# gnlpfjh/Scalable-E3-GNN

Hardware: AMD Instinct MI355X
Metric: particles/sec (octree build + SEGNN fwd), 1M pts l_max=2, 1/2/4/8 MI355X (higher is better)
Workload: dtype f32; 1 GPU; 1000000 particles/GPU uniform in unit box, radius graph k~24 (E=23519616), SEGNN l_max=2 4 layers H=32 f32 storage; particles_per_gpu=1000000, edges_per_gpu=23519616, hidden=32, layers=4, lmax=2, parallelism=single GPU

## Files before the change

include/e3gnn.h:

```cpp
#ifndef E3GNN_H
#define E3GNN_H

#include <stdint.h>

#ifdef __cplusplus
extern "C" {
#endif

#define E3GNN_ABI_VERSION 3

enum {
  E3_OK = 0,
  E3_ERR_INVALID_ARG = 1,
  E3_ERR_BAD_IRREPS = 2,
  E3_ERR_MISSING_WEIGHT = 3,
  E3_ERR_UNSUPPORTED = 4,
  E3_ERR_HIP = 5,
  E3_ERR_NO_DEVICE = 6
};

enum { E3_F32 = 0, E3_F64 = 1, E3_BF16 = 2 };

enum { E3_CLS_0E = 0, E3_CLS_0O = 1, E3_CLS_1E = 2, E3_CLS_1O = 3 };

typedef struct e3_l1tp_plan e3_l1tp_plan;

int         e3_abi_version(void);
const char* e3_status_string(int status);
const char* e3_last_hip_error(void);

int e3_l1tp_plan_create(const int32_t* in1_blocks, int n_in1,
                        const int32_t* out_blocks, int n_out,
                        e3_l1tp_plan** plan);
int e3_l1tp_plan_destroy(e3_l1tp_plan* plan);

int e3_l1tp_in1_dim(const e3_l1tp_plan* plan);
int e3_l1tp_out_dim(const e3_l1tp_plan* plan);
int e3_l1tp_weight_shape(const e3_l1tp_plan* plan, int cls, int* rows, int* cols);
int e3_l1tp_norm_len(const e3_l1tp_plan* plan, int cls);

int64_t e3_l1tp_packed_bytes(const e3_l1tp_plan* plan, int dtype);
int e3_l1tp_pack_weights(const e3_l1tp_plan* plan,
                         const void* const weights[4], const void* const norms[4],
                         int dtype, void* packed, void* stream);

int e3_l1tp_forward(const e3_l1tp_plan* plan,
                    const void* in1, int64_t ld_in1,
                    const void* in2, int64_t ld_in2,
                    const void* packed,
                    void* out, int64_t ld_out,
                    int64_t B, int dtype, int kernel, void* stream);

int64_t e3_l1tp_backward_workspace_bytes(const e3_l1tp_plan* plan, int64_t B, int dtype);
int e3_l1tp_backward(const e3_l1tp_plan* plan,
                     const void* in1, int64_t ld_in1,
                     const void* in2, int64_t ld_in2,
                     const void* const weights[4], const void* const norms[4],
                     const void* grad_out, int64_t ld_gout,
                     void* grad_in1, int64_t ld_gin1,
                     void* grad_in2,
                     void* const grad_weights[4],
                     void* workspace,
                     int64_t B, int dtype, void* stream);

typedef struct e3_rg_params {
  float lo[3], hi[3];
  float r;
  int32_t n[3];
  float inv[3];
  int32_t bits;
} e3_rg_params;

int     e3_rg_grid(e3_rg_params* prm);
int64_t e3_rg_workspace_bytes(int64_t N, const e3_rg_params* prm);
int e3_rg_sort_count(const float* pos, int64_t N, const e3_rg_params* prm,
                     int32_t* perm, float* sorted_pos4, int32_t* rowptr,
                     void* workspace, int64_t workspace_bytes, void* stream);
int e3_rg_fill(int64_t N, const e3_rg_params* prm, const float* sorted_pos4, const int32_t* rowptr,
               int32_t* src, void* workspace, int64_t workspace_bytes, void* stream);

int e3_rg_sort_count_pbc(const float* pos, int64_t N, const e3_rg_params* prm, int32_t periodic,
                         int32_t* perm, float* sorted_pos4, int32_t* rowptr,
                         void* workspace, int64_t workspace_bytes, void* stream);
int e3_rg_fill_pbc(int64_t N, const e3_rg_params* prm, int32_t periodic, const float* sorted_pos4,
                   const int32_t* rowptr, int32_t* src, void* workspace, int64_t workspace_bytes, void* stream);

int e3_cell_derive(const float cell[9], float ginv[9], float heights[3], float* volume);
int e3_rg_sort_count_cell(const float* pos, int64_t N, const e3_rg_params* prm, const float cell[9], const float origin[3],
                          int32_t* perm, float* sorted_pos4, int32_t* rowptr,
                          void* workspace, int64_t workspace_bytes, void* stream);
int e3_rg_fill_cell(int64_t N, const e3_rg_params* prm, const float cell[9], const float origin[3],
                    const float* sorted_pos4, const int32_t* rowptr, int32_t* src,
                    void* workspace, int64_t workspace_bytes, void* stream);

int e3_edge_geometry(const float* pos4, const int32_t* rowptr, const int32_t* src, int64_t N,
                     float* edge_y, float* edge_d, float* node_a, void* stream);
int e3_edge_geometry_pbc(const float* pos4, const int32_t* rowptr, const int32_t* src, int64_t N, const float box[3],
                         float* edge_y, float* edge_d, float* node_a, void* stream);
int e3_edge_geometry_cell(const float* pos4, const int32_t* rowptr, const int32_t* src, int64_t N, const float cell[9],
                          float* edge_y, float* edge_d, float* node_a, void* stream);
int e3_gather_concat(const float* h, int64_t ld_h, int D, const int32_t* rowptr, const int32_t* src, int64_t N,
                     const float* extra, int n_extra, float* out, int64_t ld_out, void* stream);
int e3_gate(const float* in, int64_t ld_in, float* out, int64_t ld_out, int64_t B, int ns, int nv, void* stream);
int e3_segment_sum(const float* msg, int64_t ld_msg, const int32_t* rowptr, int64_t N, int D,
                   float* agg, int64_t ld_agg, void* stream);

int64_t e3_split_edges_workspace_bytes(int64_t N);
int e3_split_edges(const int32_t* rowptr, const int32_t* src, const uint8_t* is_ghost, int64_t N, int64_t E,
                   int32_t* rowptr_kept, int32_t* src_kept, int32_t* dst_kept, int32_t* src_interior, int32_t* dst_interior,
                   int32_t* src_boundary, int32_t* dst_boundary, int32_t* counts, void* workspace, void* stream);

#define E3_HALO_MAX_ENTRIES 26
typedef struct e3_halo_entry {
  float lo[3], hi[3], shift[3];
} e3_halo_entry;
int64_t e3_halo_select_workspace_bytes(int64_t n, int n_entries);
int e3_halo_select_count(const float* pos, int64_t n, const float lo[3], const float hi[3], int32_t periodic, float r,
                         const e3_halo_entry* entries, int n_entries, float* pos_wrapped, int32_t* counts, void* workspace,
                         int64_t workspace_bytes, void* stream);
int e3_halo_select_fill(const float* pos_wrapped, int64_t n, const float lo[3], const float hi[3], int32_t periodic, float r,
                        const e3_halo_entry* entries, int n_entries, int64_t total, int32_t* idx, float* ghost_pos,
                        void* workspace, int64_t workspace_bytes, void* stream);

#define E3_MORTON_MAX_RANKS 64
int e3_morton_keys(const float* pos, int64_t n, const float lo[3], const float hi[3], const int32_t n_cells[3], int32_t* keys,
                   void* stream);
int64_t e3_morton_select_workspace_bytes(int64_t n, int n_ranks);
int e3_morton_select_count(const float* pos, int64_t n, const float lo[3], const float hi[3], const int32_t n_cells[3], float r,
                           const int32_t* splitters, int n_ranks, int self_rank, int32_t* counts, void* workspace,
                           int64_t workspace_bytes, void* stream);
int e3_morton_select_fill(const float* pos, int64_t n, const float lo[3], const float hi[3], const int32_t n_cells[3], float r,
                          const int32_t* splitters, int n_ranks, int self_rank, int64_t total, int32_t* idx, void* workspace,
                          int64_t workspace_bytes, void* stream);

typedef struct e3_tp_plan e3_tp_plan;
typedef struct e3_tp_segment {
  const void* base;
  int64_t ld;
  const int32_t* row_index;
  int32_t ncols;
  int32_t reserved;
} e3_tp_segment;
int e3_tp_plan_create(const int32_t* in1_blocks, int n_in1, int lmax_sh,
                      const int32_t* out_blocks, int n_out, e3_tp_plan** plan);
int e3_tp_plan_destroy(e3_tp_plan* plan);
int e3_tp_in1_dim(const e3_tp_plan* plan);
int e3_tp_in2_dim(const e3_tp_plan* plan);
int e3_tp_out_dim(const e3_tp_plan* plan);
int e3_tp_weight_shape(const e3_tp_plan* plan, int cls, int* rows, int* cols);
int e3_tp_norm_len(const e3_tp_plan* plan, int cls);
int64_t e3_tp_packed_bytes(const e3_tp_plan* plan, int dtype);
int e3_tp_pack_weights(const e3_tp_plan* plan, const void* const weights[6], const void* const norms[6],
                       int dtype, void* packed, void* stream);
int e3_tp_forward(const e3_tp_plan* plan, const void* in1, int64_t ld_in1, const void* in2, int64_t ld_in2,
                  const void* packed, void* out, int64_t ld_out, int64_t B, int dtype, const float* in_scale,
                  int exact, void* stream);
int e3_pow2_scale(const e3_tp_segment* segs, const int64_t* nrows, int nseg, int target_log2, float* out4,
                  void* stream);
int e3_add_pow2_scale(const float* h, const float* u, float* out, int64_t n, int target_log2, float* out4,
                      void* stream);
int e3_tp_forward_fused(const e3_tp_plan* plan, const e3_tp_segment* segs, int nseg,
                        const void* in2, int64_t ld_in2, const void* packed, void* out, int64_t ld_out,
                        int64_t B, int dtype, int gate, const float* in_scale, void* stream);
int e3_tp_forward_fused_epilogue(const e3_tp_plan* plan, const e3_tp_segment* segs, int nseg, const void* in2,
                                 int64_t ld_in2, const void* packed, void* out, int64_t ld_out, int64_t B, int dtype,
                                 int gate, const float* in_scale, const void* residual, int64_t ld_residual,
                                 float* out_scale4, int target_log2, void* stream);
int e3_tp_forward_update_pair(const e3_tp_plan* plan1, const e3_tp_plan* plan2, const e3_tp_segment* segs, int nseg,
                              const void* in2, int64_t ld_in2, const void* packed1, const void* packed2,
                              const float* in_scale, const void* residual, int64_t ld_residual, void* out,
                              int64_t ld_out, int64_t B, int dtype, float* out_scale4, int target_log2, void* stream);
int e3_tp_backward(const e3_tp_plan* plan, const void* in1, int64_t ld_in1, const void* in2, int64_t ld_in2,
                   const void* packed, const void* grad_out, int64_t ld_gout, void* grad_in1, int64_t ld_gin1,
                   void* grad_in2, int64_t ld_gin2, void* const grad_weights[6], int64_t B, int dtype, void* stream);
int e3_tp_backward_weights(const e3_tp_plan* plan, const void* in1, int64_t ld_in1, const void* in2, int64_t ld_in2,
                           const void* packed, const void* grad_out, int64_t ld_gout, void* const grad_weights[6],
                           int64_t B, int dtype, void* stream);
int e3_tp_backward_operands(const e3_tp_plan* plan, const void* in1, int64_t ld_in1, const void* in2, int64_t ld_in2,
                            const void* packed, const void* grad_out, int64_t ld_gout, void* const features[6],
                            void* const gout[6], int64_t B, int dtype, void* stream);
int e3_tp_backward_contract(const e3_tp_plan* plan, const void* in1, int64_t ld_in1, const void* in2, int64_t ld_in2,
                            void* const t[6], void* grad_in1, int64_t ld_gin1, void* grad_in2, int64_t ld_gin2,
                            int64_t B, int dtype, void* stream);
int e3_tp_fused_supported(const e3_tp_plan* plan, int gate);
const char* e3_tp_last_fused_kernel(void);
int e3_tp_forward_fused_scatter(const e3_tp_plan* plan, const e3_tp_segment* segs, int nseg,
                                const void* in2, int64_t ld_in2, const void* packed, const int32_t* row_node,
                                void* out_nodes, int64_t ld_out, int64_t B, int dtype, int gate,
                                const float* in_scale, void* stream);
typedef struct e3_msg_plan e3_msg_plan;
int e3_msg_plan_create(int lmax, int hidden, e3_msg_plan** plan);
int e3_msg_plan_destroy(e3_msg_plan* plan);
int64_t e3_msg_packed_bytes(const e3_msg_plan* plan);
int64_t e3_msg_premix_floats_per_node(const e3_msg_plan* plan);
int e3_msg_weight_shape(const e3_msg_plan* plan, int tp , int l3, int* rows, int* cols);
int e3_msg_supports(const e3_msg_plan* plan, int dtype);
int e3_msg_pack_weights(e3_msg_plan* plan, const void* const w1[3], const void* const n1[3],
                        const void* const w2[3], const void* const n2[3], int dtype, void* packed, void* stream);
int e3_msg_premix(e3_msg_plan* plan, const void* h, int64_t ld_h, int64_t N, const void* packed,
                  const float* in_scale, float* premix, int dtype, void* stream);
int e3_msg_forward(e3_msg_plan* plan, const void* h, int64_t ld_h, int64_t N, const float* pos4,
                   const int32_t* src, const int32_t* dst, int64_t E, const void* packed, const float* in_scale,
                   const float* premix, float* out, int64_t ld_out, int dtype, int accumulate, int tiles_per_block,
                   void* stream);
int e3_msg_forward_pbc(e3_msg_plan* plan, const void* h, int64_t ld_h, int64_t N, const float* pos4,
                       const int32_t* src, const int32_t* dst, int64_t E, const void* packed, const float* in_scale,
                       const float* premix, float* out, int64_t ld_out, int dtype, int accumulate, int tiles_per_block,
                       const float box[3], void* stream);
int e3_msg_forward_cell(e3_msg_plan* plan, const void* h, int64_t ld_h, int64_t N, const float* pos4,
                        const int32_t* src, const int32_t* dst, int64_t E, const void* packed, const float* in_scale,
                        const float* premix, float* out, int64_t ld_out, int dtype, int accumulate, int tiles_per_block,
                        const float cell[9], void* stream);
int e3_segment_sum_bf16(const void* msg, int64_t ld_msg, const int32_t* rowptr, int64_t N, int D,
                        void* agg, int64_t ld_agg, void* stream);
int e3_edge_geometry_l2(const float* pos4, const int32_t* rowptr, const int32_t* src, int64_t N,
                        float* edge_y, float* edge_d, float* node_a, void* stream);
int e3_edge_geometry_l2_pbc(const float* pos4, const int32_t* rowptr, const int32_t* src, int64_t N, const float box[3],
                            float* edge_y, float* edge_d, float* node_a, void* stream);
int e3_edge_geometry_l2_cell(const float* pos4, const int32_t* rowptr, const int32_t* src, int64_t N, const float cell[9],
                             float* edge_y, float* edge_d, float* node_a, void* stream);
int e3_gate_blocks(const float* in, int64_t ld_in, float* out, int64_t ld_out, int64_t B, int ns,
                   int nblocks, const int32_t* ls, const int32_t* muls, void* stream);

int e3_edge_geometry_backward(const float* pos4, const int32_t* rowptr, const int32_t* src, int64_t N, int lmax,
                              const float* g_edge_y, const float* g_edge_d, const float* g_node_a, float* g_pos,
                              void* stream);
int e3_edge_geometry_backward_pbc(const float* pos4, const int32_t* rowptr, const int32_t* src, int64_t N, int lmax,
                                  const float box[3], const float* g_edge_y, const float* g_edge_d,
                                  const float* g_node_a, float* g_pos, void* stream);
int e3_edge_geometry_backward_cell(const float* pos4, const int32_t* rowptr, const int32_t* src, int64_t N, int lmax,
                                   const float cell[9], const float* g_edge_y, const float* g_edge_d,
                                   const float* g_node_a, float* g_pos, void* stream);
int e3_gather_concat_backward(const float* g_out, int64_t ld_gout, int D, const int32_t* rowptr, const int32_t* src,
                              int64_t N, int n_extra, float* g_h, int64_t ld_gh, float* g_extra, void* stream);

int e3_edge_geometry_strained(const float* pos4, const int32_t* rowptr, const int32_t* src, int64_t N, int lmax,
                              const float* box, const float* strain, const int32_t* structure, int S, float* edge_y,
                              float* edge_d, float* node_a, void* stream);
int64_t e3_edge_geometry_backward_strained_workspace_bytes(int64_t N);
int e3_edge_geometry_backward_strained(const float* pos4, const int32_t* rowptr, const int32_t* src, int64_t N, int lmax,
                                       const float* box, const float* strain, const int32_t* structure, int S,
                                       const float* g_edge_y, const float* g_edge_d, const float* g_node_a, float* g_pos,
                                       float* g_strain, void* workspace, int64_t workspace_bytes, void* stream);
int e3_edge_geometry_strained_cell(const float* pos4, const int32_t* rowptr, const int32_t* src, int64_t N, int lmax,
                                   const float cell[9], const float* strain, const int32_t* structure, int S,
                                   float* edge_y, float* edge_d, float* node_a, void* stream);
int e3_edge_geometry_backward_strained_cell(const float* pos4, const int32_t* rowptr, const int32_t* src, int64_t N,
                                            int lmax, const float cell[9], const float* strain, const int32_t* structure,
                                            int S, const float* g_edge_y, const float* g_edge_d, const float* g_node_a,
                                            float* g_pos, float* g_strain, void* workspace, int64_t workspace_bytes,
                                            void* stream);
int e3_gate_blocks_backward(const float* in, int64_t ld_in, const float* g_out, int64_t ld_gout, float* g_in,
                            int64_t ld_gin, int64_t B, int ns, int nblocks, const int32_t* ls, const int32_t* muls,
                            void* stream);
int e3_segment_sum_backward(const float* g_agg, int64_t ld_gagg, const int32_t* rowptr, int64_t N, int D, float* g_msg,
                            int64_t ld_gmsg, void* stream);

#ifdef __cplusplus
}
#endif
#endif
```

scalable-e3-gnn_amd/_lib.py:

```python
from __future__ import annotations

import ctypes
import os
from ctypes import POINTER, c_char_p, c_int, c_int32, c_int64, c_void_p

_HERE = os.path.dirname(os.path.abspath(__file__))
LIB_PATH = os.path.join(_HERE, "lib", "libe3gnn_hip.so")

E3_OK = 0
E3_F32, E3_F64, E3_BF16 = 0, 1, 2
CLS_NAMES = ("l0e", "l0o", "l1e", "l1o")

_lib = None

VoidP4 = c_void_p * 4
Float3 = ctypes.c_float * 3
Float9 = ctypes.c_float * 9
Int3 = c_int32 * 3


class HaloEntry(ctypes.Structure):
    _fields_ = [("lo", ctypes.c_float * 3), ("hi", ctypes.c_float * 3), ("shift", ctypes.c_float * 3)]


SIGNATURES = {
    "e3_abi_version": (c_int, []),
    "e3_status_string": (c_char_p, [c_int]),
    "e3_last_hip_error": (c_char_p, []),
    "e3_l1tp_plan_create": (c_int, [POINTER(c_int32), c_int, POINTER(c_int32), c_int, POINTER(c_void_p)]),
    "e3_l1tp_plan_destroy": (c_int, [c_void_p]),
    "e3_l1tp_in1_dim": (c_int, [c_void_p]),
    "e3_l1tp_out_dim": (c_int, [c_void_p]),
    "e3_l1tp_weight_shape": (c_int, [c_void_p, c_int, POINTER(c_int), POINTER(c_int)]),
    "e3_l1tp_norm_len": (c_int, [c_void_p, c_int]),
    "e3_l1tp_packed_bytes": (c_int64, [c_void_p, c_int]),
    "e3_l1tp_pack_weights": (c_int, [c_void_p, VoidP4, VoidP4, c_int, c_void_p, c_void_p]),
    "e3_l1tp_forward": (c_int, [c_void_p, c_void_p, c_int64, c_void_p, c_int64, c_void_p, c_void_p, c_int64,
                                c_int64, c_int, c_int, c_void_p]),
    "e3_l1tp_backward_workspace_bytes": (c_int64, [c_void_p, c_int64, c_int]),
    "e3_rg_grid": (c_int, [c_void_p]),
    "e3_rg_workspace_bytes": (c_int64, [c_int64, c_void_p]),
    "e3_rg_sort_count": (c_int, [c_void_p, c_int64, c_void_p, c_void_p, c_void_p, c_void_p, c_void_p, c_int64,
                                 c_void_p]),
    "e3_rg_fill": (c_int, [c_int64, c_void_p, c_void_p, c_void_p, c_void_p, c_void_p, c_int64, c_void_p]),
    "e3_edge_geometry": (c_int, [c_void_p, c_void_p, c_void_p, c_int64, c_void_p, c_void_p, c_void_p, c_void_p]),
    "e3_gather_concat": (c_int, [c_void_p, c_int64, c_int, c_void_p, c_void_p, c_int64, c_void_p, c_int, c_void_p,
                                 c_int64, c_void_p]),
    "e3_gate": (c_int, [c_void_p, c_int64, c_void_p, c_int64, c_int64, c_int, c_int, c_void_p]),
    "e3_segment_sum": (c_int, [c_void_p, c_int64, c_void_p, c_int64, c_int, c_void_p, c_int64, c_void_p]),
    "e3_split_edges_workspace_bytes": (c_int64, [c_int64]),
    "e3_split_edges": (c_int, [c_void_p, c_void_p, c_void_p, c_int64, c_int64, c_void_p, c_void_p, c_void_p, c_void_p,
                               c_void_p, c_void_p, c_void_p, c_void_p, c_void_p, c_void_p]),
    "e3_halo_select_workspace_bytes": (c_int64, [c_int64, c_int]),
    "e3_halo_select_count": (c_int, [c_void_p, c_int64, Float3, Float3, c_int32, ctypes.c_float, c_void_p, c_int, c_void_p,
                                     c_void_p, c_void_p, c_int64, c_void_p]),
    "e3_halo_select_fill": (c_int, [c_void_p, c_int64, Float3, Float3, c_int32, ctypes.c_float, c_void_p, c_int, c_int64,
                                    c_void_p, c_void_p, c_void_p, c_int64, c_void_p]),
    "e3_morton_keys": (c_int, [c_void_p, c_int64, Float3, Float3, Int3, c_void_p, c_void_p]),
    "e3_morton_select_workspace_bytes": (c_int64, [c_int64, c_int]),
    "e3_morton_select_count": (c_int, [c_void_p, c_int64, Float3, Float3, Int3, ctypes.c_float, POINTER(c_int32), c_int,
                                       c_int, c_void_p, c_void_p, c_int64, c_void_p]),
    "e3_morton_select_fill": (c_int, [c_void_p, c_int64, Float3, Float3, Int3, ctypes.c_float, POINTER(c_int32), c_int,
                                      c_int, c_int64, c_void_p, c_void_p, c_int64, c_void_p]),
    "e3_tp_plan_create": (c_int, [POINTER(c_int32), c_int, c_int, POINTER(c_int32), c_int, POINTER(c_void_p)]),
    "e3_tp_plan_destroy": (c_int, [c_void_p]),
    "e3_tp_in1_dim": (c_int, [c_void_p]),
    "e3_tp_in2_dim": (c_int, [c_void_p]),
    "e3_tp_out_dim": (c_int, [c_void_p]),
    "e3_tp_weight_shape": (c_int, [c_void_p, c_int, POINTER(c_int), POINTER(c_int)]),
    "e3_tp_norm_len": (c_int, [c_void_p, c_int]),
    "e3_tp_packed_bytes": (c_int64, [c_void_p, c_int]),
    "e3_tp_pack_weights": (c_int, [c_void_p, c_void_p * 6, c_void_p * 6, c_int, c_void_p, c_void_p]),
    "e3_tp_forward": (c_int, [c_void_p, c_void_p, c_int64, c_void_p, c_int64, c_void_p, c_void_p, c_int64, c_int64,
                              c_int, c_void_p, c_int, c_void_p]),
    "e3_tp_forward_fused": (c_int, [c_void_p, c_void_p, c_int, c_void_p, c_int64, c_void_p, c_void_p, c_int64, c_int64,
                                    c_int, c_int, c_void_p, c_void_p]),
    "e3_msg_plan_create": (c_int, [c_int, c_int, POINTER(c_void_p)]),
    "e3_msg_plan_destroy": (c_int, [c_void_p]),
    "e3_msg_packed_bytes": (c_int64, [c_void_p]),
    "e3_msg_premix_floats_per_node": (c_int64, [c_void_p]),
    "e3_msg_weight_shape": (c_int, [c_void_p, c_int, c_int, POINTER(c_int), POINTER(c_int)]),
    "e3_msg_supports": (c_int, [c_void_p, c_int]),
    "e3_msg_pack_weights": (c_int, [c_void_p, c_void_p * 3, c_void_p * 3, c_void_p * 3, c_void_p * 3, c_int, c_void_p,
                                    c_void_p]),
    "e3_msg_premix": (c_int, [c_void_p, c_void_p, c_int64, c_int64, c_void_p, c_void_p, c_void_p, c_int, c_void_p]),
    "e3_msg_forward": (c_int, [c_void_p, c_void_p, c_int64, c_int64, c_void_p, c_void_p, c_void_p, c_int64, c_void_p,
                               c_void_p, c_void_p, c_void_p, c_int64, c_int, c_int, c_int, c_void_p]),
    "e3_edge_geometry_backward": (c_int, [c_void_p, c_void_p, c_void_p, c_int64, c_int, c_void_p, c_void_p, c_void_p,
                                          c_void_p, c_void_p]),
    "e3_rg_sort_count_pbc": (c_int, [c_void_p, c_int64, c_void_p, c_int32, c_void_p, c_void_p, c_void_p, c_void_p,
                                     c_int64, c_void_p]),
    "e3_rg_fill_pbc": (c_int, [c_int64, c_void_p, c_int32, c_void_p, c_void_p, c_void_p, c_void_p, c_int64, c_void_p]),
    "e3_edge_geometry_pbc": (c_int, [c_void_p, c_void_p, c_void_p, c_int64, Float3, c_void_p, c_void_p, c_void_p,
                                     c_void_p]),
    "e3_edge_geometry_l2_pbc": (c_int, [c_void_p, c_void_p, c_void_p, c_int64, Float3, c_void_p, c_void_p, c_void_p,
                                        c_void_p]),
    "e3_edge_geometry_backward_pbc": (c_int, [c_void_p, c_void_p, c_void_p, c_int64, c_int, Float3, c_void_p, c_void_p,
                                              c_void_p, c_void_p, c_void_p]),
    "e3_msg_forward_pbc": (c_int, [c_void_p, c_void_p, c_int64, c_int64, c_void_p, c_void_p, c_void_p, c_int64,
                                   c_void_p, c_void_p, c_void_p, c_void_p, c_int64, c_int, c_int, c_int, Float3,
                                   c_void_p]),
    "e3_cell_derive": (c_int, [Float9, Float9, Float3, POINTER(ctypes.c_float)]),
    "e3_rg_sort_count_cell": (c_int, [c_void_p, c_int64, c_void_p, Float9, Float3, c_void_p, c_void_p, c_void_p, c_void_p,
                                      c_int64, c_void_p]),
    "e3_rg_fill_cell": (c_int, [c_int64, c_void_p, Float9, Float3, c_void_p, c_void_p, c_void_p, c_void_p, c_int64,
                                c_void_p]),
    "e3_edge_geometry_cell": (c_int, [c_void_p, c_void_p, c_void_p, c_int64, Float9, c_void_p, c_void_p, c_void_p,
                                      c_void_p]),
    "e3_edge_geometry_l2_cell": (c_int, [c_void_p, c_void_p, c_void_p, c_int64, Float9, c_void_p, c_void_p, c_void_p,
                                         c_void_p]),
    "e3_edge_geometry_backward_cell": (c_int, [c_void_p, c_void_p, c_void_p, c_int64, c_int, Float9, c_void_p, c_void_p,
                                               c_void_p, c_void_p, c_void_p]),
    "e3_msg_forward_cell": (c_int, [c_void_p, c_void_p, c_int64, c_int64, c_void_p, c_void_p, c_void_p, c_int64,
                                    c_void_p, c_void_p, c_void_p, c_void_p, c_int64, c_int, c_int, c_int, Float9,
                                    c_void_p]),
    "e3_edge_geometry_strained_cell": (c_int, [c_void_p, c_void_p, c_void_p, c_int64, c_int, Float9, c_void_p, c_void_p,
                                               c_int, c_void_p, c_void_p, c_void_p, c_void_p]),
    "e3_edge_geometry_backward_strained_cell": (c_int, [c_void_p, c_void_p, c_void_p, c_int64, c_int, Float9, c_void_p,
                                                        c_void_p, c_int, c_void_p, c_void_p, c_void_p, c_void_p, c_void_p,
                                                        c_void_p, c_int64, c_void_p]),
    "e3_gather_concat_backward": (c_int, [c_void_p, c_int64, c_int, c_void_p, c_void_p, c_int64, c_int, c_void_p, c_int64,
                                          c_void_p, c_void_p]),
    "e3_gate_blocks_backward": (c_int, [c_void_p, c_int64, c_void_p, c_int64, c_void_p, c_int64, c_int64, c_int, c_int,
                                        POINTER(c_int32), POINTER(c_int32), c_void_p]),
    "e3_segment_sum_backward": (c_int, [c_void_p, c_int64, c_void_p, c_int64, c_int, c_void_p, c_int64, c_void_p]),
    "e3_pow2_scale": (c_int, [c_void_p, POINTER(c_int64), c_int, c_int, c_void_p, c_void_p]),
    "e3_add_pow2_scale": (c_int, [c_void_p, c_void_p, c_void_p, c_int64, c_int, c_void_p, c_void_p]),
    "e3_tp_backward": (c_int, [c_void_p, c_void_p, c_int64, c_void_p, c_int64, c_void_p, c_void_p, c_int64, c_void_p,
                               c_int64, c_void_p, c_int64, c_void_p * 6, c_int64, c_int, c_void_p]),
    "e3_tp_backward_weights": (c_int, [c_void_p, c_void_p, c_int64, c_void_p, c_int64, c_void_p, c_void_p, c_int64, c_void_p,
                                       c_int64, c_int, c_void_p]),
    "e3_tp_backward_operands": (c_int, [c_void_p, c_void_p, c_int64, c_void_p, c_int64, c_void_p, c_void_p, c_int64, c_void_p,
                                        c_void_p, c_int64, c_int, c_void_p]),
    "e3_tp_backward_contract": (c_int, [c_void_p, c_void_p, c_int64, c_void_p, c_int64, c_void_p, c_void_p, c_int64, c_void_p,
                                        c_int64, c_int64, c_int, c_void_p]),
    "e3_tp_forward_fused_epilogue": (c_int, [c_void_p, c_void_p, c_int, c_void_p, c_int64, c_void_p, c_void_p, c_int64,
                                             c_int64, c_int, c_int, c_void_p, c_void_p, c_int64, c_void_p, c_int, c_void_p]),
    "e3_tp_forward_update_pair": (c_int, [c_void_p, c_void_p, c_void_p, c_int, c_void_p, c_int64, c_void_p, c_void_p,
                                          c_void_p, c_void_p, c_int64, c_void_p, c_int64, c_int64, c_int, c_void_p, c_int,
                                          c_void_p]),
    "e3_tp_fused_supported": (c_int, [c_void_p, c_int]),
    "e3_tp_last_fused_kernel": (ctypes.c_char_p, []),
    "e3_tp_forward_fused_scatter": (c_int, [c_void_p, c_void_p, c_int, c_void_p, c_int64, c_void_p, c_void_p, c_void_p,
                                            c_int64, c_int64, c_int, c_int, c_void_p, c_void_p]),
    "e3_segment_sum_bf16": (c_int, [c_void_p, c_int64, c_void_p, c_int64, c_int, c_void_p, c_int64, c_void_p]),
    "e3_edge_geometry_l2": (c_int, [c_void_p, c_void_p, c_void_p, c_int64, c_void_p, c_void_p, c_void_p, c_void_p]),
    "e3_gate_blocks": (c_int, [c_void_p, c_int64, c_void_p, c_int64, c_int64, c_int, c_int, POINTER(c_int32),
                               POINTER(c_int32), c_void_p]),
    "e3_l1tp_backward": (c_int, [c_void_p, c_void_p, c_int64, c_void_p, c_int64, VoidP4, VoidP4, c_void_p, c_int64,
                                 c_void_p, c_int64, c_void_p, VoidP4, c_void_p, c_int64, c_int, c_void_p]),
    "e3_edge_geometry_strained": (c_int, [c_void_p, c_void_p, c_void_p, c_int64, c_int, POINTER(ctypes.c_float), c_void_p,
                                          c_void_p, c_int, c_void_p, c_void_p, c_void_p, c_void_p]),
    "e3_edge_geometry_backward_strained_workspace_bytes": (c_int64, [c_int64]),
    "e3_edge_geometry_backward_strained": (c_int, [c_void_p, c_void_p, c_void_p, c_int64, c_int, POINTER(ctypes.c_float),
                                                   c_void_p, c_void_p, c_int, c_void_p, c_void_p, c_void_p, c_void_p,
                                                   c_void_p, c_void_p, c_int64, c_void_p]),
}


def load():
    global _lib
    if _lib is not None:
        return _lib
    if not os.path.exists(LIB_PATH):
        raise RuntimeError(
            f"{LIB_PATH} is missing: the HIP library has not been built. Run "
            "`python -c 'import __graft_entry__ as g; g.build()'` (or `make -C scalable-e3-gnn_amd/csrc`). "
            "There is no CPU fallback.")
    import torch

    lib = ctypes.CDLL(LIB_PATH)
    for name, (res, args) in SIGNATURES.items():
        fn = getattr(lib, name, None)
        if fn is None:
            continue
        fn.restype = res
        fn.argtypes = args
    _lib = lib
    return lib


def check(status: int, what: str = ""):
    if status != E3_OK:
        lib = load()
        msg = lib.e3_status_string(status).decode()
        if status == 5:
            msg += " — " + lib.e3_last_hip_error().decode()
        raise RuntimeError(f"libe3gnn_hip: {what}: {msg} (status {status})")


def blocks_array(blocks):
    flat = [int(v) for b in blocks for v in b]
    return (c_int32 * len(flat))(*flat), len(blocks)


def ptr4(tensors):
    return VoidP4(*[(t.data_ptr() if (t is not None and t.numel() > 0) else None) for t in tensors])


def dtype_code(dtype) -> int:
    import torch

    try:
        return {torch.float32: E3_F32, torch.float64: E3_F64, torch.bfloat16: E3_BF16}[dtype]
    except KeyError:
        raise RuntimeError(f"libe3gnn_hip supports float32 / float64 / bfloat16, got {dtype}") from None


class DevicePlans:

    def __init__(self, create_name: str, destroy_name: str, *args):
        self._create, self._destroy_name, self._args = create_name, destroy_name, args
        self._handles = {}

    def _make(self):
        lib = load()
        cargs = []
        for a in self._args:
            if isinstance(a, (list, tuple)):
                arr, n = blocks_array(a)
                cargs += [arr, n]
            else:
                cargs.append(int(a))
        h = c_void_p()
        check(getattr(lib, self._create)(*cargs, ctypes.byref(h)), self._create)
        return h

    def handle(self, device=None) -> c_void_p:
        key = -1
        if device is not None:
            import torch
            key = torch.device(device).index
            if key is None:
                key = torch.cuda.current_device()
        h = self._handles.get(key)
        if h is None:
            h = self._handles[key] = self._make()
        return h

    def __deepcopy__(self, memo):
        return DevicePlans(self._create, self._destroy_name, *self._args)

    def __reduce__(self):
        return (DevicePlans, (self._create, self._destroy_name) + tuple(self._args))

    def __del__(self):
        try:
            lib = load()
            for h in self._handles.values():
                if h:
                    getattr(lib, self._destroy_name)(h)
            self._handles = {}
        except Exception:
            pass
```

scalable-e3-gnn_amd/csrc/e3_edge_ops.hip:

```cpp
#include "e3_common.h"

#include <algorithm>
#include <cmath>

namespace e3 {

constexpr float kSqrt3 = 1.7320508075688772f;

template <int PBC, bool STRAIN>
__global__ __launch_bounds__(256) void edge_geometry_kernel(const float4* __restrict__ pos4,
                                                            const int32_t* __restrict__ rowptr,
                                                            const int32_t* __restrict__ src, int64_t N,
                                                            float4* __restrict__ edge_y, float* __restrict__ edge_d,
                                                            float4* __restrict__ node_a,
                                                            const typename PbcArg<PBC>::type box, const StrainArg st) {
  const int lane = threadIdx.x & 63;
  const int64_t wave0 = (blockIdx.x * (int64_t)blockDim.x + threadIdx.x) >> 6;
  const int64_t nw = ((int64_t)gridDim.x * blockDim.x) >> 6;
  for (int64_t i = wave0; i < N; i += nw) {
    const int b = rowptr[i], e = rowptr[i + 1];
    const float4 pi = pos4[i];
    float eps[9];
    if constexpr (STRAIN) load_strain(st, row_structure(st, i), eps);
    float sx = 0.f, sy = 0.f, sz = 0.f;
    for (int q = b + lane; q < e; q += 64) {
      const float4 pj = pos4[src[q]];
      float rx, ry, rz;
      edge_rel<PBC>(pj, pi, box, rx, ry, rz);
      if constexpr (STRAIN) apply_strain(eps, rx, ry, rz);
      const float d = sqrtf(rx * rx + ry * ry + rz * rz);
      const float s = d > 0.f ? kSqrt3 / d : 0.f;
      const float4 y = make_float4(1.0f, s * rx, s * ry, s * rz);
      if (edge_y) edge_y[q] = y;
      if (edge_d) edge_d[q] = d;
      sx += y.y; sy += y.z; sz += y.w;
    }
    if (node_a) {
      for (int o = 32; o > 0; o >>= 1) {
        sx += __shfl_xor(sx, o);
        sy += __shfl_xor(sy, o);
        sz += __shfl_xor(sz, o);
      }
      if (lane == 0) {
        const float inv = e > b ? 1.0f / (float)(e - b) : 0.f;
        node_a[i] = make_float4(1.0f, sx * inv, sy * inv, sz * inv);
      }
    }
  }
}

__global__ __launch_bounds__(256) void gather_concat_kernel(const float* __restrict__ h, int64_t ld_h, int D,
                                                            const int32_t* __restrict__ rowptr,
                                                            const int32_t* __restrict__ src, int64_t N,
                                                            const float* __restrict__ extra, int n_extra,
                                                            float* __restrict__ out, int64_t ld_out) {
  const int lane = threadIdx.x & 63;
  const int64_t wave0 = (blockIdx.x * (int64_t)blockDim.x + threadIdx.x) >> 6;
  const int64_t nw = ((int64_t)gridDim.x * blockDim.x) >> 6;
  for (int64_t i = wave0; i < N; i += nw) {
    const int b = rowptr[i], e = rowptr[i + 1];
    if (b == e) continue;
    const float* hi = h + i * ld_h;
    for (int c0 = 0; c0 < D; c0 += 64) {
      const int c = c0 + lane;
      const float vi = c < D ? hi[c] : 0.f;
      for (int q = b; q < e; ++q) {
        if (c < D) {
          float* o = out + (int64_t)q * ld_out;
          o[c] = vi;
          o[D + c] = h[(int64_t)src[q] * ld_h + c];
        }
      }
    }
    for (int q = b; q < e; ++q)
      if (lane < n_extra) out[(int64_t)q * ld_out + 2 * D + lane] = extra[(int64_t)q * n_extra + lane];
  }
}

__device__ __forceinline__ float sigmoidf_(float x) { return 1.0f / (1.0f + __expf(-x)); }

__global__ __launch_bounds__(256) void gate_kernel(const float* __restrict__ in, int64_t ld_in, float* __restrict__ out,
                                                   int64_t ld_out, int64_t B, int ns, int nv) {
  const int W = ns + 3 * nv;
  const int64_t total = B * (int64_t)W;
  for (int64_t t = blockIdx.x * (int64_t)blockDim.x + threadIdx.x; t < total; t += (int64_t)gridDim.x * blockDim.x) {
    const int64_t row = t / W;
    const int c = (int)(t - row * W);
    const float* x = in + row * ld_in;
    float v;
    if (c < ns) {
      const float s = x[c];
      v = s * sigmoidf_(s);
    } else {
      const int k = (c - ns) / 3;
      v = sigmoidf_(x[ns + k]) * x[ns + nv + (c - ns)];
    }
    out[row * ld_out + c] = v;
  }
}

__global__ __launch_bounds__(256) void segment_sum_kernel(const float* __restrict__ msg, int64_t ld_msg,
                                                          const int32_t* __restrict__ rowptr, int64_t N, int D,
                                                          float* __restrict__ agg, int64_t ld_agg) {
  const int lane = threadIdx.x & 63;
  const int64_t wave0 = (blockIdx.x * (int64_t)blockDim.x + threadIdx.x) >> 6;
  const int64_t nw = ((int64_t)gridDim.x * blockDim.x) >> 6;
  for (int64_t i = wave0; i < N; i += nw) {
    const int b = rowptr[i], e = rowptr[i + 1];
    for (int c = lane; c < D; c += 64) {
      float acc = 0.f;
      const float* m = msg + (int64_t)b * ld_msg + c;
#pragma unroll 4
      for (int q = b; q < e; ++q) {
        acc += *m;
        m += ld_msg;
      }
      agg[i * ld_agg + c] = acc;
    }
  }
}


template <int PBC, bool STRAIN>
__global__ __launch_bounds__(256) void edge_geometry_l2_kernel(const float4* __restrict__ pos4,
                                                               const int32_t* __restrict__ rowptr,
                                                               const int32_t* __restrict__ src, int64_t N,
                                                               float* __restrict__ edge_y, float* __restrict__ edge_d,
                                                               float* __restrict__ node_a,
                                                               const typename PbcArg<PBC>::type box, const StrainArg st) {
  const int lane = threadIdx.x & 63;
  const int64_t wave0 = (blockIdx.x * (int64_t)blockDim.x + threadIdx.x) >> 6;
  const int64_t nw = ((int64_t)gridDim.x * blockDim.x) >> 6;
  const float s5 = 2.2360679774997896f;
  for (int64_t i = wave0; i < N; i += nw) {
    const int b = rowptr[i], e = rowptr[i + 1];
    const float4 pi = pos4[i];
    float eps[9];
    if constexpr (STRAIN) load_strain(st, row_structure(st, i), eps);
    float acc[8] = {0, 0, 0, 0, 0, 0, 0, 0};
    for (int q = b + lane; q < e; q += 64) {
      const float4 pj = pos4[src[q]];
      float rx, ry, rz;
      edge_rel<PBC>(pj, pi, box, rx, ry, rz);
      if constexpr (STRAIN) apply_strain(eps, rx, ry, rz);
      const float d = sqrtf(rx * rx + ry * ry + rz * rz);
      const float inv = d > 0.f ? 1.0f / d : 0.f;
      const float x = rx * inv, y = ry * inv, z = rz * inv;
      float Y[9];
      Y[0] = 1.0f;
      Y[1] = kSqrt3 * x; Y[2] = kSqrt3 * y; Y[3] = kSqrt3 * z;
      Y[4] = s5 * kSqrt3 * x * y;
      Y[5] = s5 * kSqrt3 * y * z;
      Y[6] = s5 * 0.5f * (2.f * z * z - x * x - y * y);
      Y[7] = s5 * kSqrt3 * z * x;
      Y[8] = s5 * 0.5f * kSqrt3 * (x * x - y * y);
      if (edge_y) {
        float* o = edge_y + (int64_t)q * 9;
#pragma unroll
        for (int k = 0; k < 9; ++k) o[k] = Y[k];
      }
      if (edge_d) edge_d[q] = d;
#pragma unroll
      for (int k = 0; k < 8; ++k) acc[k] += Y[k + 1];
    }
    if (node_a) {
#pragma unroll
      for (int k = 0; k < 8; ++k)
        for (int o = 32; o > 0; o >>= 1) acc[k] += __shfl_xor(acc[k], o);
      if (lane == 0) {
        const float inv = e > b ? 1.0f / (float)(e - b) : 0.f;
        float* a = node_a + i * 9;
        a[0] = 1.0f;
#pragma unroll
        for (int k = 0; k < 8; ++k) a[k + 1] = acc[k] * inv;
      }
    }
  }
}

struct GateBlocks {
  int nblocks;
  int l[8], mul[8];
};

__global__ __launch_bounds__(256) void gate_blocks_kernel(const float* __restrict__ in, int64_t ld_in,
                                                          float* __restrict__ out, int64_t ld_out, int64_t B, int ns,
                                                          int ngates, int W, GateBlocks gb) {
  const int64_t total = B * (int64_t)W;
  for (int64_t t = blockIdx.x * (int64_t)blockDim.x + threadIdx.x; t < total; t += (int64_t)gridDim.x * blockDim.x) {
    const int64_t row = t / W;
    int c = (int)(t - row * W);
    const float* x = in + row * ld_in;
    float v;
    if (c < ns) {
      const float s = x[c];
      v = s * sigmoidf_(s);
    } else {
      int rem = c - ns, g0 = 0, bi = 0;
      while (rem >= gb.mul[bi] * (2 * gb.l[bi] + 1)) { rem -= gb.mul[bi] * (2 * gb.l[bi] + 1); g0 += gb.mul[bi]; ++bi; }
      const int k = rem / (2 * gb.l[bi] + 1);
      v = sigmoidf_(x[ns + g0 + k]) * x[ngates + c];
    }
    out[row * ld_out + c] = v;
  }
}

__global__ __launch_bounds__(256) void segment_sum_bf16_kernel(const bf16* __restrict__ msg, int64_t ld_msg,
                                                               const int32_t* __restrict__ rowptr, int64_t N, int D,
                                                               bf16* __restrict__ agg, int64_t ld_agg) {
  const int lane = threadIdx.x & 63;
  const int64_t wave0 = (blockIdx.x * (int64_t)blockDim.x + threadIdx.x) >> 6;
  const int64_t nw = ((int64_t)gridDim.x * blockDim.x) >> 6;
  for (int64_t i = wave0; i < N; i += nw) {
    const int b = rowptr[i], e = rowptr[i + 1];
    for (int c = lane; c < D; c += 64) {
      float acc = 0.f;
      const bf16* m = msg + (int64_t)b * ld_msg + c;
#pragma unroll 4
      for (int q = b; q < e; ++q) {
        acc += __bfloat162float(*m);
        m += ld_msg;
      }
      agg[i * ld_agg + c] = __float2bfloat16(acc);
    }
  }
}

static inline int wave_grid(int64_t N) { return (int)std::max<int64_t>(1, std::min<int64_t>((N + 3) / 4, 256 * 16)); }

}

using namespace e3;

template <int PBC>
static int edge_geometry(int lmax, const float* pos4, const int32_t* rowptr, const int32_t* src, int64_t N, float* edge_y,
                         float* edge_d, float* node_a, const typename PbcArg<PBC>::type& b, const StrainArg* st,
                         void* stream) {
  if (N < 0) return E3_ERR_INVALID_ARG;
  if (N == 0) return E3_OK;
  if (!pos4 || !rowptr || !src || (!edge_y && !node_a)) return E3_ERR_INVALID_ARG;
  const StrainArg sa = st ? *st : StrainArg{nullptr, nullptr, 0};
  const hipStream_t s = (hipStream_t)stream;
  if (lmax == 1) {
    auto kern = st ? edge_geometry_kernel<PBC, true> : edge_geometry_kernel<PBC, false>;
    hipLaunchKernelGGL(kern, dim3(wave_grid(N)), dim3(256), 0, s, (const float4*)pos4, rowptr, src, N, (float4*)edge_y,
                       edge_d, (float4*)node_a, b, sa);
  } else {
    auto kern = st ? edge_geometry_l2_kernel<PBC, true> : edge_geometry_l2_kernel<PBC, false>;
    hipLaunchKernelGGL(kern, dim3(wave_grid(N)), dim3(256), 0, s, (const float4*)pos4, rowptr, src, N, edge_y, edge_d,
                       node_a, b, sa);
  }
  E3_HIP_CHECK(hipGetLastError());
  return E3_OK;
}
static int edge_geometry(int lmax, const float* pos4, const int32_t* rowptr, const int32_t* src, int64_t N, float* edge_y,
                         float* edge_d, float* node_a, const float* box, const StrainArg* st, void* stream) {
  const PbcBox b = make_box(box);
  return box ? edge_geometry<kBox>(lmax, pos4, rowptr, src, N, edge_y, edge_d, node_a, b, st, stream)
             : edge_geometry<kOpen>(lmax, pos4, rowptr, src, N, edge_y, edge_d, node_a, b, st, stream);
}

bool e3::cell_derive(const float* cell, float ginv[9], float heights[3], float* volume) {
#pragma clang fp contract(off)
  if (!cell) return false;
  double a[9];
  for (int k = 0; k < 9; ++k) {
    if (!(fabs((double)cell[k]) < 3.0e38)) return false;
    a[k] = (double)cell[k];
  }
  const double c00 = a[4] * a[8] - a[5] * a[7], c01 = a[5] * a[6] - a[3] * a[8], c02 = a[3] * a[7] - a[4] * a[6];
  const double c10 = a[2] * a[7] - a[1] * a[8], c11 = a[0] * a[8] - a[2] * a[6], c12 = a[1] * a[6] - a[0] * a[7];
  const double c20 = a[1] * a[5] - a[2] * a[4], c21 = a[2] * a[3] - a[0] * a[5], c22 = a[0] * a[4] - a[1] * a[3];
  const double det = (a[0] * c00 + a[1] * c01) + a[2] * c02;
  if (!(fabs(det) > 0.0)) return false;
  const double g[9] = {c00 / det, c10 / det, c20 / det, c01 / det, c11 / det, c21 / det, c02 / det, c12 / det, c22 / det};
  for (int k = 0; k < 9; ++k) {
    ginv[k] = (float)g[k];
    if (!(fabsf(ginv[k]) < 3.0e38f)) return false;
  }
  for (int c = 0; c < 3; ++c) {
    heights[c] = (float)(1.0 / sqrt((g[c] * g[c] + g[3 + c] * g[3 + c]) + g[6 + c] * g[6 + c]));
    if (!(heights[c] > 0.0f && heights[c] < 3.0e38f)) return false;
  }
  *volume = (float)fabs(det);
  return *volume > 0.0f && *volume < 3.0e38f;
}

extern "C" {

int e3_edge_geometry(const float* pos4, const int32_t* rowptr, const int32_t* src, int64_t N, float* edge_y,
                     float* edge_d, float* node_a, void* stream) {
  return edge_geometry(1, pos4, rowptr, src, N, edge_y, edge_d, node_a, nullptr, nullptr, stream);
}

int e3_edge_geometry_pbc(const float* pos4, const int32_t* rowptr, const int32_t* src, int64_t N, const float box[3],
                         float* edge_y, float* edge_d, float* node_a, void* stream) {
  if (!box_valid(box, 0.0f)) return E3_ERR_INVALID_ARG;
  return edge_geometry(1, pos4, rowptr, src, N, edge_y, edge_d, node_a, box, nullptr, stream);
}

int e3_cell_derive(const float cell[9], float ginv[9], float heights[3], float* volume) {
  if (!ginv || !heights || !volume) return E3_ERR_INVALID_ARG;
  return cell_derive(cell, ginv, heights, volume) ? E3_OK : E3_ERR_INVALID_ARG;
}

int e3_edge_geometry_cell(const float* pos4, const int32_t* rowptr, const int32_t* src, int64_t N, const float cell[9],
                          float* edge_y, float* edge_d, float* node_a, void* stream) {
  PbcCell c;
  if (!make_cell(cell, 0.0f, &c)) return E3_ERR_INVALID_ARG;
  return edge_geometry<kCell>(1, pos4, rowptr, src, N, edge_y, edge_d, node_a, c, nullptr, stream);
}

int e3_edge_geometry_l2_cell(const float* pos4, const int32_t* rowptr, const int32_t* src, int64_t N, const float cell[9],
                             float* edge_y, float* edge_d, float* node_a, void* stream) {
  PbcCell c;
  if (!make_cell(cell, 0.0f, &c)) return E3_ERR_INVALID_ARG;
  return edge_geometry<kCell>(2, pos4, rowptr, src, N, edge_y, edge_d, node_a, c, nullptr, stream);
}

int e3_edge_geometry_strained_cell(const float* pos4, const int32_t* rowptr, const int32_t* src, int64_t N, int lmax,
                                   const float cell[9], const float* strain, const int32_t* structure, int S,
                                   float* edge_y, float* edge_d, float* node_a, void* stream) {
  PbcCell c;
  if ((lmax != 1 && lmax != 2) || !strain || S < 1 || !make_cell(cell, 0.0f, &c)) return E3_ERR_INVALID_ARG;
  const StrainArg st = {strain, structure, S};
  return edge_geometry<kCell>(lmax, pos4, rowptr, src, N, edge_y, edge_d, node_a, c, &st, stream);
}

int e3_gather_concat(const float* h, int64_t ld_h, int D, const int32_t* rowptr, const int32_t* src, int64_t N,
                     const float* extra, int n_extra, float* out, int64_t ld_out, void* stream) {
  if (N < 0 || D <= 0 || n_extra < 0 || n_extra > 64 || ld_out < 2 * D + n_extra) return E3_ERR_INVALID_ARG;
  if (N == 0) return E3_OK;
  if (!h || !rowptr || !src || !out || (n_extra > 0 && !extra)) return E3_ERR_INVALID_ARG;
  hipLaunchKernelGGL(gather_concat_kernel, dim3(wave_grid(N)), dim3(256), 0, (hipStream_t)stream, h, ld_h, D, rowptr,
                     src, N, extra, n_extra, out, ld_out);
  E3_HIP_CHECK(hipGetLastError());
  return E3_OK;
}

int e3_gate(const float* in, int64_t ld_in, float* out, int64_t ld_out, int64_t B, int ns, int nv, void* stream) {
  if (B < 0 || ns < 0 || nv < 0 || ld_in < ns + 4 * nv || ld_out < ns + 3 * nv) return E3_ERR_INVALID_ARG;
  if (B == 0 || ns + nv == 0) return E3_OK;
  if (!in || !out) return E3_ERR_INVALID_ARG;
  int64_t total = B * (int64_t)(ns + 3 * nv);
  int grid = (int)std::min<int64_t>((total + 255) / 256, 256 * 16);
  hipLaunchKernelGGL(gate_kernel, dim3(grid), dim3(256), 0, (hipStream_t)stream, in, ld_in, out, ld_out, B, ns, nv);
  E3_HIP_CHECK(hipGetLastError());
  return E3_OK;
}

int e3_segment_sum(const float* msg, int64_t ld_msg, const int32_t* rowptr, int64_t N, int D, float* agg,
                   int64_t ld_agg, void* stream) {
  if (N < 0 || D <= 0 || ld_msg < D || ld_agg < D) return E3_ERR_INVALID_ARG;
  if (N == 0) return E3_OK;
  if (!msg || !rowptr || !agg) return E3_ERR_INVALID_ARG;
  hipLaunchKernelGGL(segment_sum_kernel, dim3(wave_grid(N)), dim3(256), 0, (hipStream_t)stream, msg, ld_msg, rowptr, N,
                     D, agg, ld_agg);
  E3_HIP_CHECK(hipGetLastError());
  return E3_OK;
}

int e3_segment_sum_bf16(const void* msg, int64_t ld_msg, const int32_t* rowptr, int64_t N, int D, void* agg,
                        int64_t ld_agg, void* stream) {
  if (N < 0 || D <= 0 || ld_msg < D || ld_agg < D) return E3_ERR_INVALID_ARG;
  if (N == 0) return E3_OK;
  if (!msg || !rowptr || !agg) return E3_ERR_INVALID_ARG;
  hipLaunchKernelGGL(segment_sum_bf16_kernel, dim3(wave_grid(N)), dim3(256), 0, (hipStream_t)stream, (const bf16*)msg,
                     ld_msg, rowptr, N, D, (bf16*)agg, ld_agg);
  E3_HIP_CHECK(hipGetLastError());
  return E3_OK;
}

int e3_edge_geometry_l2(const float* pos4, const int32_t* rowptr, const int32_t* src, int64_t N, float* edge_y,
                        float* edge_d, float* node_a, void* stream) {
  return edge_geometry(2, pos4, rowptr, src, N, edge_y, edge_d, node_a, nullptr, nullptr, stream);
}

int e3_edge_geometry_l2_pbc(const float* pos4, const int32_t* rowptr, const int32_t* src, int64_t N, const float box[3],
                            float* edge_y, float* edge_d, float* node_a, void* stream) {
  if (!box_valid(box, 0.0f)) return E3_ERR_INVALID_ARG;
  return edge_geometry(2, pos4, rowptr, src, N, edge_y, edge_d, node_a, box, nullptr, stream);
}

int e3_edge_geometry_strained(const float* pos4, const int32_t* rowptr, const int32_t* src, int64_t N, int lmax,
                              const float* box, const float* strain, const int32_t* structure, int S, float* edge_y,
                              float* edge_d, float* node_a, void* stream) {
  if ((lmax != 1 && lmax != 2) || !strain || S < 1 || (box && !box_valid(box, 0.0f))) return E3_ERR_INVALID_ARG;
  const StrainArg st = {strain, structure, S};
  return edge_geometry(lmax, pos4, rowptr, src, N, edge_y, edge_d, node_a, box, &st, stream);
}

int e3_gate_blocks(const float* in, int64_t ld_in, float* out, int64_t ld_out, int64_t B, int ns, int nblocks,
                   const int32_t* ls, const int32_t* muls, void* stream) {
  if (B < 0 || ns < 0 || nblocks < 0 || nblocks > 8 || (nblocks > 0 && (!ls || !muls))) return E3_ERR_INVALID_ARG;
  GateBlocks gb;
  gb.nblocks = nblocks;
  int ngates = 0, wide = 0;
  for (int i = 0; i < 8; ++i) { gb.l[i] = 0; gb.mul[i] = 1 << 30; }
  for (int i = 0; i < nblocks; ++i) {
    if (ls[i] < 0 || ls[i] > 2 || muls[i] < 0) return E3_ERR_INVALID_ARG;
    gb.l[i] = ls[i]; gb.mul[i] = muls[i];
    ngates += muls[i];
    wide += muls[i] * (2 * ls[i] + 1);
  }
  const int W = ns + wide;
  if (ld_in < W + ngates || ld_out < W) return E3_ERR_INVALID_ARG;
  if (B == 0 || W == 0) return E3_OK;
  if (!in || !out) return E3_ERR_INVALID_ARG;
  int64_t total = B * (int64_t)W;
  int grid = (int)std::min<int64_t>((total + 255) / 256, 256 * 16);
  hipLaunchKernelGGL(gate_blocks_kernel, dim3(grid), dim3(256), 0, (hipStream_t)stream, in, ld_in, out, ld_out, B, ns,
                     ngates, W, gb);
  E3_HIP_CHECK(hipGetLastError());
  return E3_OK;
}

}
```

scalable-e3-gnn_amd/csrc/e3_msg_fused.hip:

```cpp
#include "e3_common.h"
#include "cg_tables.h"
#include "e3_msg_ws.h"

#include <algorithm>
#include <cstddef>
#include <mutex>
#include <type_traits>
#include <utility>
#include <vector>

#ifndef E3_MSG_WD
#define E3_MSG_WD 1
#endif
#ifndef E3_MSG_UDP
#define E3_MSG_UDP 1
#endif
#ifndef E3_MSG_WPS
#define E3_MSG_WPS 2
#endif

#ifndef E3_MSG_STAMP
#define E3_MSG_STAMP 0
#endif

// ... 774 lines not shown
          f32x4 o;
#pragma unroll
          for (int r = 0; r < 4; ++r) {
            const float sv = a0[t][r] * nv[r] * isrow;
            o[r] = sv * sigmoid_(sv);
          }
          *reinterpret_cast<f32x4*>(wp + 16 * t) = o;
        }
        auto put_block = [&](auto dtag, auto& acc, const int slot, const int gslot, float* wq) {
          constexpr int Dc = decltype(dtag)::value;
#pragma unroll
          for (int t = 0; t < TT; ++t) {
            const f32x4 gn = nt2[4 * (gslot + t)];
            float gt[4];
#pragma unroll
            for (int r = 0; r < 4; ++r) gt[r] = sigmoid_(a0[gslot + t][r] * gn[r] * isrow) * isrow;
            float o[4 * Dc];
#pragma unroll
            for (int c = 0; c < Dc; ++c) {
              const f32x4 nv = nt2[4 * (slot + Dc * t + c)];
#pragma unroll
              for (int r = 0; r < 4; ++r) o[r * Dc + c] = acc[t][c][r] * nv[r] * gt[r];
            }
            f32x4* dq = reinterpret_cast<f32x4*>(wq + 16 * t * Dc);
#pragma unroll
            for (int k = 0; k < Dc; ++k) dq[k] = f32x4{o[4 * k], o[4 * k + 1], o[4 * k + 2], o[4 * k + 3]};
          }
        };
        put_block(std::integral_constant<int, 3>{}, a1, G::slot0(1), TT, wbuf + j * RS + H + 12 * g);
        if constexpr (LMAX == 2) put_block(std::integral_constant<int, 5>{}, a2, G::slot0(2), 2 * TT, wbuf + j * RS + 4 * H + 20 * g);
        wave_sync_lds();
        E3_STAMP(6)
        int ln;
        asm volatile("v_mbcnt_lo_u32_b32 %0, -1, 0\n\tv_mbcnt_hi_u32_b32 %0, -1, %0" : "=v"(ln));
        const float* sp = wbuf + ln;
#pragma unroll
        for (int rb = 0; rb < 16; rb += 4) {
          float v[4][NQ];
#pragma unroll
          for (int rr = 0; rr < 4; ++rr)
#pragma unroll
            for (int q = 0; q < NQ; ++q) v[rr][q] = (64 * q + ln < D) ? sp[(rb + rr) * RS + 64 * q] : 0.f;
#pragma unroll
          for (int rr = 0; rr < 4; ++rr) {
            const int dn = __builtin_amdgcn_readlane(sd, rb + rr);
            if (dn >= 0) {
              if (dn != cur) {
                flush();
                cur = dn;
              }
#pragma unroll
              for (int q = 0; q < NQ; ++q) carry[q] += v[rr][q];
            }
          }
        }
      }
      E3_STAMP(7)
    }
    flush();
    cur = -1;
  }
#if E3_MSG_STAMP
  if (lane == 0)
    for (int i = 0; i < 8; ++i) atomicAdd(&g_msg_stamps[i], (unsigned long long)st_acc[i]);
#endif
#undef E3_STAMP
}

static_assert(std::is_same_v<decltype(&msg_fused_kernel<1, 1, false, kCell>),
                             void (*)(decltype(MsgFusedKernarg::hv), decltype(MsgFusedKernarg::ldh), decltype(MsgFusedKernarg::pos4),
                                      decltype(MsgFusedKernarg::src), decltype(MsgFusedKernarg::dst), decltype(MsgFusedKernarg::E),
                                      decltype(MsgFusedKernarg::packed), decltype(MsgFusedKernarg::U),
                                      decltype(MsgFusedKernarg::in_scale), decltype(MsgFusedKernarg::out),
                                      decltype(MsgFusedKernarg::ldo), decltype(MsgFusedKernarg::blk),
                                      decltype(MsgFusedKernarg::cell))>,
              "MsgFusedKernarg must list the parameters of msg_fused_kernel in order");
static_assert(offsetof(MsgFusedKernarg, cell) == 92 && sizeof(PbcCell) == 72, "the cell follows `int blk` at byte 92");

struct MsgKernels {
  int lmax, tt;
  const void* fused[2];
  const void* fused_pbc[2];
  const void* fused_cell[2];
  const void* premix[2];
  int64_t total_floats;
  int UD, D, lds_tab, lds_wave, nblk, NS, WD, o_norm1, o_norm2, o_wd, o_w, waves_per_simd;
};
template <int LMAX, int TT>
static MsgKernels make_entry() {
  using G = MsgGeom<LMAX, TT>;
  MsgKernels k = {LMAX, TT, {(const void*)msg_fused_kernel<LMAX, TT, false, kOpen>, nullptr},
                  {(const void*)msg_fused_kernel<LMAX, TT, false, kBox>, nullptr},
                  {(const void*)msg_fused_kernel<LMAX, TT, false, kCell>, nullptr},
                  {(const void*)msg_premix_kernel<LMAX, TT, false>, nullptr}, G::total_floats,
                  G::UD, G::D, G::lds_tab, G::lds_wave, G::nblk(), G::NS, G::WD, G::o_norm1, G::o_norm2, G::o_wd, G::o_w,
                  msg_waves_per_simd(LMAX, TT)};
  if constexpr (TT >= 2) {
    k.fused[1] = (const void*)msg_fused_kernel<LMAX, TT, true, kOpen>;
    k.fused_pbc[1] = (const void*)msg_fused_kernel<LMAX, TT, true, kBox>;
    k.fused_cell[1] = (const void*)msg_fused_kernel<LMAX, TT, true, kCell>;
    k.premix[1] = (const void*)msg_premix_kernel<LMAX, TT, true>;
  }
  return k;
}
static const std::vector<MsgKernels>& msg_kernels() {
  static const std::vector<MsgKernels> k = {make_entry<2, 2>(), make_entry<1, 2>(), make_entry<2, 1>(), make_entry<1, 1>(),
                                            make_entry<2, 4>(), make_entry<1, 4>()};
  return k;
}

}

using namespace e3;

struct e3_msg_plan {
  int lmax, H;
  const MsgKernels* k;
  std::vector<MsgPackDesc> desc;
  int rowd[3];
  int K1[3], K2[3], M[3];
  MsgPackDesc* d_desc = nullptr;
  int device = -1;
  int grid[2] = {0, 0};
  int grid_pbc[2] = {0, 0};
  int grid_cell[2] = {0, 0};
  std::mutex mu;
};

static int msg_ensure_device(e3_msg_plan* P) {
  std::lock_guard<std::mutex> lock(P->mu);
  int cur = -1;
  if (hipGetDevice(&cur) != hipSuccess) return E3_ERR_NO_DEVICE;
  if (P->d_desc) return cur == P->device ? E3_OK : E3_ERR_INVALID_ARG;
  MsgPackDesc* d = nullptr;
  E3_HIP_CHECK(hipMalloc((void**)&d, P->desc.size() * sizeof(MsgPackDesc)));
  if (hipMemcpy(d, P->desc.data(), P->desc.size() * sizeof(MsgPackDesc), hipMemcpyHostToDevice) != hipSuccess) {
    (void)hipFree(d);
    return E3_ERR_HIP;
  }
  const size_t lds = (size_t)(P->k->lds_tab + 4 * P->k->lds_wave) * 4 + 4 * 256;
  int cus = 0;
  if (hipDeviceGetAttribute(&cus, hipDeviceAttributeMultiprocessorCount, cur) != hipSuccess || cus <= 0) cus = 256;
  for (int io = 0; io < 2; ++io) {
    if (!P->k->fused[io]) continue;
    for (int pb = 0; pb < 2; ++pb) {
      const void* kern = pb ? P->k->fused_pbc[io] : P->k->fused[io];
      int per_cu = 0;
      if (hipFuncSetAttribute(kern, hipFuncAttributeMaxDynamicSharedMemorySize, (int)lds) != hipSuccess ||
          hipOccupancyMaxActiveBlocksPerMultiprocessor(&per_cu, kern, 256, lds) != hipSuccess || per_cu < 1) {
        (void)hipFree(d);
        return E3_ERR_HIP;
      }
      (pb ? P->grid_pbc : P->grid)[io] = cus * (per_cu < 4 ? per_cu : 4);
    }
  }
  P->device = cur;
  P->d_desc = d;
  return E3_OK;
}

static int msg_ensure_cell(e3_msg_plan* P, int io) {
  std::lock_guard<std::mutex> lock(P->mu);
  if (P->grid_cell[io]) return E3_OK;
  const size_t lds = (size_t)(P->k->lds_tab + 4 * P->k->lds_wave) * 4 + 4 * 256;
  int cus = 0, per_cu = 0;
  if (hipDeviceGetAttribute(&cus, hipDeviceAttributeMultiprocessorCount, P->device) != hipSuccess || cus <= 0) cus = 256;
  const void* kern = P->k->fused_cell[io];
  if (!kern || hipFuncSetAttribute(kern, hipFuncAttributeMaxDynamicSharedMemorySize, (int)lds) != hipSuccess ||
      hipOccupancyMaxActiveBlocksPerMultiprocessor(&per_cu, kern, 256, lds) != hipSuccess || per_cu < 1)
    return E3_ERR_HIP;
  P->grid_cell[io] = cus * (per_cu < 4 ? per_cu : 4);
  return E3_OK;
}

extern "C" {

int e3_msg_plan_create(int lmax, int hidden, e3_msg_plan** plan_out) {
  if (!plan_out || lmax < 1 || lmax > 2) return E3_ERR_INVALID_ARG;
  const MsgKernels* k = nullptr;
  for (auto& e : msg_kernels())
    if (e.lmax == lmax && 16 * e.tt == hidden) k = &e;
  if (!k) return E3_ERR_UNSUPPORTED;
  auto* P = new e3_msg_plan();
  P->lmax = lmax; P->H = hidden; P->k = k;
  const int H = hidden, TT = k->tt, KS = (H + 31) / 32;
  auto ok = [&](int l1, int l2, int l3) {
    return l1 <= lmax && l2 <= lmax && l3 <= lmax && ((l1 + l2 + l3) % 2 == 0) && l3 >= std::abs(l1 - l2) && l3 <= l1 + l2;
  };
  auto T = [&](int l3) { return l3 == 0 ? TT * (1 + lmax) : TT; };
  const int n1[3] = {2 * H + 1, 2 * H, 2 * H}, n2[3] = {H, H, H};
  int wrow1[3][3][3], wrow2[3][3][3];
  for (int l3 = 0; l3 <= 2; ++l3) {
    int r1 = 0, r2 = 0;
    for (int l1 = 0; l1 <= 2; ++l1)
      for (int l2 = 0; l2 <= 2; ++l2) {
        wrow1[l1][l2][l3] = wrow2[l1][l2][l3] = -1;
        if (l3 > lmax || !ok(l1, l2, l3)) continue;
        wrow1[l1][l2][l3] = r1; r1 += n1[l1];
        wrow2[l1][l2][l3] = r2; r2 += n2[l1];
      }
    P->K1[l3] = l3 <= lmax ? r1 : 0;
    P->K2[l3] = l3 <= lmax ? r2 : 0;
    P->M[l3] = l3 <= lmax ? 16 * T(l3) : 0;
    P->rowd[l3] = (l3 <= lmax) ? wrow1[0][l3][l3] + 2 * H : 0;
  }
  int b = 0;
  for (int l1 = 0; l1 <= lmax; ++l1)
    for (int l3 = 0; l3 <= lmax; ++l3)
      for (int l2 = 0; l2 <= lmax; ++l2) {
        if (!ok(l1, l2, l3)) continue;
        for (int ks = 0; ks < KS; ++ks)
          for (int t = 0; t < T(l3); ++t) {
            const int nvalid = std::min(32, H - 32 * ks);
            const int M = 16 * T(l3);
            P->desc.push_back({0, l3, wrow1[l1][l2][l3] + H + 32 * ks, nvalid, M, 16 * t, b + ks * T(l3) + t});
            P->desc.push_back({2, l3, wrow1[l1][l2][l3] + 32 * ks, nvalid, M, 16 * t, b + ks * T(l3) + t});
            P->desc.push_back({1, l3, wrow2[l1][l2][l3] + 32 * ks, nvalid, M, 16 * t, b + ks * T(l3) + t});
          }
        b += KS * T(l3);
      }
  if (b != k->nblk) { delete P; return E3_ERR_INVALID_ARG; }
  *plan_out = P;
  return E3_OK;
}

int e3_msg_plan_destroy(e3_msg_plan* P) {
  if (!P) return E3_OK;
  if (P->d_desc) (void)hipFree(P->d_desc);
  delete P;
  return E3_OK;
}

int64_t e3_msg_packed_bytes(const e3_msg_plan* P) { return P ? (P->k->total_floats * 4 + 255) / 256 * 256 : -1; }
int64_t e3_msg_premix_floats_per_node(const e3_msg_plan* P) { return P ? P->k->UD + 1 : -1; }
int e3_msg_weight_shape(const e3_msg_plan* P, int tp, int l3, int* rows, int* cols) {
  if (!P || !rows || !cols || l3 < 0 || l3 > 2 || (tp != 1 && tp != 2)) return E3_ERR_INVALID_ARG;
  *rows = tp == 1 ? P->K1[l3] : P->K2[l3];
  *cols = P->M[l3];
  return E3_OK;
}

int e3_msg_supports(const e3_msg_plan* P, int dtype) {
  if (!P) return 0;
  return dtype == E3_F32 ? 1 : (dtype == E3_BF16 && P->k->fused[1] != nullptr) ? 1 : 0;
}

int e3_msg_pack_weights(e3_msg_plan* P, const void* const w1[3], const void* const n1[3], const void* const w2[3],
                        const void* const n2[3], int dtype, void* packed, void* stream) {
  if (!P || !w1 || !w2 || !packed) return E3_ERR_INVALID_ARG;
  if (!e3_msg_supports(P, dtype)) return E3_ERR_UNSUPPORTED;
  for (int l = 0; l <= P->lmax; ++l)
    if (!w1[l] || !w2[l]) return E3_ERR_MISSING_WEIGHT;
  int st = msg_ensure_device(P);
  if (st != E3_OK) return st;
  const MsgKernels& k = *P->k;
  MsgPackArgs a;
  for (int l = 0; l < 3; ++l) {
    const bool on = l <= P->lmax;
    a.w1[l] = on ? w1[l] : nullptr; a.w2[l] = on ? w2[l] : nullptr;
    a.n1[l] = (on && n1) ? n1[l] : nullptr; a.n2[l] = (on && n2) ? n2[l] : nullptr;
    a.nw1[l] = on ? (int64_t)P->K1[l] * P->M[l] : 0;
    a.nw2[l] = on ? (int64_t)P->K2[l] * P->M[l] : 0;
    a.rowd[l] = P->rowd[l];
  }
  a.M0 = P->M[0]; a.H = P->H; a.LMAX = P->lmax; a.TT = k.tt; a.NS = k.NS; a.WD = k.WD;
  a.o_norm1 = k.o_norm1; a.o_norm2 = k.o_norm2; a.o_wd = k.o_wd; a.o_w = k.o_w; a.nblk = k.nblk;
  hipStream_t s = (hipStream_t)stream;
  E3_HIP_CHECK(hipMemsetAsync(packed, 0, 256, s));
  const dim3 grid(std::min<int>((int)P->desc.size(), 512));
  if (dtype == E3_F32) {
    hipLaunchKernelGGL(msg_absmax_kernel, dim3(64), dim3(256), 0, s, a, (uint32_t*)packed);
    hipLaunchKernelGGL(msg_pack_kernel<float>, grid, dim3(256), 0, s, a, P->d_desc, (int)P->desc.size(), (float*)packed);
  } else {
    hipLaunchKernelGGL(msg_pack_kernel<bf16>, grid, dim3(256), 0, s, a, P->d_desc, (int)P->desc.size(), (float*)packed);
  }
  E3_HIP_CHECK(hipGetLastError());
  return E3_OK;
}

int e3_msg_premix(e3_msg_plan* P, const void* h, int64_t ld_h, int64_t N, const void* packed, const float* in_scale,
                  float* premix, int dtype, void* stream) {
  if (!P || N < 0) return E3_ERR_INVALID_ARG;
  if (!e3_msg_supports(P, dtype)) return E3_ERR_UNSUPPORTED;
  const MsgKernels& k = *P->k;
  const int io = dtype == E3_BF16 ? 1 : 0, es = io ? 2 : 4;
  if (N == 0) return E3_OK;
  if (!h || !packed || !premix || ld_h < k.D) return E3_ERR_INVALID_ARG;
  if ((ld_h * es & 15) || ((uintptr_t)h & 15) || ((uintptr_t)premix & 15)) return E3_ERR_INVALID_ARG;
  int st = msg_ensure_device(P);
  if (st != E3_OK) return st;
  const int64_t ntiles = (N + 15) / 16;
  const int grid = (int)std::min<int64_t>((ntiles + 3) / 4, 2048);
  float* hmax = premix + (size_t)N * k.UD;
  void* args[] = {&h, &ld_h, &N, &packed, &in_scale, &premix, &hmax};
  if (hipLaunchKernel(k.premix[io], dim3(grid), dim3(256), args, 0, (hipStream_t)stream) != hipSuccess) return E3_ERR_HIP;
  return E3_OK;
}

}

static int msg_forward(e3_msg_plan* P, const void* h, int64_t ld_h, int64_t N, const float* pos4, const int32_t* src,
                       const int32_t* dst, int64_t E, const void* packed, const float* in_scale, const float* premix,
                       float* out, int64_t ld_out, int dtype, int accumulate, int tiles_per_block, void* stream,
                       const float* box, const PbcCell* cell = nullptr) {
  if (!P || N < 0 || E < 0 || E > 0x7fffffffLL - 16) return E3_ERR_INVALID_ARG;
  if (!e3_msg_supports(P, dtype)) return E3_ERR_UNSUPPORTED;
  const MsgKernels& k = *P->k;
  const int io = dtype == E3_BF16 ? 1 : 0, es = io ? 2 : 4;
  if (N == 0) return E3_OK;
  if (!h || !pos4 || !packed || !premix || !out || ld_h < k.D || ld_out < k.D || (E > 0 && (!src || !dst)))
    return E3_ERR_INVALID_ARG;
  if ((ld_h * es & 15) || ((uintptr_t)h & 15) || ((uintptr_t)premix & 15)) return E3_ERR_INVALID_ARG;
  int st = msg_ensure_device(P);
  if (st != E3_OK) return st;
  hipStream_t s = (hipStream_t)stream;
  if (!accumulate) E3_HIP_CHECK(hipMemset2DAsync(out, (size_t)ld_out * 4, 0, (size_t)k.D * 4, (size_t)N, s));
  if (E == 0) return E3_OK;
  if (tiles_per_block >= 0 && msg_ws_supported(P->lmax, P->H, dtype)) {
    st = msg_ws_launch(P->lmax, P->H, dtype, h, ld_h, N, pos4, src, dst, E, packed, in_scale, premix, out, ld_out,
                       tiles_per_block > (1 << 20) ? (1 << 24) : tiles_per_block * 16, s, box, cell);
    if (st != E3_ERR_UNSUPPORTED) return st;
  }
  if (tiles_per_block < 0) tiles_per_block = -tiles_per_block;
  if (cell && (st = msg_ensure_cell(P, io)) != E3_OK) return st;
  const int64_t ntiles = (E + 15) / 16;
  int nwg = (cell ? P->grid_cell : (box ? P->grid_pbc : P->grid))[io];
  nwg = (int)std::min<int64_t>(nwg, (ntiles + 3) / 4);
  nwg = std::max(8, (nwg + 7) / 8 * 8);
  int blk = tiles_per_block > 0 ? tiles_per_block : 4;
  if (blk > (1 << 16)) blk = 1 << 16;
  const size_t lds = (size_t)(k.lds_tab + 4 * k.lds_wave) * 4 + 4 * 256;
  PbcBox pbox;
  if (!cell) pbox = make_box(box);
  void* args[] = {&h, &ld_h, &pos4, &src, &dst, &E, &packed, &premix, &in_scale, &out, &ld_out, &blk,
                  cell ? (void*)cell : (void*)&pbox};
  if (hipLaunchKernel(cell ? k.fused_cell[io] : (box ? k.fused_pbc[io] : k.fused[io]), dim3(nwg), dim3(256), args, lds,
                      s) != hipSuccess)
    return E3_ERR_HIP;
  return E3_OK;
}

extern "C" {

int e3_msg_forward(e3_msg_plan* P, const void* h, int64_t ld_h, int64_t N, const float* pos4, const int32_t* src,
                   const int32_t* dst, int64_t E, const void* packed, const float* in_scale, const float* premix,
                   float* out, int64_t ld_out, int dtype, int accumulate, int tiles_per_block, void* stream) {
  return msg_forward(P, h, ld_h, N, pos4, src, dst, E, packed, in_scale, premix, out, ld_out, dtype, accumulate,
                     tiles_per_block, stream, nullptr);
}

int e3_msg_forward_pbc(e3_msg_plan* P, const void* h, int64_t ld_h, int64_t N, const float* pos4, const int32_t* src,
                       const int32_t* dst, int64_t E, const void* packed, const float* in_scale, const float* premix,
                       float* out, int64_t ld_out, int dtype, int accumulate, int tiles_per_block, const float box[3],
                       void* stream) {
  if (!box_valid(box, 0.0f)) return E3_ERR_INVALID_ARG;
  return msg_forward(P, h, ld_h, N, pos4, src, dst, E, packed, in_scale, premix, out, ld_out, dtype, accumulate,
                     tiles_per_block, stream, box);
}

int e3_msg_forward_cell(e3_msg_plan* P, const void* h, int64_t ld_h, int64_t N, const float* pos4, const int32_t* src,
                        const int32_t* dst, int64_t E, const void* packed, const float* in_scale, const float* premix,
                        float* out, int64_t ld_out, int dtype, int accumulate, int tiles_per_block, const float cell[9],
                        void* stream) {
  PbcCell c;
  if (!make_cell(cell, 0.0f, &c)) return E3_ERR_INVALID_ARG;
  return msg_forward(P, h, ld_h, N, pos4, src, dst, E, packed, in_scale, premix, out, ld_out, dtype, accumulate,
                     tiles_per_block, stream, nullptr, &c);
}

#if E3_MSG_STAMP
int e3_msg_debug_stamps(unsigned long long* out8, int reset) {
  if (out8 && hipMemcpyFromSymbol(out8, HIP_SYMBOL(e3::g_msg_stamps), 64) != hipSuccess) return E3_ERR_HIP;
  if (reset) {
    unsigned long long z[8] = {0, 0, 0, 0, 0, 0, 0, 0};
    if (hipMemcpyToSymbol(HIP_SYMBOL(e3::g_msg_stamps), z, 64) != hipSuccess) return E3_ERR_HIP;
  }
  return E3_OK;
}
#endif
}
```

scalable-e3-gnn_amd/csrc/e3_msg_ws.h:

```cpp
#pragma once
#include <hip/hip_runtime.h>
#include <stdint.h>
namespace e3 {
struct PbcCell;
bool msg_ws_supported(int lmax, int hidden, int dtype);
int msg_ws_launch(int lmax, int hidden, int dtype, const void* h, int64_t ldh, int64_t N, const float* pos4, const int32_t* src,
                  const int32_t* dst, int64_t E, const void* packed, const float* in_scale, const float* premix, float* out,
                  int64_t ldo, int chunk_edges, hipStream_t stream, const float* box = nullptr,
                  const PbcCell* cell = nullptr);
}
```

scalable-e3-gnn_amd/csrc/e3_msg_ws.hip:

```cpp
#include "e3_common.h"
#include "cg_tables.h"
#include "e3_msg_ws.h"

#include <algorithm>
#include <type_traits>

#ifndef E3_WS_STAMP
#define E3_WS_STAMP 0
#endif

namespace e3 {
#include "e3_tp_mfma_core.h"
#include "e3_msg_common.h"

#if E3_WS_STAMP
__device__ unsigned long long g_ws_stamps[8][4];
__device__ unsigned long long g_ws_tp[8][8];
#define WS_TPMARK(i) { if (tpm) { const uint32_t t_ = (uint32_t)__builtin_readcyclecounter(); tpm[i] += t_ - tpm0; tpm0 = t_; } }
#else
#define WS_TPMARK(i)
#endif

template <int LMAX, int TT, bool IO16>
struct Ws {
  using G = MsgGeom<LMAX, TT>;
  static_assert(TT == 2 && (LMAX == 1 || LMAX == 2), "instantiated for H = 32, l_max = 1 / 2");
  static constexpr int H = G::H, D = G::D, NS = G::NS, UD = G::UD;
  static constexpr int ES = IO16 ? 2 : 4;
  static constexpr int NC = (LMAX + 1) * (LMAX + 1);
  static constexpr int NFR = NC + LMAX;
  static constexpr int FRB = IO16 ? 1024 : 2048;
  static constexpr int frag(int l, int a) { return l * l + a; }
  static constexpr int frag_ff(int l) { return NC + l - 1; }
  static constexpr int GA_ROW = (NC - 1) * H * ES;
  static constexpr int GA_STRIDE = GA_ROW + 16;
  static constexpr int GA_BYTES = 16 * GA_STRIDE;
  static constexpr int GB_ROW = H * ES;
  static constexpr int GB_BYTES = 16 * GB_ROW;
  static constexpr int G_BYTES = GA_BYTES + GB_BYTES;
  static constexpr int RS = D + 4;
  static constexpr int U_ROW = UD * 4;
  static constexpr int U_PIECES = (U_ROW + 1023) / 1024, U_LAST = (U_ROW - (U_PIECES - 1) * 1024) / 16;
  static_assert(U_ROW % 16 == 0, "pre-mix rows are copied in 16-byte units");
  static constexpr int o_tab = 0;
  static constexpr int o_tinfo = (o_tab + (2 * NS * 16 + G::WD) * 4 + 15) / 16 * 16;
  static constexpr int o_ids = o_tinfo + 4 * 32;
  static constexpr int o_idok = o_ids + 4 * 128;
  static constexpr int o_pos = o_idok + 16;
  static constexpr int o_hmx = o_pos + 2 * 512;
  static constexpr int o_srow = o_hmx + 2 * 128;
  static constexpr int z_y = 0, z_112 = 12, z_121 = 28, z_211 = 40, z_222 = 56, ZT = LMAX == 2 ? 84 : 12;
  static constexpr int o_zt = o_srow + 2 * 64;
  static constexpr int o_init = o_zt + 2 * 16 * ZT * 4;
  static constexpr int o_g = o_init + G::T(0) * 1024;
  static constexpr int o_b1 = o_g + G_BYTES;
  static constexpr int o_b2 = o_b1 + NFR * FRB;
  static constexpr int o_o = o_b2 + NFR * FRB;
  static constexpr int o_u = o_o + 16 * RS * 4;
  static constexpr int total = o_u + 4 * U_ROW;
  static_assert(total <= 160 * 1024, "LDS image exceeds the CU");
};

struct TileInfo { int e0, n, n0, node0, node1, sl0, sl1; };

__device__ __forceinline__ void dma16(const void* gsrc, uint32_t lds_dst) {
  uint32_t keep;
  asm volatile("s_mov_b32 %0, m0\n\ts_mov_b32 m0, %2\n\ts_nop 0\n\tglobal_load_lds_dwordx4 %1, off\n\ts_mov_b32 m0, %0"
               : "=&s"(keep) : "v"(gsrc), "s"(lds_dst) : "memory");
}
#ifndef WS_UNT
#define WS_UNT 1
#endif
__device__ __forceinline__ void dma16_stream(const void* gsrc, uint32_t lds_dst) {
#if WS_UNT
  uint32_t keep;
  asm volatile("s_mov_b32 %0, m0\n\ts_mov_b32 m0, %2\n\ts_nop 0\n\tglobal_load_lds_dwordx4 %1, off nt\n\ts_mov_b32 m0, %0"
               : "=&s"(keep) : "v"(gsrc), "s"(lds_dst) : "memory");
#else
  dma16(gsrc, lds_dst);
#endif
}
__device__ __forceinline__ void dma4(const void* gsrc, uint32_t lds_dst) {
  uint32_t keep;
  asm volatile("s_mov_b32 %0, m0\n\ts_mov_b32 m0, %2\n\ts_nop 0\n\tglobal_load_lds_dword %1, off\n\ts_mov_b32 m0, %0"
               : "=&s"(keep) : "v"(gsrc), "s"(lds_dst) : "memory");
}
__device__ __forceinline__ void ws_wait_vm0() { asm volatile("s_waitcnt vmcnt(0)" ::: "memory"); }
__device__ __forceinline__ void ws_barrier() { asm volatile("s_waitcnt lgkmcnt(0)\n\ts_barrier" ::: "memory"); }
__device__ __forceinline__ int sgpr(int v) { return __builtin_amdgcn_readfirstlane(v); }
__device__ __forceinline__ void split2_f16_scaled(const float v0, const float v1, const float s, uint32_t& hi, uint32_t& lo) {
  uint32_t h, l;
  asm("v_fma_mixlo_f16 %0, %1, %2, 0 op_sel_hi:[0,0,0]" : "=v"(h) : "v"(s), "v"(v0));
  asm("v_fma_mixhi_f16 %0, %1, %2, 0 op_sel_hi:[0,0,0]" : "+v"(h) : "v"(s), "v"(v1));
  asm("v_fma_mixlo_f16 %0, %1, %2, -%3 op_sel:[0,0,0] op_sel_hi:[0,0,1]" : "=v"(l) : "v"(s), "v"(v0), "v"(h));
  asm("v_fma_mixhi_f16 %0, %1, %2, -%3 op_sel:[0,0,1] op_sel_hi:[0,0,1]" : "+v"(l) : "v"(s), "v"(v1), "v"(h));
  hi = h; lo = l;
}
template <bool IO16>
__device__ __forceinline__ void ws_put4(unsigned char* dst, const float (&f)[4], const float s) {
  if constexpr (IO16) {
    const uint32_t a = __builtin_bit_cast(uint32_t, __builtin_convertvector(f32x2_t{f[0], f[1]}, bf16x2_t));
    const uint32_t b = __builtin_bit_cast(uint32_t, __builtin_convertvector(f32x2_t{f[2], f[3]}, bf16x2_t));
    *reinterpret_cast<uint2*>(dst) = uint2{a, b};
  } else {
    uint32_t h0, l0, h1, l1;
    split2_f16_scaled(f[0], f[1], s, h0, l0);
    split2_f16_scaled(f[2], f[3], s, h1, l1);
    *reinterpret_cast<uint2*>(dst) = uint2{h0, h1};
    *reinterpret_cast<uint2*>(dst + 1024) = uint2{l0, l1};
  }
}
template <class F>
__device__ __forceinline__ void sfor3(F&& f) {
  f(std::integral_constant<int, 0>{}); f(std::integral_constant<int, 1>{}); f(std::integral_constant<int, 2>{});
}

template <int LMAX, int TT, int ROLE>
struct Own {
  using G = MsgGeom<LMAX, TT>;
  static constexpr int t = ROLE & 1;
  static constexpr int LV = ROLE < 2 ? LMAX : LMAX - 1;
  static constexpr int tG = LV > 0 ? TT * LV + t : -1;
  static constexpr int tS = ROLE >= 2 ? t : -1;
  static constexpr int sl3(int s) { return s == 0 ? LV : 0; }
  static constexpr int stile(int s) { return s == 0 ? t : s == 1 ? tG : tS; }
  static constexpr bool shas(int s) { return s == 0 ? LV > 0 : stile(s) >= 0; }
  static constexpr bool has(int s, int l1, int l2) { return shas(s) && G::ok(l1, l2, sl3(s)); }
  static constexpr int widx(int s, int l1, int l2) {
    int n = 0;
    for (int ss = 0; ss < 3; ++ss)
      for (int a = 0; a <= LMAX; ++a)
        for (int b = 0; b <= LMAX; ++b) {
          if (ss == s && a == l1 && b == l2) return has(ss, a, b) ? n : -1;
          if (has(ss, a, b)) ++n;
        }
    return n;
  }
  static constexpr int NW = widx(3, 0, 0);
};

template <int NW>
struct RoleW { uint4 h[NW], l[NW]; };

template <int LMAX, int TT, int ROLE, bool IO16>
__device__ __forceinline__ void ws_load_w(const float* packed, const int prod , const int lane,
                                          RoleW<Own<LMAX, TT, ROLE>::NW>& w) {
  using G = MsgGeom<LMAX, TT>;
  using O = Own<LMAX, TT, ROLE>;
  const unsigned char* base = reinterpret_cast<const unsigned char*>(packed + G::o_w) + (size_t)prod * G::nblk() * 2048 + lane * 16;
  auto one = [&](auto stag, auto atag, auto btag) {
    constexpr int s = decltype(stag)::value, l1 = decltype(atag)::value, l2 = decltype(btag)::value;
    if constexpr (l1 <= LMAX && l2 <= LMAX && O::has(s, l1, l2)) {
      constexpr int i = O::widx(s, l1, l2), blk = G::blk(l1, l2, O::sl3(s)) + O::stile(s);
      w.h[i] = *reinterpret_cast<const uint4*>(base + (size_t)blk * 2048);
      if constexpr (!IO16) w.l[i] = *reinterpret_cast<const uint4*>(base + (size_t)blk * 2048 + 1024);
      else w.l[i] = uint4{0, 0, 0, 0};
    }
  };
  using I0 = std::integral_constant<int, 0>; using I1 = std::integral_constant<int, 1>; using I2 = std::integral_constant<int, 2>;
  auto slot = [&](auto stag) {
    one(stag, I0{}, I0{}); one(stag, I0{}, I1{}); one(stag, I0{}, I2{});
    one(stag, I1{}, I0{}); one(stag, I1{}, I1{}); one(stag, I1{}, I2{});
    one(stag, I2{}, I0{}); one(stag, I2{}, I1{}); one(stag, I2{}, I2{});
  };
  slot(I0{}); slot(I1{}); slot(I2{});
}

#ifndef WS_XROT
#define WS_XROT 2
#endif
#ifndef WS_NREG
#define WS_NREG 1
#endif
#ifndef WS_PRIO1
#define WS_PRIO1 WS_PRIO
#endif
#ifndef WS_LMAX1
#define WS_LMAX1 0
#endif
#ifndef WS_INITMAP
#define WS_INITMAP 0
#endif
#ifndef WS_YROT
#define WS_YROT 0
#endif
#ifndef WS_PF
#define WS_PF 2
#endif
#ifndef WS_PKT
#define WS_PKT 15
#endif
#ifndef WS_PKZ
#define WS_PKZ 11
#endif
#ifndef WS_PRIO
#define WS_PRIO 0
#endif
template <int LMAX>
struct TpItems {
  static constexpr int N = (LMAX + 1) * (LMAX + 1) + LMAX;
  static constexpr int len(int l) { return 2 * l + 1 + (l > 0 ? 1 : 0); }
  static constexpr int start(int l) { int n = 0; for (int k = LMAX; k > l; --k) n += len(k); return n; }
  static constexpr int l1(int i) { int l = LMAX; while (l > 0 && i >= start(l) + len(l)) --l; return l; }
  static constexpr int a(int i) { const int l = l1(i), k = i - start(l); return k < 2 * l + 1 ? k : -1; }
  static constexpr bool first(int i) { return i == start(l1(i)); }
};

template <int LMAX, int TT, int ROLE, bool FIRST, bool IO16>
struct TpRun {
  using G = MsgGeom<LMAX, TT>;
  using O = Own<LMAX, TT, ROLE>;
  using L = Ws<LMAX, TT, IO16>;
  using IT = TpItems<LMAX>;
  static constexpr int LV = O::LV, t = O::t, tG = O::tG, tS = O::tS;
  static constexpr bool SC = tG >= 0 || tS >= 0;

  const RoleW<O::NW>& w;
  const unsigned char* bfr;
  const float* zt;
  const float* urow;
  const float* wd;
  const f32x4* init;
  f32x4 (&accV)[5];
  f32x4& accG;
  f32x4& accS;
  float dsc;
  uint4 bh[WS_PF + 1], bl[WS_PF + 1];
  f32x4 uV[3][3][5];
  f32x4 wdV;
  f32x4 yv[3];
  f32x4 zq[3][3][7];
#if E3_WS_STAMP
  uint32_t* tpm = nullptr;
  uint32_t tpm0 = 0;
#endif
  static constexpr int zoff(int l1, int l2) {
    return (l1 == 1 && l2 == 1 && LV == 2) ? L::z_112 : (l1 == 1 && l2 == 2 && LV == 1) ? L::z_121
         : (l1 == 2 && l2 == 1 && LV == 1) ? L::z_211 : (l1 == 2 && l2 == 2 && LV == 2) ? L::z_222 : -1;
  }
  __device__ __forceinline__ float yy(const int i) const { return yv[i >> 2][i & 3]; }

  template <int I>
  __device__ __forceinline__ void request() {
    if constexpr (I < IT::N) {
      constexpr int L1 = IT::l1(I), a = IT::a(I), slot = I % (WS_PF + 1);
      constexpr int fr = a >= 0 ? L::frag(L1, a) : L::frag_ff(L1);
      if constexpr (a >= 0 || SC) {
        bh[slot] = *reinterpret_cast<const uint4*>(bfr + fr * L::FRB);
        if constexpr (!IO16) bl[slot] = *reinterpret_cast<const uint4*>(bfr + fr * L::FRB + 1024);
        else bl[slot] = uint4{0, 0, 0, 0};
      }
      const f32x4 zero4 = {0.f, 0.f, 0.f, 0.f};
      if constexpr (a >= 0) {
        sfor3([&](auto l2tag) {
          constexpr int L2 = decltype(l2tag)::value;
          if constexpr (LV > 0 && G::ok(L1, L2, LV)) {
            if constexpr (FIRST) uV[L1][L2][a] = *reinterpret_cast<const f32x4*>(urow + G::uoff(L1, L2, LV) + (a * G::T(LV) + t) * 16);
            else uV[L1][L2][a] = zero4;
            if constexpr (a == 0 && zoff(L1, L2) >= 0) {
              constexpr int NZ = ((2 * L1 + 1) * (2 * LV + 1) + 3) / 4;
#pragma unroll
              for (int q = 0; q < NZ; ++q) zq[L1][L2][q] = *reinterpret_cast<const f32x4*>(zt + zoff(L1, L2) + 4 * q);
            }
          }
        });
        if constexpr (L1 == 0 && FIRST && LV > 0) wdV = *reinterpret_cast<const f32x4*>(wd + G::wdoff(LV) + t * 16);
      }
    }
  }

  template <int I>
  __device__ __forceinline__ void compute() {
    constexpr int L1 = IT::l1(I), a = IT::a(I), slot = I % (WS_PF + 1);
    const uint4 xh = bh[slot], xl = bl[slot];
    if constexpr (a >= 0) {
      if constexpr (L1 == 0 && FIRST && LV > 0) {
        uV[0][LV][0] = __builtin_elementwise_fma(wdV, f32x4{dsc, dsc, dsc, dsc}, uV[0][LV][0]);
      }
      sfor3([&](auto l2tag) {
        constexpr int L2 = decltype(l2tag)::value;
        if constexpr (LV > 0 && G::ok(L1, L2, LV)) {
          constexpr int i = O::widx(0, L1, L2);
          uV[L1][L2][a] = mma3<IO16>(w.h[i], w.l[i], xh, xl, uV[L1][L2][a]);
        }
      });
      if constexpr (L1 == 0) {
        if constexpr (tG >= 0) accG = mma3<IO16>(w.h[O::widx(1, 0, 0)], w.l[O::widx(1, 0, 0)], xh, xl, accG);
        if constexpr (tS >= 0) accS = mma3<IO16>(w.h[O::widx(2, 0, 0)], w.l[O::widx(2, 0, 0)], xh, xl, accS);
      }
    } else if constexpr (SC) {
      if constexpr (tG >= 0) accG = mma3<IO16>(w.h[O::widx(1, L1, L1)], w.l[O::widx(1, L1, L1)], xh, xl, accG);
      if constexpr (tS >= 0) accS = mma3<IO16>(w.h[O::widx(2, L1, L1)], w.l[O::widx(2, L1, L1)], xh, xl, accS);
    }
  }

  template <int L1>
  __device__ __forceinline__ void fold() {
    constexpr int D1 = 2 * L1 + 1;
    sfor3([&](auto l2tag) {
      constexpr int L2 = decltype(l2tag)::value;
      if constexpr (LV > 0 && G::ok(L1, L2, LV)) {
        constexpr int D3 = 2 * LV + 1;
        if constexpr (zoff(L1, L2) >= 0) {
#pragma unroll
          for (int c = 0; c < D3; ++c)
#pragma unroll
            for (int aa = 0; aa < D1; ++aa)
              if (z_nonzero<L1, L2, LV>(aa, c)) {
                const float z = zq[L1][L2][(aa * D3 + c) >> 2][(aa * D3 + c) & 3];
                constexpr int zi = (L1 == 1 && L2 == 1) ? 0 : (L1 == 1 && L2 == 2) ? 1 : (L1 == 2 && L2 == 1) ? 2 : 3;
                if constexpr (!IO16 && (WS_PKT & 1) && ((WS_PKZ >> zi) & 1)) {
                  accV[c] = __builtin_elementwise_fma(uV[L1][L2][aa], f32x4{z, z, z, z}, accV[c]);
                } else {
#pragma unroll
                  for (int r = 0; r < 4; ++r) accV[c][r] = __builtin_fmaf(uV[L1][L2][aa][r], z, accV[c][r]);
                }
              }
        } else {
          float y9[9];
#pragma unroll
          for (int i = 0; i < 9; ++i) y9[i] = yy(i);
          float zz[D1][D3];
          make_z<L1, L2, LV>(y9, zz);
#pragma unroll
          for (int c = 0; c < D3; ++c)
#pragma unroll
            for (int aa = 0; aa < D1; ++aa)
              if (z_nonzero<L1, L2, LV>(aa, c)) {
                if constexpr (!IO16 && (WS_PKT & 2)) {
                  accV[c] = __builtin_elementwise_fma(uV[L1][L2][aa], f32x4{zz[aa][c], zz[aa][c], zz[aa][c], zz[aa][c]}, accV[c]);
                } else {
#pragma unroll
                  for (int r = 0; r < 4; ++r) accV[c][r] = __builtin_fmaf(uV[L1][L2][aa][r], zz[aa][c], accV[c][r]);
                }
              }
        }
      }
    });
  }

  template <int I>
  __device__ __forceinline__ void step() {
    request<I + WS_PF>();
    __builtin_amdgcn_sched_barrier(0);
    compute<I>();
    if constexpr (IT::first(I) && IT::l1(I) < LMAX) fold<IT::l1(I) + 1>();
    if constexpr (I + 1 < IT::N && IT::first(I + 1)) { WS_TPMARK(1 + LMAX - IT::l1(I)) }
    if constexpr (I + 1 < IT::N) step<I + 1>();
    else { WS_TPMARK(1 + LMAX) fold<0>(); WS_TPMARK(2 + LMAX) }
  }

  __device__ __forceinline__ void run() {
    const f32x4 zero4 = {0.f, 0.f, 0.f, 0.f};
#pragma unroll
    for (int c = 0; c < 5; ++c) accV[c] = zero4;
#pragma unroll
    for (int q = 0; q < 3; ++q) yv[q] = *reinterpret_cast<const f32x4*>(zt + L::z_y + 4 * q);
    accG = zero4; accS = zero4;
    if constexpr (FIRST) {
      if constexpr (tG >= 0) accG = init[64 * tG];
      if constexpr (tS >= 0) accS = init[64 * tS];
    }
    request<0>();
    if constexpr (WS_PF >= 2) request<1>();
    if constexpr (WS_PF >= 3) request<2>();
    static_assert(WS_PF >= 1 && WS_PF <= 3, "prefetch distance");
    __builtin_amdgcn_sched_barrier(0);
    dsc = yv[2][1];
    WS_TPMARK(0)
    step<0>();
  }
};

template <int LMAX, int TT, int ROLE, bool FIRST, bool IO16>
__device__ __forceinline__ void ws_tp(const RoleW<Own<LMAX, TT, ROLE>::NW>& w, const unsigned char* bfr, const float* zt,
                                      const float* urow, const float* wd, const f32x4* init,
                                      f32x4 (&accV)[5], f32x4& accG, f32x4& accS, float (&y)[10], uint32_t* tpmarks = nullptr) {
  TpRun<LMAX, TT, ROLE, FIRST, IO16> r{w, bfr, zt, urow, wd, init, accV, accG, accS};
#if E3_WS_STAMP
  r.tpm = tpmarks;
  r.tpm0 = (uint32_t)__builtin_readcyclecounter();
#endif
  r.run();
#pragma unroll
  for (int i = 0; i < 10; ++i) y[i] = r.yy(i);
}

template <class BOX>
struct WsArgsT {
  const void* h; int64_t ldh;
  const float4* pos4; const int32_t* src; const int32_t* dst; int64_t E;
  const float* packed; const float* U; const float* hmax; const float* in_scale; float* out; int64_t ldo;
  int chunk;
  BOX box;
};
using WsArgs = WsArgsT<PbcBox>;

template <int LMAX, int TT, bool IO16, int W, int PBC>
__device__ __forceinline__ void ws_run(const WsArgsT<typename PbcArg<PBC>::type>& A, unsigned char* smem) {
  using G = MsgGeom<LMAX, TT>;
  using L = Ws<LMAX, TT, IO16>;
  constexpr int H = G::H, D = G::D, ES = L::ES;
  constexpr bool TEAM1 = W >= 4;
  constexpr int ROLE = W & 3;
  constexpr int SX = TEAM1 ? -1 : ((W + WS_XROT) & 3);
  constexpr int ITB = SX < 0 ? 0 : (WS_INITMAP ? (SX == 3 ? 0 : 4) : 2 * SX);
  constexpr int ITE0 = SX < 0 ? 0 : (WS_INITMAP ? (SX == 3 ? 4 : (SX == 2 ? 6 : 4)) : (SX <= 2 ? 2 * SX + 2 : 2 * SX));
  constexpr int ITE = ITE0 < G::T(0) ? ITE0 : G::T(0);
  constexpr int SY = TEAM1 ? ((W + WS_YROT) & 3) : -1;
  using O = Own<LMAX, TT, ROLE>;
  using I0 = std::integral_constant<int, 0>; using I1 = std::integral_constant<int, 1>; using I2 = std::integral_constant<int, 2>;
  const int lane = threadIdx.x & 63, j = lane & 15, g = lane >> 4;
  const uint32_t lds0 = (uint32_t)(uintptr_t)smem;
  const float* n1tab = reinterpret_cast<const float*>(smem + L::o_tab);
  const float* n2tab = n1tab + G::NS * 16;
  const float* wdtab = n2tab + G::NS * 16;
  const float xs = (!IO16 && A.in_scale) ? A.in_scale[0] : 1.0f;
  const float bwx = A.packed[6] * ((!IO16 && A.in_scale) ? A.in_scale[1] : 1.0f);
  const char* hb = reinterpret_cast<const char*>(A.h);

  auto tinfo = [&](const int tile) -> TileInfo {
    TileInfo ti = {0, 0, 0, -1, -1, 0, 0};
    if (tile >= 0) {
      const int4* p = reinterpret_cast<const int4*>(smem + L::o_tinfo + (tile & 3) * 32);
      const int4 a = p[0], b = p[1];
      ti.e0 = sgpr(a.x); ti.n = sgpr(a.y); ti.n0 = sgpr(a.z); ti.node0 = sgpr(a.w);
      ti.node1 = sgpr(b.x); ti.sl0 = sgpr(b.y); ti.sl1 = sgpr(b.z);
    }
    return ti;
  };

  RoleW<O::NW> w;
  ws_load_w<LMAX, TT, ROLE, IO16>(A.packed, TEAM1 ? 1 : 0, lane, w);
  wait_vm0();
  f32x4 nrS = {0.f, 0.f, 0.f, 0.f}, nrG = {0.f, 0.f, 0.f, 0.f}, nrV[5];
  {
    const f32x4* ntq = reinterpret_cast<const f32x4*>(TEAM1 ? n2tab : n1tab) + g;
    if constexpr (O::tS >= 0) nrS = ntq[4 * O::tS];
#pragma unroll
    for (int c = 0; c < 5; ++c) nrV[c] = f32x4{0.f, 0.f, 0.f, 0.f};
    if constexpr (O::LV > 0) {
      nrG = ntq[4 * O::tG];
#pragma unroll
      for (int c = 0; c < 2 * O::LV + 1; ++c) nrV[c] = ntq[4 * (G::slot0(O::LV) + (2 * O::LV + 1) * O::t + c)];
    }
  }

  const int Ei = (int)A.E;
  const int per_xcd = (int)(gridDim.x >> 3), wg_idx = (int)(blockIdx.x >> 3);
  const int e_per_xcd = ((Ei + 7) / 8 + 15) / 16 * 16;
  const int xlo = (int)(blockIdx.x & 7) * e_per_xcd;
  const int xhi = xlo + e_per_xcd < Ei ? xlo + e_per_xcd : Ei;

  auto gather_part = [&](const int tile, const int part) {
    const int* ids = reinterpret_cast<const int*>(smem + L::o_ids) + (tile & 3) * 32;
    const uint32_t gb = lds0 + L::o_g;
    static_assert(L::GA_ROW % 16 == 0 && L::GA_ROW <= 1024 && (L::GB_ROW == 128 || L::GB_ROW == 64), "copy shapes of the image");
    constexpr int LA = L::GA_ROW / 16;
    constexpr int UPR = L::GB_ROW / 16;
    constexpr int RPC = 64 / UPR;
    const int myid = ids[lane & 15];
    const int ridb = ids[(RPC == 8 ? 8 * part : 0) + lane / UPR];
    asm volatile("s_waitcnt lgkmcnt(0)" ::: "memory");
#pragma unroll
    for (int k = 0; k < 8; ++k) {
      const int r = 8 * part + k;
      const int rid = part == 0 ? __builtin_amdgcn_readlane(myid, k) : __builtin_amdgcn_readlane(myid, 8 + k);
      const char* rowp = hb + ((int64_t)rid * A.ldh + H) * ES;
      if (LA >= 64 || lane < LA) dma16(rowp + lane * 16, sgpr((int)(gb + r * L::GA_STRIDE)));
    }
    if (RPC == 8 || part == 0)
      dma16(hb + (int64_t)ridb * A.ldh * ES + (lane % UPR) * 16, sgpr((int)(gb + L::GA_BYTES + (RPC == 8 ? part * 1024 : 0))));
  };
  auto ids_requested = [&](const int tile) -> bool {
    return sgpr(reinterpret_cast<const int*>(smem + L::o_idok)[tile & 3]) != 0;
  };

  int pci = 0, pe0 = 0, pcend = 0, psl0 = -1, psl1 = -1, plast_node = -1, plast_slot = 0, pnext = 0;
  bool pok = false;
  auto chunk_start = [&](const int ci) {
    pe0 = sgpr(xlo + (ci * per_xcd + wg_idx) * A.chunk);
    pok = pe0 < xhi;
    pcend = sgpr(pe0 + A.chunk < xhi ? pe0 + A.chunk : xhi);
  };
  auto issue_ids = [&](const int tile) {
    if (lane == 0) reinterpret_cast<int*>(smem + L::o_idok)[tile & 3] = pok ? 1 : 0;
    if (pok && lane < 32) {
      int e = pe0 + (lane & 15);
      e = e < Ei ? e : Ei - 1;
      const int32_t* p = (lane < 16 ? A.src : A.dst) + e;
      dma4(p, sgpr((int)(lds0 + L::o_ids + (tile & 3) * 128)));
    }
  };
  auto cut = [&](const int tile) {
    int* tip = reinterpret_cast<int*>(smem + L::o_tinfo) + (tile & 3) * 8;
    if (!pok) {
      if (lane < 8) tip[lane] = lane < 3 ? 0 : (lane < 5 ? -1 : 0);
      issue_ids(tile + 1);
      return;
    }
    const int* ids = reinterpret_cast<const int*>(smem + L::o_ids) + (tile & 3) * 32;
    const int nmax = sgpr(pcend - pe0 < 16 ? pcend - pe0 : 16);
    const int did = ids[16 + j], dprev = ids[16 + (j > 0 ? j - 1 : 0)];
    const unsigned long long m = __ballot(lane >= 1 && lane < nmax && did != dprev);
    const unsigned long long m2 = m & (m - 1);
    const int n0 = sgpr(m ? (int)__builtin_ctzll(m) : nmax);
    const int n = sgpr(m2 ? (int)__builtin_ctzll(m2) : nmax);
    const int node0 = __builtin_amdgcn_readlane(did, 0);
    const int node1 = n0 < n ? __builtin_amdgcn_readlane(did, n0) : -1;
    const int myid = ids[(lane & 16) + ((lane & 15) < n ? (lane & 15) : n - 1)];
    asm volatile("s_waitcnt lgkmcnt(0)" ::: "memory");
    auto alloc = [&](const int avoid) {
      int sl = pnext;
#pragma unroll
      for (int k = 0; k < 3; ++k)
        if (sl == psl0 || sl == psl1 || sl == avoid) sl = (sl + 1) & 3;
      pnext = (sl + 1) & 3;
      return sl;
    };
    auto urow_copy = [&](const int node, const int slot) {
      const char* up = reinterpret_cast<const char*>(A.U) + (int64_t)node * L::U_ROW + lane * 16;
      const uint32_t dstb = lds0 + L::o_u + slot * L::U_ROW;
#pragma unroll
      for (int i = 0; i < L::U_PIECES; ++i)
        if (i + 1 < L::U_PIECES || lane < L::U_LAST) dma16_stream(up + i * 1024, sgpr((int)(dstb + i * 1024)));
    };
    int sl0, sl1 = -1;
    if (node0 == plast_node) sl0 = plast_slot;
    else { sl0 = sgpr(alloc(-1)); urow_copy(node0, sl0); }
    if (node1 >= 0) { sl1 = sgpr(alloc(sl0)); urow_copy(node1, sl1); }
    psl0 = sl0; psl1 = sl1;
    plast_node = node1 >= 0 ? node1 : node0;
    plast_slot = node1 >= 0 ? sl1 : sl0;
    if (lane == 0) {
      tip[0] = pe0; tip[1] = n; tip[2] = n0; tip[3] = node0; tip[4] = node1; tip[5] = sl0; tip[6] = sl1 >= 0 ? sl1 : sl0;
    }
    if (lane < 32) {
      dma16(A.pos4 + myid, sgpr((int)(lds0 + L::o_pos + (tile & 1) * 512)));
      dma4(A.hmax + myid, sgpr((int)(lds0 + L::o_hmx + (tile & 1) * 128)));
    }
    pe0 = sgpr(pe0 + n);
    if (pe0 >= pcend) chunk_start(++pci);
    issue_ids(tile + 1);
  };

  if constexpr (SX == 3) {
    chunk_start(0);
    issue_ids(0);
    ws_wait_vm0();
    asm volatile("s_waitcnt lgkmcnt(0)" ::: "memory");
    const bool ok0 = pok;
    cut(0);
    asm volatile("s_waitcnt lgkmcnt(0)" ::: "memory");
    if (ok0) { gather_part(0, 0); gather_part(0, 1); }
    ws_wait_vm0();
  }
  ws_barrier();

  constexpr int NQ = (D + 63) / 64;
  constexpr bool RSW = SY == 0 || SY == 1;
  constexpr int Q0 = !RSW ? 0 : (SY == 0 ? 0 : (NQ + 1) / 2), Q1 = !RSW ? 0 : (SY == 0 ? (NQ + 1) / 2 : NQ);
  constexpr int NQW = Q1 - Q0 > 0 ? Q1 - Q0 : 1;
  int cur = -1;
  float carry[NQW];
#pragma unroll
  for (int q = 0; q < NQW; ++q) carry[q] = 0.f;
  auto flush = [&]() {
    if (cur >= 0) {
      float* o = A.out + (int64_t)cur * A.ldo;
#pragma unroll
      for (int q = 0; q < Q1 - Q0; ++q)
        if (64 * (Q0 + q) + lane < D) __builtin_amdgcn_global_atomic_fadd_f32(o + 64 * (Q0 + q) + lane, carry[q]);
    }
#pragma unroll
    for (int q = 0; q < NQW; ++q) carry[q] = 0.f;
  };
#if E3_WS_STAMP
  uint32_t tpmk[8] = {0, 0, 0, 0, 0, 0, 0, 0};
  uint32_t st_acc[4] = {0, 0, 0, 0}, st_t = (uint32_t)__builtin_readcyclecounter();
#define WS_STAMP(i) { const uint32_t t_ = (uint32_t)__builtin_readcyclecounter(); st_acc[i] += t_ - st_t; st_t = t_; }
  uint32_t pm_t = 0;
#define WS_PM0 { pm_t = (uint32_t)__builtin_readcyclecounter(); }
#define WS_PM(i) { const uint32_t t_ = (uint32_t)__builtin_readcyclecounter(); tpmk[i] += t_ - pm_t; pm_t = t_; }
#else
  uint32_t* const tpmk = nullptr;
#define WS_STAMP(i)
#define WS_PM0
#define WS_PM(i)
#endif
  TileInfo t0 = tinfo(0), t1 = tinfo(-1);
  for (int s = 0;; ++s) {
    if (s >= 1 && t1.n == 0) break;
    WS_STAMP(3)
    WS_PM0
    if constexpr (SX == 3) cut(s + 1);
    if constexpr (!TEAM1) {
      if (SX <= 1 && t0.n > 0) {
        const int j8 = lane & 7, gg = (lane >> 3) & 3, pc = lane >> 5, row = 8 * SX + j8;
        const unsigned char* gimg = smem + L::o_g;
        unsigned char* b1 = smem + L::o_b1 + (16 * gg + row) * 16 + 8 * pc;
        const float4* pp = reinterpret_cast<const float4*>(smem + L::o_pos + (s & 1) * 512);
        const float4 ps = pp[row], pd = pp[16 + row];
        float q2[20], q1[12], q0[4];
        {
          const unsigned char* r2 = gimg + row * L::GA_STRIDE + (LMAX == 2 ? (3 * H + (16 * pc + 4 * gg) * 5) * ES : 0);
          const unsigned char* r1 = gimg + row * L::GA_STRIDE + (16 * pc + 4 * gg) * 3 * ES;
          const unsigned char* r0 = gimg + L::GA_BYTES + row * L::GB_ROW + (16 * pc + 4 * gg) * ES;
          if constexpr (!IO16) {
#pragma unroll
            for (int u = 0; u < (LMAX == 2 ? 5 : 0); ++u) { const f32x4 v = reinterpret_cast<const f32x4*>(r2)[u]; q2[4 * u] = v[0]; q2[4 * u + 1] = v[1]; q2[4 * u + 2] = v[2]; q2[4 * u + 3] = v[3]; }
#pragma unroll
            for (int u = 0; u < 3; ++u) { const f32x4 v = reinterpret_cast<const f32x4*>(r1)[u]; q1[4 * u] = v[0]; q1[4 * u + 1] = v[1]; q1[4 * u + 2] = v[2]; q1[4 * u + 3] = v[3]; }
            { const f32x4 v = reinterpret_cast<const f32x4*>(r0)[0]; q0[0] = v[0]; q0[1] = v[1]; q0[2] = v[2]; q0[3] = v[3]; }
          } else {
            auto widen = [](const uint2 v, float* o) {
              o[0] = __builtin_bit_cast(float, v.x << 16); o[1] = __builtin_bit_cast(float, v.x & 0xffff0000u);
              o[2] = __builtin_bit_cast(float, v.y << 16); o[3] = __builtin_bit_cast(float, v.y & 0xffff0000u);
            };
#pragma unroll
            for (int u = 0; u < (LMAX == 2 ? 5 : 0); ++u) widen(reinterpret_cast<const uint2*>(r2)[u], q2 + 4 * u);
#pragma unroll
            for (int u = 0; u < 3; ++u) widen(reinterpret_cast<const uint2*>(r1)[u], q1 + 4 * u);
            widen(reinterpret_cast<const uint2*>(r0)[0], q0);
          }
        }
        __builtin_amdgcn_sched_barrier(0);
        float y[9], dist;
        if constexpr (LMAX == 2) edge_sh<PBC>(ps, pd, y, dist, A.box); else edge_sh1<PBC>(ps, pd, y, dist, A.box);
        auto put4 = [&](const int fr, const float (&f)[4]) { ws_put4<IO16>(b1 + fr * L::FRB, f, xs); };
        auto degree = [&](auto ltag, float* q) {
          constexpr int L1 = decltype(ltag)::value, D1 = 2 * L1 + 1;
#pragma unroll
          for (int a = 0; a < D1; ++a) {
            const float f[4] = {q[a], q[D1 + a], q[2 * D1 + a], q[3 * D1 + a]};
            put4(L::frag(L1, a), f);
          }
          if constexpr (L1 > 0) {
            float zz[D1][1];
            make_z<L1, L1, 0>(y, zz);
            float f[4];
#pragma unroll
            for (int r = 0; r < 4; ++r) {
              float sum = zz[0][0] * q[r * D1];
#pragma unroll
              for (int a = 1; a < D1; ++a) sum = __builtin_fmaf(zz[a][0], q[r * D1 + a], sum);
              f[r] = sum;
            }
            put4(L::frag_ff(L1), f);
          }
        };
        if constexpr (LMAX == 2) degree(I2{}, q2);
        degree(I1{}, q1);
        degree(I0{}, q0);
      }
      if ((ITB < ITE || SX == 2) && t0.n > 0) {
        const float4* pp = reinterpret_cast<const float4*>(smem + L::o_pos + (s & 1) * 512);
        const float4 ps = pp[j], pd = pp[16 + j];
        const int slot = (j >= t0.n0 && j < t0.n) ? t0.sl1 : t0.sl0;
        const float* urow = reinterpret_cast<const float*>(smem + L::o_u + slot * L::U_ROW) + 4 * g;
        constexpr int T0 = G::T(0);
        float y[9], dist;
        if constexpr (LMAX == 2) edge_sh<PBC>(ps, pd, y, dist, A.box); else edge_sh1<PBC>(ps, pd, y, dist, A.box);
        const float dsc = dist * xs;
        float z110[3][1], z220[5][1];
        make_z<1, 1, 0>(y, z110);
        if constexpr (LMAX == 2) make_z<2, 2, 0>(y, z220);
        f32x4* ip = reinterpret_cast<f32x4*>(smem + L::o_init) + lane;
        static_assert(T0 == 6 || T0 == 4, "two scalar-type tiles per wave (0, 1, 2 / 0, 1)");
#pragma unroll
        for (int t2 = ITB; t2 < ITE; t2 += 2) {
          f32x4 u0[2], u1[3][2], u2[5][2], wv[2];
#pragma unroll
          for (int k = 0; k < 2; ++k) {
            const int tt = t2 + k;
            u0[k] = *reinterpret_cast<const f32x4*>(urow + G::uoff(0, 0, 0) + tt * 16);
            wv[k] = *reinterpret_cast<const f32x4*>(wdtab + 4 * g + G::wdoff(0) + tt * 16);
#pragma unroll
            for (int a = 0; a < 3; ++a) u1[a][k] = *reinterpret_cast<const f32x4*>(urow + G::uoff(1, 1, 0) + (a * T0 + tt) * 16);
            if constexpr (LMAX == 2) {
#pragma unroll
              for (int a = 0; a < 5; ++a) u2[a][k] = *reinterpret_cast<const f32x4*>(urow + G::uoff(2, 2, 0) + (a * T0 + tt) * 16);
            }
          }
          __builtin_amdgcn_sched_barrier(0);
#pragma unroll
          for (int k = 0; k < 2; ++k) {
            f32x4 v = u0[k];
#pragma unroll
            for (int r = 0; r < 4; ++r) {
              v[r] = __builtin_fmaf(wv[k][r], dsc, v[r]);
#pragma unroll
              for (int a = 0; a < 3; ++a) v[r] = __builtin_fmaf(u1[a][k][r], z110[a][0], v[r]);
              if constexpr (LMAX == 2) {
#pragma unroll
                for (int a = 0; a < 5; ++a) v[r] = __builtin_fmaf(u2[a][k][r], z220[a][0], v[r]);
              }
            }
            ip[64 * (t2 + k)] = v;
          }
          __builtin_amdgcn_sched_barrier(0);
        }
        if constexpr (SX == 2) {
        float* zr = reinterpret_cast<float*>(smem + L::o_zt + (s & 1) * 16 * L::ZT * 4) + j * L::ZT;
        auto store_dense = [&](auto atag, auto btag, auto ctag, float* dstp) {
          constexpr int A1 = decltype(atag)::value, B1 = decltype(btag)::value, C1 = decltype(ctag)::value;
          constexpr int Da = 2 * A1 + 1, Dc = 2 * C1 + 1, NE = Da * Dc;
          float zz[Da][Dc];
          make_z<A1, B1, C1>(y, zz);
          float flat[(NE + 3) / 4 * 4];
#pragma unroll
          for (int i = 0; i < (NE + 3) / 4 * 4; ++i) flat[i] = i < NE ? zz[i / Dc][i % Dc] : 0.f;
#pragma unroll
          for (int q = 0; q < (NE + 3) / 4; ++q)
            *reinterpret_cast<f32x4*>(dstp + 4 * q) = f32x4{flat[4 * q], flat[4 * q + 1], flat[4 * q + 2], flat[4 * q + 3]};
        };
        if (g == 0) {
          *reinterpret_cast<f32x4*>(zr + L::z_y) = f32x4{y[0], y[1], y[2], y[3]};
          *reinterpret_cast<f32x4*>(zr + L::z_y + 4) = f32x4{y[4], y[5], y[6], y[7]};
          *reinterpret_cast<f32x4*>(zr + L::z_y + 8) = f32x4{y[8], dsc, 0.f, 0.f};
          if constexpr (LMAX == 2) store_dense(I1{}, I1{}, I2{}, zr + L::z_112);
        } else if constexpr (LMAX == 2) {
          if (g == 1) {
            store_dense(I1{}, I2{}, I1{}, zr + L::z_121);
          } else if (g == 2) {
            store_dense(I2{}, I1{}, I1{}, zr + L::z_211);
          } else {
            store_dense(I2{}, I2{}, I2{}, zr + L::z_222);
          }
        }
        }
      }
    } else {
      if (t1.n > 0) {
        float y[10];
        const float* ztr = reinterpret_cast<const float*>(smem + L::o_zt + ((s - 1) & 1) * 16 * L::ZT * 4) + j * L::ZT;
        const uint32_t sb = reinterpret_cast<const uint32_t*>(smem + L::o_srow)[((s - 1) & 1) * 16 + j];
        const float isrow = IO16 ? 1.0f : __builtin_bit_cast(float, 0x7F000000u - sb);
        f32x4 accV[5], accG, accS;
        __builtin_amdgcn_s_setprio(WS_PRIO);
        WS_PM(5)
        ws_tp<LMAX, TT, ROLE, false, IO16>(w, smem + L::o_b2 + lane * 16, ztr, nullptr, nullptr, nullptr, accV, accG, accS, y, tpmk);
        WS_PM0
        const f32x4* nt = reinterpret_cast<const f32x4*>(n2tab) + g;
        float* orow = reinterpret_cast<float*>(smem + L::o_o) + j * L::RS;
        if constexpr (O::tS >= 0) {
          const f32x4 nv = WS_NREG ? nrS : nt[4 * O::tS];
          f32x4 o;
#pragma unroll
          for (int r = 0; r < 4; ++r) {
            const float sv = accS[r] * nv[r] * isrow;
            o[r] = sv * sigmoid_(sv);
          }
          *reinterpret_cast<f32x4*>(orow + 16 * O::t + 4 * g) = o;
        }
        if constexpr (O::LV > 0) {
          constexpr int Dc = 2 * O::LV + 1;
          const f32x4 gn = WS_NREG ? nrG : nt[4 * O::tG];
          f32x4 gt;
#pragma unroll
          for (int r = 0; r < 4; ++r) gt[r] = sigmoid_(accG[r] * gn[r] * isrow) * isrow;
          float o[4 * Dc];
#pragma unroll
          for (int c = 0; c < Dc; ++c) {
            const f32x4 nv = WS_NREG ? nrV[c] : nt[4 * (G::slot0(O::LV) + Dc * O::t + c)];
            f32x4 oc;
            if constexpr (!IO16 && (WS_PKT & 4)) {
              oc = accV[c] * nv * gt;
            } else {
#pragma unroll
              for (int r = 0; r < 4; ++r) oc[r] = accV[c][r] * nv[r] * gt[r];
            }
#pragma unroll
            for (int r = 0; r < 4; ++r) o[r * Dc + c] = oc[r];
          }
          f32x4* dq = reinterpret_cast<f32x4*>(orow + G::col0(O::LV) + (16 * O::t + 4 * g) * Dc);
#pragma unroll
          for (int k = 0; k < Dc; ++k) dq[k] = f32x4{o[4 * k], o[4 * k + 1], o[4 * k + 2], o[4 * k + 3]};
        }
      }
    }
    if constexpr (TEAM1) __builtin_amdgcn_s_setprio(0);
    WS_PM(6)
    WS_STAMP(0)
    ws_barrier();
    WS_STAMP(1)
    WS_PM0
    if constexpr (!TEAM1) {
      if (t0.n > 0) {
        float y[10];
        const float* ztr = reinterpret_cast<const float*>(smem + L::o_zt + (s & 1) * 16 * L::ZT * 4) + j * L::ZT;
        const float* hm = reinterpret_cast<const float*>(smem + L::o_hmx + (s & 1) * 128);
        const float hs = hm[j], hd = hm[16 + j];
        const int slot = (j >= t0.n0 && j < t0.n) ? t0.sl1 : t0.sl0;
        const float* urow = reinterpret_cast<const float*>(smem + L::o_u + slot * L::U_ROW) + 4 * g;
        f32x4 accV[5], accG, accS;
        __builtin_amdgcn_s_setprio(WS_PRIO1);
        WS_PM(5)
        ws_tp<LMAX, TT, ROLE, true, IO16>(w, smem + L::o_b1 + lane * 16, ztr, urow, wdtab + 4 * g,
                                          reinterpret_cast<const f32x4*>(smem + L::o_init) + lane, accV, accG, accS, y, tpmk);
        WS_PM0
        const float dsc = y[9];
        float srow = 1.0f;
        if constexpr (!IO16) srow = pow2_scale_from_bits(__builtin_bit_cast(uint32_t, bwx * fmaxf(fmaxf(hs, hd), dsc)), 12);
        const f32x4* nt = reinterpret_cast<const f32x4*>(n1tab) + g;
        unsigned char* b2 = smem + L::o_b2 + lane * 16 + 8 * O::t;
        auto put4 = [&](const int fr, const float (&f)[4]) { ws_put4<IO16>(b2 + fr * L::FRB, f, srow); };
        if constexpr (O::tS >= 0) {
          const f32x4 nv = WS_NREG ? nrS : nt[4 * O::tS];
          float f[4];
#pragma unroll
          for (int r = 0; r < 4; ++r) {
            const float sv = accS[r] * nv[r];
            f[r] = sv * sigmoid_(sv);
          }
          put4(L::frag(0, 0), f);
        }
        if constexpr (O::LV > 0) {
          constexpr int Dc = 2 * O::LV + 1;
          const f32x4 gn = WS_NREG ? nrG : nt[4 * O::tG];
          f32x4 gt;
#pragma unroll
          for (int r = 0; r < 4; ++r) gt[r] = sigmoid_(accG[r] * gn[r]);
          float y9[9];
#pragma unroll
          for (int i = 0; i < 9; ++i) y9[i] = y[i];
          float zz[Dc][1];
          make_z<O::LV, O::LV, 0>(y9, zz);
          f32x4 fsv = {0.f, 0.f, 0.f, 0.f};
#pragma unroll
          for (int c = 0; c < Dc; ++c) {
            const f32x4 nv = WS_NREG ? nrV[c] : nt[4 * (G::slot0(O::LV) + Dc * O::t + c)];
            f32x4 fv;
            if constexpr (!IO16 && (WS_PKT & 8)) {
              fv = accV[c] * nv * gt;
              const f32x4 zc = {zz[c][0], zz[c][0], zz[c][0], zz[c][0]};
              fsv = c == 0 ? zc * fv : __builtin_elementwise_fma(zc, fv, fsv);
            } else {
#pragma unroll
              for (int r = 0; r < 4; ++r) {
                fv[r] = accV[c][r] * nv[r] * gt[r];
                fsv[r] = c == 0 ? zz[0][0] * fv[r] : __builtin_fmaf(zz[c][0], fv[r], fsv[r]);
              }
            }
            const float f[4] = {fv[0], fv[1], fv[2], fv[3]};
            put4(L::frag(O::LV, c), f);
          }
          const float fs[4] = {fsv[0], fsv[1], fsv[2], fsv[3]};
          put4(L::frag_ff(O::LV), fs);
        }
        if constexpr (ROLE == 3 && !IO16) {
          if (lane < 16) reinterpret_cast<float*>(smem + L::o_srow)[(s & 1) * 16 + lane] = srow;
        }
      }
      if constexpr (SX == 3) ws_wait_vm0();
    } else if constexpr (RSW) {
      if (t1.n > 0) {
        const float* op = reinterpret_cast<const float*>(smem + L::o_o) + lane;
        float s0[NQW], s1[NQW];
#pragma unroll
        for (int q = 0; q < NQW; ++q) { s0[q] = 0.f; s1[q] = 0.f; }
        float v[16][NQW];
#pragma unroll
        for (int r = 0; r < 16; ++r)
#pragma unroll
          for (int q = 0; q < Q1 - Q0; ++q) v[r][q] = (64 * (Q0 + q) + lane < D) ? op[r * L::RS + 64 * (Q0 + q)] : 0.f;
        __builtin_amdgcn_sched_barrier(0);
        if (t1.n0 == 16) {
#pragma unroll
          for (int r = 0; r < 16; ++r)
#pragma unroll
            for (int q = 0; q < Q1 - Q0; ++q) s0[q] += v[r][q];
        } else {
#pragma unroll
          for (int r = 0; r < 16; ++r) {
#pragma unroll
            for (int q = 0; q < Q1 - Q0; ++q) {
              s0[q] += r < t1.n0 ? v[r][q] : 0.f;
              s1[q] += (r >= t1.n0 && r < t1.n) ? v[r][q] : 0.f;
            }
          }
        }
        if (t1.node0 != cur) { flush(); cur = t1.node0; }
#pragma unroll
        for (int q = 0; q < NQW; ++q) carry[q] += s0[q];
        if (t1.node1 >= 0) {
          flush();
          cur = t1.node1;
#pragma unroll
          for (int q = 0; q < NQW; ++q) carry[q] = s1[q];
        }
      }
    } else {
      if (ids_requested(s + 1)) gather_part(s + 1, SY - 2);
      ws_wait_vm0();
    }
    if constexpr (!TEAM1) __builtin_amdgcn_s_setprio(0);
    const TileInfo tn = tinfo(s + 1);
    WS_PM(7)
    WS_STAMP(2)
    ws_barrier();
    t1 = t0; t0 = tn;
  }
  if constexpr (RSW) flush();
#if E3_WS_STAMP
  if (lane == 0) {
    for (int i = 0; i < 4; ++i) atomicAdd(&g_ws_stamps[W][i], (unsigned long long)st_acc[i]);
    for (int i = 0; i < 8; ++i) atomicAdd(&g_ws_tp[W][i], (unsigned long long)tpmk[i]);
  }
#endif
#undef WS_STAMP
}

template <int LMAX, int TT, bool IO16, int PBC>
__global__ __launch_bounds__(512, 2) __attribute__((amdgpu_waves_per_eu(2, 2))) void msg_ws_kernel(
    const WsArgsT<typename PbcArg<PBC>::type> A) {
  using G = MsgGeom<LMAX, TT>;
  using L = Ws<LMAX, TT, IO16>;
  extern __shared__ __align__(16) unsigned char ws_smem[];
  {
    float* n1tab = reinterpret_cast<float*>(ws_smem + L::o_tab);
    float* n2tab = n1tab + G::NS * 16;
    float* wdtab = n2tab + G::NS * 16;
    const float ixs = (!IO16 && A.in_scale) ? A.in_scale[1] : 1.0f;
    for (int i = threadIdx.x; i < G::NS * 16; i += blockDim.x) {
      n1tab[i] = A.packed[G::o_norm1 + i] * ixs;
      n2tab[i] = A.packed[G::o_norm2 + i];
    }
    for (int i = threadIdx.x; i < G::WD; i += blockDim.x) wdtab[i] = A.packed[G::o_wd + i];
  }
  __syncthreads();
  const int wave = __builtin_amdgcn_readfirstlane((int)(threadIdx.x >> 6));
  switch (wave) {
    case 0: ws_run<LMAX, TT, IO16, 0, PBC>(A, ws_smem); break;
    case 1: ws_run<LMAX, TT, IO16, 1, PBC>(A, ws_smem); break;
    case 2: ws_run<LMAX, TT, IO16, 2, PBC>(A, ws_smem); break;
    case 3: ws_run<LMAX, TT, IO16, 3, PBC>(A, ws_smem); break;
    case 4: ws_run<LMAX, TT, IO16, 4, PBC>(A, ws_smem); break;
    case 5: ws_run<LMAX, TT, IO16, 5, PBC>(A, ws_smem); break;
    case 6: ws_run<LMAX, TT, IO16, 6, PBC>(A, ws_smem); break;
    default: ws_run<LMAX, TT, IO16, 7, PBC>(A, ws_smem); break;
  }
}

bool msg_ws_supported(int lmax, int hidden, int dtype) {
  return (lmax == 2 || (lmax == 1 && WS_LMAX1)) && hidden == 32 && (dtype == E3_F32 || dtype == E3_BF16);
}

int msg_ws_launch(int lmax, int hidden, int dtype, const void* h, int64_t ldh, int64_t N, const float* pos4, const int32_t* src,
                  const int32_t* dst, int64_t E, const void* packed, const float* in_scale, const float* premix, float* out,
                  int64_t ldo, int chunk_edges, hipStream_t stream, const float* box, const PbcCell* cell) {
  if (!msg_ws_supported(lmax, hidden, dtype)) return E3_ERR_UNSUPPORTED;
  const int pb = cell ? kCell : (box ? kBox : kOpen);
  if (E > 0x7fffffffLL - 65536) return E3_ERR_UNSUPPORTED;
  const int io = dtype == E3_BF16 ? 1 : 0;
  const int li = lmax == 2 ? 1 : 0;
#if WS_LMAX1
  const void* kern =
      pb == kCell
          ? (li ? (io ? (const void*)msg_ws_kernel<2, 2, true, kCell> : (const void*)msg_ws_kernel<2, 2, false, kCell>)
                : (io ? (const void*)msg_ws_kernel<1, 2, true, kCell> : (const void*)msg_ws_kernel<1, 2, false, kCell>))
      : pb ? (li ? (io ? (const void*)msg_ws_kernel<2, 2, true, kBox> : (const void*)msg_ws_kernel<2, 2, false, kBox>)
                 : (io ? (const void*)msg_ws_kernel<1, 2, true, kBox> : (const void*)msg_ws_kernel<1, 2, false, kBox>))
           : (li ? (io ? (const void*)msg_ws_kernel<2, 2, true, kOpen> : (const void*)msg_ws_kernel<2, 2, false, kOpen>)
                 : (io ? (const void*)msg_ws_kernel<1, 2, true, kOpen> : (const void*)msg_ws_kernel<1, 2, false, kOpen>));
  const int lds = li ? (io ? Ws<2, 2, true>::total : Ws<2, 2, false>::total) : (io ? Ws<1, 2, true>::total : Ws<1, 2, false>::total);
  const int ud = li ? MsgGeom<2, 2>::UD : MsgGeom<1, 2>::UD;
#else
  const void* kern =
      pb == kCell ? (io ? (const void*)msg_ws_kernel<2, 2, true, kCell> : (const void*)msg_ws_kernel<2, 2, false, kCell>)
      : pb        ? (io ? (const void*)msg_ws_kernel<2, 2, true, kBox> : (const void*)msg_ws_kernel<2, 2, false, kBox>)
                  : (io ? (const void*)msg_ws_kernel<2, 2, true, kOpen> : (const void*)msg_ws_kernel<2, 2, false, kOpen>);
  const int lds = io ? Ws<2, 2, true>::total : Ws<2, 2, false>::total;
  const int ud = MsgGeom<2, 2>::UD;
#endif
  int dev = 0;
  E3_HIP_CHECK(hipGetDevice(&dev));
  static std::mutex mu;
  static int cus_of[64][2][2][3];
  int cus = 0;
  {
    std::lock_guard<std::mutex> lock(mu);
    if (dev < 0 || dev >= 64) return E3_ERR_INVALID_ARG;
    if (cus_of[dev][io][li][pb] == 0) {
      E3_HIP_CHECK(hipFuncSetAttribute(kern, hipFuncAttributeMaxDynamicSharedMemorySize, lds));
      int n = 0;
      if (hipDeviceGetAttribute(&n, hipDeviceAttributeMultiprocessorCount, dev) != hipSuccess || n <= 0) n = 256;
      cus_of[dev][io][li][pb] = n;
    }
    cus = cus_of[dev][io][li][pb];
  }
  int chunk = chunk_edges > 0 ? (chunk_edges + 15) / 16 * 16 : 256;
  const int64_t nchunks = (E + chunk - 1) / chunk;
  int nwg = (int)std::min<int64_t>(cus, nchunks);
  nwg = std::max(8, (nwg + 7) / 8 * 8);
  const float* hmax = premix + (size_t)N * ud;
  auto launch = [&](const auto& pbc) {
    WsArgsT<std::decay_t<decltype(pbc)>> a = {h, ldh, reinterpret_cast<const float4*>(pos4), src, dst, E,
                                              static_cast<const float*>(packed), premix, hmax, in_scale, out, ldo, chunk, pbc};
    void* args[] = {&a};
    return hipLaunchKernel(kern, dim3(nwg), dim3(512), args, lds, stream) == hipSuccess ? E3_OK : E3_ERR_HIP;
  };
  return cell ? launch(*cell) : launch(make_box(box));
}

}

#if E3_WS_STAMP
extern "C" int e3_msg_ws_debug_stamps(unsigned long long* out96, int reset) {
  if (out96 && hipMemcpyFromSymbol(out96, HIP_SYMBOL(e3::g_ws_stamps), 256) != hipSuccess) return E3_ERR_HIP;
  if (out96 && hipMemcpyFromSymbol(out96 + 32, HIP_SYMBOL(e3::g_ws_tp), 512) != hipSuccess) return E3_ERR_HIP;
  if (reset) {
    unsigned long long z[64] = {0};
    if (hipMemcpyToSymbol(HIP_SYMBOL(e3::g_ws_stamps), z, 256) != hipSuccess) return E3_ERR_HIP;
    if (hipMemcpyToSymbol(HIP_SYMBOL(e3::g_ws_tp), z, 512) != hipSuccess) return E3_ERR_HIP;
  }
  return E3_OK;
}
#endif
```

scalable-e3-gnn_amd/message.py:

```python
from __future__ import annotations

import ctypes

import torch

from . import _lib, profiling
from .radius_graph import RadiusGraph

_NAT = ("l0e", "l1o", "l2e")


class FusedMessage:

    def __init__(self, lmax: int, hidden: int):
        self.lmax, self.hidden = int(lmax), int(hidden)
        self._plans = _lib.DevicePlans("e3_msg_plan_create", "e3_msg_plan_destroy", self.lmax, self.hidden)
        self._packed = {}
        self.tiles_per_block = 0

    def __deepcopy__(self, memo):
        return FusedMessage(self.lmax, self.hidden)

    def __reduce__(self):
        return (FusedMessage, (self.lmax, self.hidden))

    @staticmethod
    def supported(lmax: int, hidden: int) -> bool:
        return lmax in (1, 2) and hidden in (16, 32, 64)

    @property
    def width(self) -> int:
        return self.hidden * (self.lmax + 1) ** 2

    def _tensors(self, tp):
        ws = [getattr(tp, "weights_" + c, None) for c in _NAT]
        ns = [getattr(tp, "norm_" + c, None) for c in _NAT]
        return ws, ns

    def supports(self, dtype) -> bool:
        if dtype == torch.float32:
            return True
        return dtype == torch.bfloat16 and bool(_lib.load().e3_msg_supports(self._plans.handle(None), _lib.E3_BF16))

    def packed(self, msg1, msg2, device, dtype=torch.float32) -> torch.Tensor:
        lib = _lib.load()
        w1, n1 = self._tensors(msg1)
        w2, n2 = self._tensors(msg2)
        ts = w1 + n1 + w2 + n2
        key = tuple((t.data_ptr(), t._version) if t is not None else None for t in ts)
        hit = self._packed.get((device, dtype))
        stream = torch.cuda.current_stream(device)
        if hit is not None and hit[0] == key:
            if hit[2] != stream.cuda_stream:
                stream.wait_event(hit[3])
            return hit[1]
        h = self._plans.handle(device)
        for tpi, ws in ((1, w1), (2, w2)):
            for l in range(self.lmax + 1):
                rows, cols = ctypes.c_int(), ctypes.c_int()
                lib.e3_msg_weight_shape(h, tpi, l, ctypes.byref(rows), ctypes.byref(cols))
                w = ws[l]
                if w is None or tuple(w.shape) != (rows.value, cols.value) or w.dtype != dtype or w.device != device:
                    raise RuntimeError(f"fused message: TP #{tpi} weights of degree {l} must be {dtype} "
                                       f"[{rows.value}, {cols.value}] on {device}, got "
                                       f"{None if w is None else (tuple(w.shape), w.dtype, w.device)}")
        P3 = ctypes.c_void_p * 3
        keep = [t.detach().contiguous() if t is not None else None for t in ts]
        ptr = lambda t: t.data_ptr() if (t is not None and t.numel()) else None
        packed = torch.empty(int(lib.e3_msg_packed_bytes(h)), dtype=torch.uint8, device=device)
        with torch.cuda.device(device):
            for t in keep[3:6] + keep[9:12]:
                if t is not None and t.numel() and t.dtype != dtype:
                    raise RuntimeError(f"fused message: norm buffers must be {dtype} (cast the module), got {t.dtype}")
            _lib.check(lib.e3_msg_pack_weights(h, P3(*map(ptr, keep[0:3])), P3(*map(ptr, keep[3:6])),
                                               P3(*map(ptr, keep[6:9])), P3(*map(ptr, keep[9:12])), _lib.dtype_code(dtype),
                                               packed.data_ptr(), stream.cuda_stream), "e3_msg_pack_weights")
        ev = torch.cuda.Event()
        ev.record(stream)
        self._packed[(device, dtype)] = (key, packed, stream.cuda_stream, ev)
        return packed

    def flops_per_edge(self) -> int:
        H, L = self.hidden, self.lmax
        fl = 0
        for tp, n in ((1, [2 * H + 1, 2 * H, 2 * H]), (2, [H, H, H])):
            for l3 in range(L + 1):
                M = H * (1 + L) if l3 == 0 else H
                for l1 in range(L + 1):
                    for l2 in range(L + 1):
                        if abs(l1 - l2) <= l3 <= l1 + l2 and (l1 + l2 + l3) % 2 == 0:
                            fl += 2 * n[l1] * M * min(2 * l1 + 1, 2 * l3 + 1)
        return fl

    def refresh_row_max(self, state, h: torch.Tensor, rows: torch.Tensor, in_scale: torch.Tensor | None):
        premix = state[1]
        N = h.shape[0]
        ud = premix.numel() // N - 1
        hmax = premix[N * ud:]
        if rows.numel():
            a = h[rows].float().abs()
            m = torch.where(a < float("inf"), a, 0.0).amax(1)
        else:
            m = h.new_zeros(0, dtype=torch.float32)
        if in_scale is not None and h.dtype == torch.float32:
            m = m * in_scale[0]
        hmax[rows] = m
        return m.max() if m.numel() else torch.zeros((), device=h.device)

    def executed_flops_per_edge(self) -> int:
        H, L = self.hidden, self.lmax
        fl = 0
        for _tp in (1, 2):
            for l3 in range(L + 1):
                M = H * (1 + L) if l3 == 0 else H
                for l1 in range(L + 1):
                    for l2 in range(L + 1):
                        if abs(l1 - l2) <= l3 <= l1 + l2 and (l1 + l2 + l3) % 2 == 0:
                            groups = 1 if (l3 == 0 and l1 > 0) else (2 * l1 + 1)
                            fl += 2 * H * M * groups
        return fl

    def forward(self, h: torch.Tensor, g: RadiusGraph, msg1, msg2, in_scale: torch.Tensor | None = None, edges=None,
                cont=None, return_state: bool = False):
        if not h.is_cuda or not self.supports(h.dtype):
            raise RuntimeError(f"fused message: ROCm tensor in float32 (or bfloat16 for hidden >= 32) required, got "
                               f"{h.dtype} on {h.device} (no CPU path)")
        io, code, esz = h.dtype, _lib.dtype_code(h.dtype), h.element_size()
        N, W = h.shape
        if W != self.width or N != g.rowptr.numel() - 1:
            raise RuntimeError(f"fused message: h must be [{g.rowptr.numel() - 1}, {self.width}], got {tuple(h.shape)}")
        if h.stride(-1) != 1 or (h.stride(0) * esz) % 16 or h.data_ptr() % 16:
            h = h.contiguous()
        dev = h.device
        lib = _lib.load()
        src, dst = (g.src, g.dst) if edges is None else edges
        E = int(src.numel())
        assert src.dtype == torch.int32 and dst.dtype == torch.int32 and dst.numel() == E
        if cont is None:
            out = torch.empty((N, W), dtype=torch.float32, device=dev)
        else:
            out = cont[0]
        if N == 0:
            return (out.to(io), None) if return_state else out.to(io)
        with torch.cuda.device(dev):
            packed = self.packed(msg1, msg2, dev, io)
            if in_scale is None and io == torch.float32:
                from . import ops
                in_scale = ops.pow2_scale([h])
            sc = in_scale.data_ptr() if (in_scale is not None and io == torch.float32) else None
            hd = self._plans.handle(dev)
            stream = torch.cuda.current_stream(dev).cuda_stream
            mode = "<bf16 storage, bf16 MFMA>" if io == torch.bfloat16 else "<fp16x3 split MFMA>"
            ud = int(lib.e3_msg_premix_floats_per_node(hd))
            if cont is not None:
                premix = cont[1]
            else:
                premix = torch.empty(N * ud, dtype=torch.float32, device=dev)
                t0 = profiling.begin() if profiling.enabled() else None
                _lib.check(lib.e3_msg_premix(hd, h.data_ptr(), h.stride(0), N, packed.data_ptr(), sc,
                                             premix.data_ptr(), code, stream), "e3_msg_premix")
                if t0 is not None:
                    profiling.end(f"msg_premix lmax={self.lmax} H={self.hidden} N={N} {io}", N, N * (esz * W + 4 * ud), t0,
                                  flops=2 * self.hidden * ud * N, kernel="e3::msg_premix_kernel" + mode)
            t0 = profiling.begin() if profiling.enabled() else None
            args = (hd, h.data_ptr(), h.stride(0), N, g.pos4.data_ptr(), src.data_ptr(), dst.data_ptr(), E,
                    packed.data_ptr(), sc, premix.data_ptr(), out.data_ptr(), out.stride(0), code,
                    0 if cont is None else 1, int(self.tiles_per_block))
            if g.cell is not None:
                _lib.check(lib.e3_msg_forward_cell(*args, g.cell_arg, stream), "e3_msg_forward_cell")
            elif g.box is not None:
                _lib.check(lib.e3_msg_forward_pbc(*args, g.box_arg, stream), "e3_msg_forward_pbc")
            else:
                _lib.check(lib.e3_msg_forward(*args, stream), "e3_msg_forward")
            if t0 is not None:
                nb = esz * N * W + 16 * N + 8 * E + 4 * N * W
                ws = bool(self.lmax == 2 and self.hidden == 32 and int(self.tiles_per_block) >= 0)
                profiling.end(f"msg_fused lmax={self.lmax} H={self.hidden} E={E} {io}", E, nb, t0,
                              flops=self.flops_per_edge() * E,
                              kernel=("e3::msg_ws_kernel" if ws else "e3::msg_fused_kernel") + mode,
                              executed_flops=self.executed_flops_per_edge() * E)
        return (out, (out, premix)) if return_state else out
```

scalable-e3-gnn_amd/ops.py:

```python
from __future__ import annotations

import torch

from . import _lib
from .radius_graph import RadiusGraph


def _check(t: torch.Tensor, name: str):
    if not t.is_cuda:
        raise RuntimeError(f"{name}: ROCm tensor required (no CPU path)")
    if t.dtype != torch.float32:
        raise RuntimeError(f"{name}: float32 required, got {t.dtype}")


def _stream(t):
    return torch.cuda.current_stream(t.device).cuda_stream


def _wants_grad(*ts) -> bool:
    return torch.is_grad_enabled() and any(t is not None and t.requires_grad for t in ts)


def _edge_geometry_raw(pos4, g, want_dist, want_node_attr, lmax, want_edge=True, strain=None, structure=None):
    N, E, dev = g.rowptr.numel() - 1, g.num_edges, pos4.device
    ny = (lmax + 1) ** 2
    Y = torch.empty((E, ny), dtype=torch.float32, device=dev) if want_edge else None
    d = torch.empty(E, dtype=torch.float32, device=dev) if (want_dist and want_edge) else None
    A = torch.empty((N, ny), dtype=torch.float32, device=dev) if want_node_attr else None
    fn = {1: "e3_edge_geometry", 2: "e3_edge_geometry_l2"}[lmax]
    outs = (Y.data_ptr() if Y is not None else None, d.data_ptr() if d is not None else None,
            A.data_ptr() if A is not None else None, _stream(pos4))
    with torch.cuda.device(dev):
        if strain is not None and g.cell is not None:
            _lib.check(_lib.load().e3_edge_geometry_strained_cell(
                pos4.data_ptr(), g.rowptr.data_ptr(), g.src.data_ptr(), N, lmax, g.cell_arg, strain.data_ptr(),
                structure.data_ptr() if structure is not None else None, strain.shape[0], *outs),
                "e3_edge_geometry_strained_cell")
        elif strain is not None:
            _lib.check(_lib.load().e3_edge_geometry_strained(
                pos4.data_ptr(), g.rowptr.data_ptr(), g.src.data_ptr(), N, lmax, g.box_arg, strain.data_ptr(),
                structure.data_ptr() if structure is not None else None, strain.shape[0], *outs),
                "e3_edge_geometry_strained")
        elif g.cell is not None:
            _lib.check(getattr(_lib.load(), fn + "_cell")(pos4.data_ptr(), g.rowptr.data_ptr(), g.src.data_ptr(), N,
                                                          g.cell_arg, *outs), fn + "_cell")
        elif g.box is not None:
            _lib.check(getattr(_lib.load(), fn + "_pbc")(pos4.data_ptr(), g.rowptr.data_ptr(), g.src.data_ptr(), N,
                                                         g.box_arg, *outs), fn + "_pbc")
        else:
            _lib.check(getattr(_lib.load(), fn)(pos4.data_ptr(), g.rowptr.data_ptr(), g.src.data_ptr(), N, *outs),
                       "e3_edge_geometry")
    return Y, d, A


def _strain_args(strain, structure, g):
    N = g.rowptr.numel() - 1
    if tuple(strain.shape) == (3, 3):
        strain = strain.reshape(1, 3, 3)
    if strain.dim() != 3 or tuple(strain.shape[1:]) != (3, 3) or strain.shape[0] < 1:
        raise ValueError(f"strain must be [S,3,3] (S >= 1) or [3,3], got {tuple(strain.shape)}")
    if structure is not None:
        if structure.dim() != 1 or structure.shape[0] != N:
            raise ValueError(f"structure must be [N] = [{N}] (graph order), got {tuple(structure.shape)}")
        if structure.dtype.is_floating_point or structure.dtype.is_complex or structure.dtype == torch.bool:
            raise ValueError(f"structure must be an integer tensor, got {structure.dtype}")
    _check(strain, "strain")
    if structure is not None:
        if not structure.is_cuda:
            raise RuntimeError("structure: ROCm tensor required (no CPU path)")
        structure = structure.to(torch.int32).contiguous()
    return strain.contiguous(), structure


class _EdgeGeometryFn(torch.autograd.Function):

    @staticmethod
    def forward(ctx, pos, strain, g, lmax, structure):
        pos4 = torch.zeros((pos.shape[0], 4), dtype=torch.float32, device=pos.device)
        pos4[:, :3] = pos
        Y, d, A = _edge_geometry_raw(pos4, g, True, True, lmax, strain=strain, structure=structure)
        ctx.g, ctx.lmax, ctx.structure = g, lmax, structure
        ctx.save_for_backward(pos4, strain)
        return Y, d, A

    @staticmethod
    def backward(ctx, gY, gd, gA):
        pos4, strain = ctx.saved_tensors
        g = ctx.g
        N = pos4.shape[0]
        gpos = torch.empty((N, 3), dtype=torch.float32, device=pos4.device)
        c = lambda t: t.contiguous() if t is not None else None
        gY, gd, gA = c(gY), c(gd), c(gA)
        p = lambda t: t.data_ptr() if t is not None else None
        gstrain = None
        with torch.cuda.device(pos4.device):
            lib = _lib.load()
            if strain is not None:
                gstrain = torch.empty_like(strain)
                ws = torch.empty(max(1, lib.e3_edge_geometry_backward_strained_workspace_bytes(N)), dtype=torch.uint8,
                                 device=pos4.device)
                name = "e3_edge_geometry_backward_strained" + ("_cell" if g.cell is not None else "")
                _lib.check(getattr(lib, name)(
                    pos4.data_ptr(), g.rowptr.data_ptr(), g.src.data_ptr(), N, ctx.lmax,
                    g.cell_arg if g.cell is not None else g.box_arg, strain.data_ptr(),
                    p(ctx.structure), strain.shape[0], p(gY), p(gd), p(gA), gpos.data_ptr(), gstrain.data_ptr(),
                    ws.data_ptr(), ws.numel(), _stream(pos4)), name)
            elif g.cell is not None:
                _lib.check(lib.e3_edge_geometry_backward_cell(
                    pos4.data_ptr(), g.rowptr.data_ptr(), g.src.data_ptr(), N, ctx.lmax, g.cell_arg, p(gY), p(gd), p(gA),
                    gpos.data_ptr(), _stream(pos4)), "e3_edge_geometry_backward_cell")
            elif g.box is not None:
                _lib.check(lib.e3_edge_geometry_backward_pbc(
                    pos4.data_ptr(), g.rowptr.data_ptr(), g.src.data_ptr(), N, ctx.lmax, g.box_arg, p(gY), p(gd), p(gA),
                    gpos.data_ptr(), _stream(pos4)), "e3_edge_geometry_backward_pbc")
            else:
                _lib.check(lib.e3_edge_geometry_backward(pos4.data_ptr(), g.rowptr.data_ptr(), g.src.data_ptr(),
                                                         N, ctx.lmax, p(gY), p(gd), p(gA), gpos.data_ptr(),
                                                         _stream(pos4)), "e3_edge_geometry_backward")
        return gpos, gstrain, None, None, None


def edge_geometry(g: RadiusGraph, want_dist=True, want_node_attr=True, lmax: int = 1, pos: torch.Tensor | None = None,
                  want_edge=True, strain: torch.Tensor | None = None, structure: torch.Tensor | None = None):
    _check(g.pos4, "pos4")
    if strain is None:
        if structure is not None:
            raise ValueError("structure= is the structure of each row for a strain=; it needs strain=")
        if pos is not None and _wants_grad(pos):
            _check(pos, "pos")
            return _EdgeGeometryFn.apply(pos, None, g, lmax, None)
        pos4 = g.pos4
        if pos is not None:
            pos4 = torch.zeros_like(g.pos4)
            pos4[:, :3] = pos
        return _edge_geometry_raw(pos4, g, want_dist, want_node_attr, lmax, want_edge)
    eps, sid = _strain_args(strain, structure, g)
    if pos is not None:
        _check(pos, "pos")
    if _wants_grad(pos, strain):
        return _EdgeGeometryFn.apply(pos if pos is not None else g.pos4[:, :3], eps, g, lmax, sid)
    pos4 = g.pos4
    if pos is not None:
        pos4 = torch.zeros_like(g.pos4)
        pos4[:, :3] = pos
    return _edge_geometry_raw(pos4, g, want_dist, want_node_attr, lmax, want_edge, strain=eps, structure=sid)


class _GatherConcatFn(torch.autograd.Function):
    @staticmethod
    def forward(ctx, h, extra, g):
        ctx.g, ctx.has_extra = g, extra is not None
        ctx.D, ctx.nx = h.shape[1], (extra.reshape(g.num_edges, -1).shape[1] if extra is not None else 0)
        return _gather_concat_raw(h, g, extra)

    @staticmethod
    def backward(ctx, gm):
        g, D, nx = ctx.g, ctx.D, ctx.nx
        gm = gm.contiguous()
        N = g.rowptr.numel() - 1
        gh = torch.empty((N, D), dtype=torch.float32, device=gm.device)
        gx = torch.empty((g.num_edges, nx), dtype=torch.float32, device=gm.device) if nx else None
        with torch.cuda.device(gm.device):
            _lib.check(_lib.load().e3_gather_concat_backward(gm.data_ptr(), gm.stride(0), D, g.rowptr.data_ptr(),
                                                             g.src.data_ptr(), N, nx, gh.data_ptr(), gh.stride(0),
                                                             gx.data_ptr() if gx is not None else None, _stream(gm)),
                       "e3_gather_concat_backward")
        if gx is not None and nx == 1:
            gx = gx
        return gh, gx, None


def _gather_concat_raw(h, g, extra):
    if h.stride(-1) != 1:
        h = h.contiguous()
    N, D = h.shape
    E = g.num_edges
    nx = 0
    if extra is not None:
        extra = extra.reshape(E, -1).contiguous()
        nx = extra.shape[1]
    out = torch.empty((E, 2 * D + nx), dtype=torch.float32, device=h.device)
    with torch.cuda.device(h.device):
        _lib.check(_lib.load().e3_gather_concat(h.data_ptr(), h.stride(0), D, g.rowptr.data_ptr(), g.src.data_ptr(), N,
                                                extra.data_ptr() if nx else None, nx, out.data_ptr(), out.stride(0),
                                                _stream(h)), "e3_gather_concat")
    return out


def gather_concat(h: torch.Tensor, g: RadiusGraph, extra: torch.Tensor | None = None) -> torch.Tensor:
    _check(h, "h")
    if extra is not None:
        _check(extra, "extra")
    if _wants_grad(h, extra):
        ex2 = extra.reshape(g.num_edges, -1) if extra is not None else None
        return _GatherConcatFn.apply(h, ex2, g)
    return _gather_concat_raw(h, g, extra)


class _GateBlocksFn(torch.autograd.Function):
    @staticmethod
    def forward(ctx, x, ns, blocks):
        ctx.ns, ctx.blocks = ns, blocks
        ctx.save_for_backward(x)
        return _gate_blocks_raw(x, ns, blocks)

    @staticmethod
    def backward(ctx, go):
        import ctypes
        (x,) = ctx.saved_tensors
        go = go.contiguous()
        gi = torch.empty_like(x)
        blocks = ctx.blocks
        ls = (ctypes.c_int32 * len(blocks))(*[l for l, _ in blocks])
        ms = (ctypes.c_int32 * len(blocks))(*[m for _, m in blocks])
        with torch.cuda.device(x.device):
            _lib.check(_lib.load().e3_gate_blocks_backward(x.data_ptr(), x.stride(0), go.data_ptr(), go.stride(0),
                                                           gi.data_ptr(), gi.stride(0), x.shape[0], ctx.ns, len(blocks),
                                                           ls, ms, _stream(x)), "e3_gate_blocks_backward")
        return gi, None, None


def gate(x: torch.Tensor, ns: int, nv: int) -> torch.Tensor:
    _check(x, "x")
    if x.stride(-1) != 1:
        x = x.contiguous()
    B = x.shape[0]
    assert x.shape[1] == ns + 4 * nv, (x.shape, ns, nv)
    if _wants_grad(x):
        return _GateBlocksFn.apply(x, ns, ((1, nv),))
    out = torch.empty((B, ns + 3 * nv), dtype=torch.float32, device=x.device)
    with torch.cuda.device(x.device):
        _lib.check(_lib.load().e3_gate(x.data_ptr(), x.stride(0), out.data_ptr(), out.stride(0), B, ns, nv,
                                       _stream(x)), "e3_gate")
    return out


class _SegmentSumFn(torch.autograd.Function):
    @staticmethod
    def forward(ctx, msg, g):
        ctx.g = g
        return _segment_sum_raw(msg, g)

    @staticmethod
    def backward(ctx, ga):
        g = ctx.g
        ga = ga.contiguous()
        N, D = ga.shape
        gm = torch.empty((g.num_edges, D), dtype=torch.float32, device=ga.device)
        with torch.cuda.device(ga.device):
            _lib.check(_lib.load().e3_segment_sum_backward(ga.data_ptr(), ga.stride(0), g.rowptr.data_ptr(), N, D,
                                                           gm.data_ptr(), max(gm.stride(0), D), _stream(ga)),
                       "e3_segment_sum_backward")
        return gm, None


def _segment_sum_raw(msg, g):
    if msg.stride(-1) != 1:
        msg = msg.contiguous()
    N = g.rowptr.numel() - 1
    D = msg.shape[1]
    agg = torch.empty((N, D), dtype=msg.dtype, device=msg.device)
    fn = "e3_segment_sum" if msg.dtype == torch.float32 else "e3_segment_sum_bf16"
    with torch.cuda.device(msg.device):
        _lib.check(getattr(_lib.load(), fn)(msg.data_ptr(), msg.stride(0), g.rowptr.data_ptr(), N, D,
                                            agg.data_ptr(), agg.stride(0), _stream(msg)), fn)
    return agg


def segment_sum(msg: torch.Tensor, g: RadiusGraph) -> torch.Tensor:
    if not msg.is_cuda:
        raise RuntimeError("msg: ROCm tensor required (no CPU path)")
    if msg.dtype not in (torch.float32, torch.bfloat16):
        raise RuntimeError(f"segment_sum: float32 / bfloat16 required, got {msg.dtype}")
    if msg.dtype == torch.float32 and _wants_grad(msg):
        return _SegmentSumFn.apply(msg, g)
    return _segment_sum_raw(msg, g)


def _gate_blocks_raw(x, ns, blocks):
    import ctypes
    B = x.shape[0]
    wide = sum(m * (2 * l + 1) for l, m in blocks)
    out = torch.empty((B, ns + wide), dtype=torch.float32, device=x.device)
    ls = (ctypes.c_int32 * len(blocks))(*[l for l, _ in blocks])
    ms = (ctypes.c_int32 * len(blocks))(*[m for _, m in blocks])
    with torch.cuda.device(x.device):
        _lib.check(_lib.load().e3_gate_blocks(x.data_ptr(), x.stride(0), out.data_ptr(), out.stride(0), B, ns,
                                              len(blocks), ls, ms, _stream(x)), "e3_gate_blocks")
    return out


def gate_blocks(x: torch.Tensor, ns: int, blocks) -> torch.Tensor:
    _check(x, "x")
    if x.stride(-1) != 1:
        x = x.contiguous()
    blocks = tuple((int(l), int(m)) for l, m in blocks)
    ng = sum(m for _, m in blocks)
    wide = sum(m * (2 * l + 1) for l, m in blocks)
    assert x.shape[1] == ns + ng + wide, (x.shape, ns, blocks)
    if _wants_grad(x):
        return _GateBlocksFn.apply(x, ns, blocks)
    return _gate_blocks_raw(x, ns, blocks)


def pow2_scale(tensors, target_log2: int = 10) -> torch.Tensor:
    import ctypes
    from .tensor_product import TPSegment
    ts = []
    for t in tensors:
        _check(t, "pow2_scale")
        if t.dim() == 1:
            t = t.unsqueeze(1)
        if t.stride(-1) != 1:
            t = t.contiguous()
        ts.append(t)
    assert 1 <= len(ts) <= 4
    dev = ts[0].device
    out = torch.empty(4, dtype=torch.float32, device=dev)
    segs = (TPSegment * len(ts))()
    rows = (ctypes.c_int64 * len(ts))()
    for i, t in enumerate(ts):
        segs[i].base, segs[i].ld, segs[i].ncols = t.data_ptr(), t.stride(0), t.shape[1]
        rows[i] = t.shape[0]
    with torch.cuda.device(dev):
        _lib.check(_lib.load().e3_pow2_scale(ctypes.byref(segs), rows, len(ts), target_log2, out.data_ptr(),
                                             _stream(out)), "e3_pow2_scale")
    return out


def join_pow2_scales(a: torch.Tensor, b: torch.Tensor) -> torch.Tensor:
    return torch.stack([torch.minimum(a[0], b[0]), torch.maximum(a[1], b[1]), torch.maximum(a[2], b[2]), a[3]])


def add_pow2_scale(h: torch.Tensor, u: torch.Tensor, target_log2: int = 10):
    _check(h, "h")
    _check(u, "u")
    assert h.shape == u.shape
    h, u = h.contiguous(), u.contiguous()
    out = torch.empty_like(h)
    sc = torch.empty(4, dtype=torch.float32, device=h.device)
    if h.numel() % 4 or (h.data_ptr() | u.data_ptr() | out.data_ptr()) % 16:
        torch.add(h, u, out=out)
        return out, pow2_scale([out], target_log2)
    with torch.cuda.device(h.device):
        _lib.check(_lib.load().e3_add_pow2_scale(h.data_ptr(), u.data_ptr(), out.data_ptr(), h.numel(), target_log2,
                                                 sc.data_ptr(), _stream(h)), "e3_add_pow2_scale")
    return out, sc
```

scalable-e3-gnn_amd/segnn.py:

```python
from __future__ import annotations

import torch
from torch import nn

from . import ops
from .irreps import Irreps
from .l1_tensor_prod import L1TensorProduct
from .message import FusedMessage
from .radius_graph import RadiusGraph
from .tensor_product import SHTensorProduct


def _hidden_irreps(H: int, lmax: int):
    hid = Irreps(f"{H}x0e+{H}x1o" + (f"+{H}x2e" if lmax == 2 else ""))
    gated = Irreps(f"{H}x0e+{lmax * H}x0e+{H}x1o" + (f"+{H}x2e" if lmax == 2 else ""))
    return hid, gated


def _make_tp(in_irreps, out_irreps, lmax: int):
    if lmax == 1:
        if Irreps(in_irreps).lmax == 1 and Irreps(out_irreps).lmax == 1:
            return L1TensorProduct(in_irreps, out_irreps)
        return SHTensorProduct(in_irreps, out_irreps, lmax_sh=1)
    return SHTensorProduct(in_irreps, out_irreps, lmax_sh=2)


class SEGNNLayer(nn.Module):
    _warned_unfused = False

    def __init__(self, H: int, lmax: int = 1):
        super().__init__()
        hid, gated = _hidden_irreps(H, lmax)
        self.H, self.lmax = H, lmax
        self.fused = True
        self.fuse_scatter = True
        self.fuse_message = True
        self._msg = FusedMessage(lmax, H) if FusedMessage.supported(lmax, H) else None
        self.msg1 = _make_tp(hid + hid + Irreps("1x0e"), gated, lmax)
        self.msg2 = _make_tp(hid, gated, lmax)
        self.upd1 = _make_tp(hid + hid, gated, lmax)
        self.upd2 = _make_tp(hid, hid, lmax)

    def _gate(self, t):
        H = self.H
        return ops.gate(t, H, H) if self.lmax == 1 else ops.gate_blocks(t, H, [(1, H), (2, H)])

    def fused_available(self) -> bool:
        f = getattr(self, "_fused_ok", None)
        if f is None:
            f = self._fused_ok = all(tp.fused_supported(True) for tp in (self.msg1, self.msg2, self.upd1))
        return f

    def fused_update_available(self) -> bool:
        f = getattr(self, "_fused_upd_ok", None)
        if f is None:
            f = self._fused_upd_ok = bool(self.upd1.fused_supported(True))
        return f

    def forward(self, h, g: RadiusGraph, Y, d, A, h_scale=None, halo=None, split=None):
        if (halo is not None or split is not None) and (g.box is not None or g.cell is not None):
            raise NotImplementedError("a periodic graph cannot be sharded (halo / split): build the local graph OPEN over the "
                                      "ghost images of GridHalo(..., periodic=...)")
        inference = not (torch.is_grad_enabled() and _needs_grad(self, h))
        if not inference and self.fused and not SEGNNLayer._warned_unfused:
            SEGNNLayer._warned_unfused = True
            import warnings
            warnings.warn("SEGNNLayer: a gradient is required (grad mode on and an input or parameter requires grad) -> the "
                          "unfused differentiable chain runs instead of the fused MFMA inference kernels; wrap inference in "
                          "torch.no_grad() to get the fast path", RuntimeWarning, stacklevel=2)
        f32 = h.dtype == torch.float32
        r16 = self.fused and inference and self.fused_available()
        one_launch = (self.fused and inference and self.fuse_message and self.fuse_scatter and self._msg is not None and
                      self._msg.supports(h.dtype))
        r16u = self.fused and inference and (r16 or (one_launch and self.fused_update_available()))
        if h.dtype == torch.bfloat16 and not ((one_launch or r16) and r16u):
            raise RuntimeError("bf16 storage needs the fused MFMA kernels (inference; hidden 32, or 64 at l_max = 2)")
        if halo is not None and not (one_launch and split is not None):
            halo.exchange(h)
        if one_launch and halo is not None and split is not None:
            tok = halo.start(h)
            if h_scale is None and f32:
                h_scale = ops.pow2_scale([h], target_log2=6)
            a, state = self._msg.forward(h, split.graph, self.msg1, self.msg2, h_scale, edges=split.interior,
                                         return_state=True)
            halo.finish(h, tok)
            if state is not None:
                top = self._msg.refresh_row_max(state, h, halo.ghost_rows(), h_scale if f32 else None)
                if f32:
                    flag = top >= 2.0 ** 15
                    halo.overflow = flag if getattr(halo, "overflow", None) is None else (halo.overflow | flag)
            a = self._msg.forward(h, split.graph, self.msg1, self.msg2, h_scale, edges=split.boundary, cont=state).to(h.dtype)
            del state
        elif one_launch:
            if h_scale is None and f32:
                h_scale = ops.pow2_scale([h])
            a = self._msg.forward(h, g, self.msg1, self.msg2, h_scale).to(h.dtype)
        elif r16:
            if d.dtype != h.dtype:
                d = d.to(h.dtype)
            m = self.msg1.forward_fused([(h, g.dst), (h, g.src), (d, None)], Y, gate=True,
                                        in_scale=ops.pow2_scale([h, d]) if f32 else None)
            a = None
            if self.fuse_scatter:
                a = self.msg2.forward_fused([(m, None)], Y, gate=True, scatter=(g.dst, g.rowptr.numel() - 1))
            if a is None:
                m = self.msg2.forward_fused([(m, None)], Y, gate=True)
                a = ops.segment_sum(m, g)
        else:
            m = ops.gather_concat(h, g, d)
            m = self._gate(self.msg1(m, Y))
            m = self._gate(self.msg2(m, Y))
            a = ops.segment_sum(m, g)
        if r16u:
            sc = None
            if f32 and h_scale is not None and halo is None:
                sc = ops.join_pow2_scales(h_scale, ops.pow2_scale([a]))
            if self.upd2.fused_supported(False) and h.stride(-1) == 1:
                if isinstance(self.upd1, SHTensorProduct) and a.stride(-1) == 1:
                    r = self.upd1.forward_update_pair(self.upd2, [(h, None), (a, None)], A, in_scale=sc, residual=h,
                                                      out_scale=10 if f32 else None)
                    if r is not None:
                        return r if f32 else (r, None)
                u, u_scale = self.upd1.forward_fused([(h, None), (a, None)], A, gate=True, in_scale=sc,
                                                     out_scale=10 if f32 else None) if f32 else \
                    (self.upd1.forward_fused([(h, None), (a, None)], A, gate=True), None)
                if f32:
                    return self.upd2.forward_fused([(u, None)], A, gate=False, in_scale=u_scale, residual=h, out_scale=10)
                return self.upd2.forward_fused([(u, None)], A, gate=False, residual=h), None
            u = self.upd1.forward_fused([(h, None), (a, None)], A, gate=True, in_scale=sc)
        else:
            u = self._gate(self.upd1(torch.cat([h, a], 1), A))
        u = self.upd2(u, A)
        if f32 and inference:
            return ops.add_pow2_scale(h, u)
        return h + u, None


def _needs_grad(mod: nn.Module, *tensors) -> bool:
    return any(t.requires_grad for t in tensors) or any(p.requires_grad for p in mod.parameters())


class SEGNN(nn.Module):
    def __init__(self, in_irreps="1x0e+1x1o", hidden: int = 32, out_irreps="1x1o", num_layers: int = 4, lmax: int = 1):
        super().__init__()
        assert lmax in (1, 2)
        self.hidden, self.lmax = hidden, lmax
        hid, _ = _hidden_irreps(hidden, lmax)
        self.in_irreps, self.out_irreps = Irreps(in_irreps), Irreps(out_irreps)
        self.embed = _make_tp(self.in_irreps, hid, lmax)
        self.layers = nn.ModuleList([SEGNNLayer(hidden, lmax) for _ in range(num_layers)])
        self.readout = _make_tp(hid, self.out_irreps, lmax)

    def forward(self, x: torch.Tensor, g: RadiusGraph, geometry=None, halo=None, split=None) -> torch.Tensor:
        if (halo is not None or split is not None) and (g.box is not None or g.cell is not None):
            raise NotImplementedError("a periodic graph cannot be sharded (halo / split): build the local graph OPEN over the "
                                      "ghost images of GridHalo(..., periodic=...)")
        if split is not None:
            g = split.graph
        if geometry is not None:
            Y, d, A = geometry
        else:
            one_launch = (not (torch.is_grad_enabled() and _needs_grad(self, x)) and
                          all(l.fused and l.fuse_message and l.fuse_scatter and l._msg is not None and
                              l._msg.supports(x.dtype) for l in self.layers))
            Y, d, A = ops.edge_geometry(g, lmax=self.lmax, want_edge=not one_launch)
        if x.dtype == torch.bfloat16 and self.lmax != 2:
            raise RuntimeError("bf16 storage is implemented for l_max = 2 (BASELINE config 3)")
        h = self.embed(x, A)
        sc = None
        if halo is not None:
            halo.overflow = None
        for layer in self.layers:
            if halo is not None:
                sc = None
            h, sc = layer(h, g, Y, d, A, sc, halo=halo, split=split)
        out = self.readout(h, A)
        if halo is not None and getattr(halo, "overflow", None) is not None and bool(halo.overflow):
            raise RuntimeError("sharded forward: a refreshed ghost row is more than 512 x larger than every row this rank held "
                               "when the layer's operand scale was fixed (fp16-split operands would overflow); run the layer "
                               "without `split` (blocking exchange) for such inputs")
        return out
```

Before: 11.36 million particles/s.

## Precompute per-edge spherical harmonics table once and stream it into the fused message kernel

The edge geometry kernel can now also write a 48-byte per-edge table (9 Y values plus distance). The warp-specialized fused message kernel gains a TAB mode that DMAs these rows into LDS instead of recomputing geometry from positions in every layer. SEGNN forward builds the table once when all layers support it and passes it to each of the four layers. This replaces per-layer recomputation with about 1.1 GB of extra memory and the bandwidth to write it once and read it each layer.

```diff
diff --git a/include/e3gnn.h b/include/e3gnn.h
--- a/include/e3gnn.h
+++ b/include/e3gnn.h
@@ -211,6 +211,10 @@
                         const int32_t* src, const int32_t* dst, int64_t E, const void* packed, const float* in_scale,
                         const float* premix, float* out, int64_t ld_out, int dtype, int accumulate, int tiles_per_block,
                         const float cell[9], void* stream);
+int e3_msg_forward_tab(e3_msg_plan* plan, const void* h, int64_t ld_h, int64_t N, const float* edge_tab,
+                       const int32_t* src, const int32_t* dst, int64_t E, const void* packed, const float* in_scale,
+                       const float* premix, float* out, int64_t ld_out, int dtype, int accumulate, int tiles_per_block,
+                       void* stream);
 int e3_segment_sum_bf16(const void* msg, int64_t ld_msg, const int32_t* rowptr, int64_t N, int D,
                         void* agg, int64_t ld_agg, void* stream);
 int e3_edge_geometry_l2(const float* pos4, const int32_t* rowptr, const int32_t* src, int64_t N,
@@ -219,6 +223,13 @@
                             float* edge_y, float* edge_d, float* node_a, void* stream);
 int e3_edge_geometry_l2_cell(const float* pos4, const int32_t* rowptr, const int32_t* src, int64_t N, const float cell[9],
                              float* edge_y, float* edge_d, float* node_a, void* stream);
+int e3_edge_geometry_l2_tab(const float* pos4, const int32_t* rowptr, const int32_t* src, int64_t N,
+                            float* edge_y, float* edge_d, float* node_a, float* edge_tab, void* stream);
+int e3_edge_geometry_l2_tab_pbc(const float* pos4, const int32_t* rowptr, const int32_t* src, int64_t N, const float box[3],
+                                float* edge_y, float* edge_d, float* node_a, float* edge_tab, void* stream);
+int e3_edge_geometry_l2_tab_cell(const float* pos4, const int32_t* rowptr, const int32_t* src, int64_t N,
+                                 const float cell[9], float* edge_y, float* edge_d, float* node_a, float* edge_tab,
+                                 void* stream);
 int e3_gate_blocks(const float* in, int64_t ld_in, float* out, int64_t ld_out, int64_t B, int ns,
                    int nblocks, const int32_t* ls, const int32_t* muls, void* stream);
 
diff --git a/scalable-e3-gnn_amd/_lib.py b/scalable-e3-gnn_amd/_lib.py
--- a/scalable-e3-gnn_amd/_lib.py
+++ b/scalable-e3-gnn_amd/_lib.py
@@ -8,6 +8,7 @@
 LIB_PATH = os.path.join(_HERE, "lib", "libe3gnn_hip.so")
 
 E3_OK = 0
+E3_ERR_UNSUPPORTED = 4
 E3_F32, E3_F64, E3_BF16 = 0, 1, 2
 CLS_NAMES = ("l0e", "l0o", "l1e", "l1o")
 
@@ -86,6 +87,8 @@
     "e3_msg_premix": (c_int, [c_void_p, c_void_p, c_int64, c_int64, c_void_p, c_void_p, c_void_p, c_int, c_void_p]),
     "e3_msg_forward": (c_int, [c_void_p, c_void_p, c_int64, c_int64, c_void_p, c_void_p, c_void_p, c_int64, c_void_p,
                                c_void_p, c_void_p, c_void_p, c_int64, c_int, c_int, c_int, c_void_p]),
+    "e3_msg_forward_tab": (c_int, [c_void_p, c_void_p, c_int64, c_int64, c_void_p, c_void_p, c_void_p, c_int64, c_void_p,
+                                   c_void_p, c_void_p, c_void_p, c_int64, c_int, c_int, c_int, c_void_p]),
     "e3_edge_geometry_backward": (c_int, [c_void_p, c_void_p, c_void_p, c_int64, c_int, c_void_p, c_void_p, c_void_p,
                                           c_void_p, c_void_p]),
     "e3_rg_sort_count_pbc": (c_int, [c_void_p, c_int64, c_void_p, c_int32, c_void_p, c_void_p, c_void_p, c_void_p,
@@ -145,6 +148,12 @@
                                             c_int64, c_int64, c_int, c_int, c_void_p, c_void_p]),
     "e3_segment_sum_bf16": (c_int, [c_void_p, c_int64, c_void_p, c_int64, c_int, c_void_p, c_int64, c_void_p]),
     "e3_edge_geometry_l2": (c_int, [c_void_p, c_void_p, c_void_p, c_int64, c_void_p, c_void_p, c_void_p, c_void_p]),
+    "e3_edge_geometry_l2_tab": (c_int, [c_void_p, c_void_p, c_void_p, c_int64, c_void_p, c_void_p, c_void_p, c_void_p,
+                                        c_void_p]),
+    "e3_edge_geometry_l2_tab_pbc": (c_int, [c_void_p, c_void_p, c_void_p, c_int64, Float3, c_void_p, c_void_p, c_void_p,
+                                            c_void_p, c_void_p]),
+    "e3_edge_geometry_l2_tab_cell": (c_int, [c_void_p, c_void_p, c_void_p, c_int64, Float9, c_void_p, c_void_p, c_void_p,
+                                             c_void_p, c_void_p]),
     "e3_gate_blocks": (c_int, [c_void_p, c_int64, c_void_p, c_int64, c_int64, c_int, c_int, POINTER(c_int32),
                                POINTER(c_int32), c_void_p]),
     "e3_l1tp_backward": (c_int, [c_void_p, c_void_p, c_int64, c_void_p, c_int64, VoidP4, VoidP4, c_void_p, c_int64,
diff --git a/scalable-e3-gnn_amd/csrc/e3_edge_ops.hip b/scalable-e3-gnn_amd/csrc/e3_edge_ops.hip
--- a/scalable-e3-gnn_amd/csrc/e3_edge_ops.hip
+++ b/scalable-e3-gnn_amd/csrc/e3_edge_ops.hip
@@ -127,7 +127,8 @@
                                                                const int32_t* __restrict__ src, int64_t N,
                                                                float* __restrict__ edge_y, float* __restrict__ edge_d,
                                                                float* __restrict__ node_a,
-                                                               const typename PbcArg<PBC>::type box, const StrainArg st) {
+                                                               const typename PbcArg<PBC>::type box, const StrainArg st,
+                                                               float4* __restrict__ edge_tab) {
   const int lane = threadIdx.x & 63;
   const int64_t wave0 = (blockIdx.x * (int64_t)blockDim.x + threadIdx.x) >> 6;
   const int64_t nw = ((int64_t)gridDim.x * blockDim.x) >> 6;
@@ -160,6 +161,14 @@
         for (int k = 0; k < 9; ++k) o[k] = Y[k];
       }
       if (edge_d) edge_d[q] = d;
+      if constexpr (!STRAIN) {
+        if (edge_tab) {
+          float4* o = edge_tab + (int64_t)q * 3;
+          o[0] = make_float4(Y[0], Y[1], Y[2], Y[3]);
+          o[1] = make_float4(Y[4], Y[5], Y[6], Y[7]);
+          o[2] = make_float4(Y[8], d, 0.f, 0.f);
+        }
+      }
 #pragma unroll
       for (int k = 0; k < 8; ++k) acc[k] += Y[k + 1];
     }
@@ -235,10 +244,11 @@
 template <int PBC>
 static int edge_geometry(int lmax, const float* pos4, const int32_t* rowptr, const int32_t* src, int64_t N, float* edge_y,
                          float* edge_d, float* node_a, const typename PbcArg<PBC>::type& b, const StrainArg* st,
-                         void* stream) {
+                         void* stream, float* edge_tab = nullptr) {
   if (N < 0) return E3_ERR_INVALID_ARG;
   if (N == 0) return E3_OK;
-  if (!pos4 || !rowptr || !src || (!edge_y && !node_a)) return E3_ERR_INVALID_ARG;
+  if (!pos4 || !rowptr || !src || (!edge_y && !node_a && !edge_tab)) return E3_ERR_INVALID_ARG;
+  if (edge_tab && (lmax != 2 || st || ((uintptr_t)edge_tab & 15))) return E3_ERR_INVALID_ARG;
   const StrainArg sa = st ? *st : StrainArg{nullptr, nullptr, 0};
   const hipStream_t s = (hipStream_t)stream;
   if (lmax == 1) {
@@ -248,16 +258,17 @@
   } else {
     auto kern = st ? edge_geometry_l2_kernel<PBC, true> : edge_geometry_l2_kernel<PBC, false>;
     hipLaunchKernelGGL(kern, dim3(wave_grid(N)), dim3(256), 0, s, (const float4*)pos4, rowptr, src, N, edge_y, edge_d,
-                       node_a, b, sa);
+                       node_a, b, sa, (float4*)edge_tab);
   }
   E3_HIP_CHECK(hipGetLastError());
   return E3_OK;
 }
 static int edge_geometry(int lmax, const float* pos4, const int32_t* rowptr, const int32_t* src, int64_t N, float* edge_y,
-                         float* edge_d, float* node_a, const float* box, const StrainArg* st, void* stream) {
+                         float* edge_d, float* node_a, const float* box, const StrainArg* st, void* stream,
+                         float* edge_tab = nullptr) {
   const PbcBox b = make_box(box);
-  return box ? edge_geometry<kBox>(lmax, pos4, rowptr, src, N, edge_y, edge_d, node_a, b, st, stream)
-             : edge_geometry<kOpen>(lmax, pos4, rowptr, src, N, edge_y, edge_d, node_a, b, st, stream);
+  return box ? edge_geometry<kBox>(lmax, pos4, rowptr, src, N, edge_y, edge_d, node_a, b, st, stream, edge_tab)
+             : edge_geometry<kOpen>(lmax, pos4, rowptr, src, N, edge_y, edge_d, node_a, b, st, stream, edge_tab);
 }
 
 bool e3::cell_derive(const float* cell, float ginv[9], float heights[3], float* volume) {
@@ -380,6 +391,25 @@
                             float* edge_y, float* edge_d, float* node_a, void* stream) {
   if (!box_valid(box, 0.0f)) return E3_ERR_INVALID_ARG;
   return edge_geometry(2, pos4, rowptr, src, N, edge_y, edge_d, node_a, box, nullptr, stream);
+}
+
+int e3_edge_geometry_l2_tab(const float* pos4, const int32_t* rowptr, const int32_t* src, int64_t N, float* edge_y,
+                            float* edge_d, float* node_a, float* edge_tab, void* stream) {
+  return edge_geometry(2, pos4, rowptr, src, N, edge_y, edge_d, node_a, nullptr, nullptr, stream, edge_tab);
+}
+
+int e3_edge_geometry_l2_tab_pbc(const float* pos4, const int32_t* rowptr, const int32_t* src, int64_t N, const float box[3],
+                                float* edge_y, float* edge_d, float* node_a, float* edge_tab, void* stream) {
+  if (!box_valid(box, 0.0f)) return E3_ERR_INVALID_ARG;
+  return edge_geometry(2, pos4, rowptr, src, N, edge_y, edge_d, node_a, box, nullptr, stream, edge_tab);
+}
+
+int e3_edge_geometry_l2_tab_cell(const float* pos4, const int32_t* rowptr, const int32_t* src, int64_t N,
+                                 const float cell[9], float* edge_y, float* edge_d, float* node_a, float* edge_tab,
+                                 void* stream) {
+  PbcCell c;
+  if (!make_cell(cell, 0.0f, &c)) return E3_ERR_INVALID_ARG;
+  return edge_geometry<kCell>(2, pos4, rowptr, src, N, edge_y, edge_d, node_a, c, nullptr, stream, edge_tab);
 }
 
 int e3_edge_geometry_strained(const float* pos4, const int32_t* rowptr, const int32_t* src, int64_t N, int lmax,
diff --git a/scalable-e3-gnn_amd/csrc/e3_msg_fused.hip b/scalable-e3-gnn_amd/csrc/e3_msg_fused.hip
--- a/scalable-e3-gnn_amd/csrc/e3_msg_fused.hip
+++ b/scalable-e3-gnn_amd/csrc/e3_msg_fused.hip
@@ -1100,14 +1100,19 @@
 static int msg_forward(e3_msg_plan* P, const void* h, int64_t ld_h, int64_t N, const float* pos4, const int32_t* src,
                        const int32_t* dst, int64_t E, const void* packed, const float* in_scale, const float* premix,
                        float* out, int64_t ld_out, int dtype, int accumulate, int tiles_per_block, void* stream,
-                       const float* box, const PbcCell* cell = nullptr) {
+                       const float* box, const PbcCell* cell = nullptr, const float* tab = nullptr,
+                       bool tab_entry = false) {
   if (!P || N < 0 || E < 0 || E > 0x7fffffffLL - 16) return E3_ERR_INVALID_ARG;
   if (!e3_msg_supports(P, dtype)) return E3_ERR_UNSUPPORTED;
+  if (tab_entry && (tiles_per_block < 0 || P->lmax != 2 || !msg_ws_supported(P->lmax, P->H, dtype) || E > 0x7fffffffLL - 65536))
+    return E3_ERR_UNSUPPORTED;
   const MsgKernels& k = *P->k;
   const int io = dtype == E3_BF16 ? 1 : 0, es = io ? 2 : 4;
   if (N == 0) return E3_OK;
-  if (!h || !pos4 || !packed || !premix || !out || ld_h < k.D || ld_out < k.D || (E > 0 && (!src || !dst)))
+  if (!h || (!pos4 && !tab_entry) || !packed || !premix || !out || ld_h < k.D || ld_out < k.D || (E > 0 && (!src || !dst)))
     return E3_ERR_INVALID_ARG;
+  if (tab_entry && E > 0 && !tab) return E3_ERR_INVALID_ARG;
+  if ((uintptr_t)tab & 15) return E3_ERR_INVALID_ARG;
   if ((ld_h * es & 15) || ((uintptr_t)h & 15) || ((uintptr_t)premix & 15)) return E3_ERR_INVALID_ARG;
   int st = msg_ensure_device(P);
   if (st != E3_OK) return st;
@@ -1116,8 +1121,8 @@
   if (E == 0) return E3_OK;
   if (tiles_per_block >= 0 && msg_ws_supported(P->lmax, P->H, dtype)) {
     st = msg_ws_launch(P->lmax, P->H, dtype, h, ld_h, N, pos4, src, dst, E, packed, in_scale, premix, out, ld_out,
-                       tiles_per_block > (1 << 20) ? (1 << 24) : tiles_per_block * 16, s, box, cell);
-    if (st != E3_ERR_UNSUPPORTED) return st;
+                       tiles_per_block > (1 << 20) ? (1 << 24) : tiles_per_block * 16, s, box, cell, tab);
+    if (st != E3_ERR_UNSUPPORTED || tab_entry) return st;
   }
   if (tiles_per_block < 0) tiles_per_block = -tiles_per_block;
   if (cell && (st = msg_ensure_cell(P, io)) != E3_OK) return st;
@@ -1166,6 +1171,13 @@
                      tiles_per_block, stream, nullptr, &c);
 }
 
+int e3_msg_forward_tab(e3_msg_plan* P, const void* h, int64_t ld_h, int64_t N, const float* edge_tab, const int32_t* src,
+                       const int32_t* dst, int64_t E, const void* packed, const float* in_scale, const float* premix,
+                       float* out, int64_t ld_out, int dtype, int accumulate, int tiles_per_block, void* stream) {
+  return msg_forward(P, h, ld_h, N, nullptr, src, dst, E, packed, in_scale, premix, out, ld_out, dtype, accumulate,
+                     tiles_per_block, stream, nullptr, nullptr, edge_tab, true);
+}
+
 #if E3_MSG_STAMP
 int e3_msg_debug_stamps(unsigned long long* out8, int reset) {
   if (out8 && hipMemcpyFromSymbol(out8, HIP_SYMBOL(e3::g_msg_stamps), 64) != hipSuccess) return E3_ERR_HIP;
diff --git a/scalable-e3-gnn_amd/csrc/e3_msg_ws.h b/scalable-e3-gnn_amd/csrc/e3_msg_ws.h
--- a/scalable-e3-gnn_amd/csrc/e3_msg_ws.h
+++ b/scalable-e3-gnn_amd/csrc/e3_msg_ws.h
@@ -7,5 +7,5 @@
 int msg_ws_launch(int lmax, int hidden, int dtype, const void* h, int64_t ldh, int64_t N, const float* pos4, const int32_t* src,
                   const int32_t* dst, int64_t E, const void* packed, const float* in_scale, const float* premix, float* out,
                   int64_t ldo, int chunk_edges, hipStream_t stream, const float* box = nullptr,
-                  const PbcCell* cell = nullptr);
+                  const PbcCell* cell = nullptr, const float* tab = nullptr);
 }
diff --git a/scalable-e3-gnn_amd/csrc/e3_msg_ws.hip b/scalable-e3-gnn_amd/csrc/e3_msg_ws.hip
--- a/scalable-e3-gnn_amd/csrc/e3_msg_ws.hip
+++ b/scalable-e3-gnn_amd/csrc/e3_msg_ws.hip
@@ -21,7 +21,7 @@
 #define WS_TPMARK(i)
 #endif
 
-template <int LMAX, int TT, bool IO16>
+template <int LMAX, int TT, bool IO16, bool TAB = false>
 struct Ws {
   using G = MsgGeom<LMAX, TT>;
   static_assert(TT == 2 && (LMAX == 1 || LMAX == 2), "instantiated for H = 32, l_max = 1 / 2");
@@ -57,7 +57,9 @@
   static constexpr int o_b2 = o_b1 + NFR * FRB;
   static constexpr int o_o = o_b2 + NFR * FRB;
   static constexpr int o_u = o_o + 16 * RS * 4;
-  static constexpr int total = o_u + 4 * U_ROW;
+  static constexpr int TROW = 48, TAB_BYTES = 16 * TROW;
+  static constexpr int o_etab = o_u + 4 * U_ROW;
+  static constexpr int total = o_etab + (TAB ? 2 * TAB_BYTES : 0);
   static_assert(total <= 160 * 1024, "LDS image exceeds the CU");
 };
 
@@ -79,6 +81,11 @@
 #else
   dma16(gsrc, lds_dst);
 #endif
+}
+__device__ __forceinline__ void dma16_base(const void* sbase, uint32_t voff, uint32_t lds_dst) {
+  uint32_t keep;
+  asm volatile("s_mov_b32 %0, m0\n\ts_mov_b32 m0, %3\n\ts_nop 0\n\tglobal_load_lds_dwordx4 %1, %2\n\ts_mov_b32 m0, %0"
+               : "=&s"(keep) : "v"(voff), "s"(sbase), "s"(lds_dst) : "memory");
 }
 __device__ __forceinline__ void dma4(const void* gsrc, uint32_t lds_dst) {
   uint32_t keep;
@@ -395,11 +402,15 @@
   BOX box;
 };
 using WsArgs = WsArgsT<PbcBox>;
+constexpr int kTab = 3;
+struct WsTab { const float* tab; };
+template <> struct PbcArg<kTab> { using type = WsTab; };
 
 template <int LMAX, int TT, bool IO16, int W, int PBC>
 __device__ __forceinline__ void ws_run(const WsArgsT<typename PbcArg<PBC>::type>& A, unsigned char* smem) {
   using G = MsgGeom<LMAX, TT>;
-  using L = Ws<LMAX, TT, IO16>;
+  constexpr bool TAB = PBC == kTab;
+  using L = Ws<LMAX, TT, IO16, TAB>;
   constexpr int H = G::H, D = G::D, ES = L::ES;
   constexpr bool TEAM1 = W >= 4;
   constexpr int ROLE = W & 3;
@@ -419,6 +430,14 @@
   const float bwx = A.packed[6] * ((!IO16 && A.in_scale) ? A.in_scale[1] : 1.0f);
   const char* hb = reinterpret_cast<const char*>(A.h);
 
+  auto tab_row = [&](const int tile, const int row, float (&y)[9], float& dist) {
+    const float* tr = reinterpret_cast<const float*>(smem + L::o_etab + (tile & 1) * L::TAB_BYTES + row * L::TROW);
+    const float a1 = tr[1];
+    const float2 a2 = *reinterpret_cast<const float2*>(tr + 2), c = *reinterpret_cast<const float2*>(tr + 8);
+    const f32x4 b = *reinterpret_cast<const f32x4*>(tr + 4);
+    y[0] = 1.0f; y[1] = a1; y[2] = a2.x; y[3] = a2.y; y[4] = b[0]; y[5] = b[1]; y[6] = b[2]; y[7] = b[3]; y[8] = c.x;
+    dist = c.y;
+  };
   auto tinfo = [&](const int tile) -> TileInfo {
     TileInfo ti = {0, 0, 0, -1, -1, 0, 0};
     if (tile >= 0) {
@@ -535,7 +554,16 @@
     if (lane == 0) {
       tip[0] = pe0; tip[1] = n; tip[2] = n0; tip[3] = node0; tip[4] = node1; tip[5] = sl0; tip[6] = sl1 >= 0 ? sl1 : sl0;
     }
-    if (lane < 32) {
+    if constexpr (TAB) {
+      if (lane < 48) {
+        const int lim = sgpr((Ei - pe0 < 16 ? Ei - pe0 : 16) * L::TROW);
+        int off = lane * 16;
+        if (off >= lim) off = lim - L::TROW + (off - lim) % L::TROW;
+        dma16_base(reinterpret_cast<const char*>(A.box.tab) + (int64_t)pe0 * L::TROW, (uint32_t)off,
+                   sgpr((int)(lds0 + L::o_etab + (tile & 1) * L::TAB_BYTES)));
+      }
+      if (lane < 32) dma4(A.hmax + myid, sgpr((int)(lds0 + L::o_hmx + (tile & 1) * 128)));
+    } else if (lane < 32) {
       dma16(A.pos4 + myid, sgpr((int)(lds0 + L::o_pos + (tile & 1) * 512)));
       dma4(A.hmax + myid, sgpr((int)(lds0 + L::o_hmx + (tile & 1) * 128)));
     }
@@ -600,7 +628,10 @@
         const unsigned char* gimg = smem + L::o_g;
         unsigned char* b1 = smem + L::o_b1 + (16 * gg + row) * 16 + 8 * pc;
         const float4* pp = reinterpret_cast<const float4*>(smem + L::o_pos + (s & 1) * 512);
-        const float4 ps = pp[row], pd = pp[16 + row];
+        float4 ps, pd;
+        float y[9], dist;
+        if constexpr (TAB) tab_row(s, row, y, dist);
+        else { ps = pp[row]; pd = pp[16 + row]; }
         float q2[20], q1[12], q0[4];
         {
           const unsigned char* r2 = gimg + row * L::GA_STRIDE + (LMAX == 2 ? (3 * H + (16 * pc + 4 * gg) * 5) * ES : 0);
@@ -625,8 +656,9 @@
           }
         }
         __builtin_amdgcn_sched_barrier(0);
-        float y[9], dist;
-        if constexpr (LMAX == 2) edge_sh<PBC>(ps, pd, y, dist, A.box); else edge_sh1<PBC>(ps, pd, y, dist, A.box);
+        if constexpr (!TAB) {
+          if constexpr (LMAX == 2) edge_sh<PBC>(ps, pd, y, dist, A.box); else edge_sh1<PBC>(ps, pd, y, dist, A.box);
+        }
         auto put4 = [&](const int fr, const float (&f)[4]) { ws_put4<IO16>(b1 + fr * L::FRB, f, xs); };
         auto degree = [&](auto ltag, float* q) {
           constexpr int L1 = decltype(ltag)::value, D1 = 2 * L1 + 1;
@@ -655,12 +687,15 @@
       }
       if ((ITB < ITE || SX == 2) && t0.n > 0) {
         const float4* pp = reinterpret_cast<const float4*>(smem + L::o_pos + (s & 1) * 512);
-        const float4 ps = pp[j], pd = pp[16 + j];
+        float4 ps, pd;
+        if constexpr (!TAB) { ps = pp[j]; pd = pp[16 + j]; }
         const int slot = (j >= t0.n0 && j < t0.n) ? t0.sl1 : t0.sl0;
         const float* urow = reinterpret_cast<const float*>(smem + L::o_u + slot * L::U_ROW) + 4 * g;
         constexpr int T0 = G::T(0);
         float y[9], dist;
-        if constexpr (LMAX == 2) edge_sh<PBC>(ps, pd, y, dist, A.box); else edge_sh1<PBC>(ps, pd, y, dist, A.box);
+        if constexpr (TAB) tab_row(s, j, y, dist);
+        else if constexpr (LMAX == 2) edge_sh<PBC>(ps, pd, y, dist, A.box);
+        else edge_sh1<PBC>(ps, pd, y, dist, A.box);
         const float dsc = dist * xs;
         float z110[3][1], z220[5][1];
         make_z<1, 1, 0>(y, z110);
@@ -915,7 +950,7 @@
 __global__ __launch_bounds__(512, 2) __attribute__((amdgpu_waves_per_eu(2, 2))) void msg_ws_kernel(
     const WsArgsT<typename PbcArg<PBC>::type> A) {
   using G = MsgGeom<LMAX, TT>;
-  using L = Ws<LMAX, TT, IO16>;
+  using L = Ws<LMAX, TT, IO16, PBC == kTab>;
   extern __shared__ __align__(16) unsigned char ws_smem[];
   {
     float* n1tab = reinterpret_cast<float*>(ws_smem + L::o_tab);
@@ -948,35 +983,39 @@
 
 int msg_ws_launch(int lmax, int hidden, int dtype, const void* h, int64_t ldh, int64_t N, const float* pos4, const int32_t* src,
                   const int32_t* dst, int64_t E, const void* packed, const float* in_scale, const float* premix, float* out,
-                  int64_t ldo, int chunk_edges, hipStream_t stream, const float* box, const PbcCell* cell) {
-  if (!msg_ws_supported(lmax, hidden, dtype)) return E3_ERR_UNSUPPORTED;
-  const int pb = cell ? kCell : (box ? kBox : kOpen);
+                  int64_t ldo, int chunk_edges, hipStream_t stream, const float* box, const PbcCell* cell, const float* tab) {
+  if (!msg_ws_supported(lmax, hidden, dtype) || (tab && lmax != 2)) return E3_ERR_UNSUPPORTED;
+  const int pb = tab ? kTab : cell ? kCell : (box ? kBox : kOpen);
   if (E > 0x7fffffffLL - 65536) return E3_ERR_UNSUPPORTED;
   const int io = dtype == E3_BF16 ? 1 : 0;
   const int li = lmax == 2 ? 1 : 0;
 #if WS_LMAX1
   const void* kern =
-      pb == kCell
+      pb == kTab ? (io ? (const void*)msg_ws_kernel<2, 2, true, kTab> : (const void*)msg_ws_kernel<2, 2, false, kTab>)
+      : pb == kCell
           ? (li ? (io ? (const void*)msg_ws_kernel<2, 2, true, kCell> : (const void*)msg_ws_kernel<2, 2, false, kCell>)
                 : (io ? (const void*)msg_ws_kernel<1, 2, true, kCell> : (const void*)msg_ws_kernel<1, 2, false, kCell>))
       : pb ? (li ? (io ? (const void*)msg_ws_kernel<2, 2, true, kBox> : (const void*)msg_ws_kernel<2, 2, false, kBox>)
                  : (io ? (const void*)msg_ws_kernel<1, 2, true, kBox> : (const void*)msg_ws_kernel<1, 2, false, kBox>))
            : (li ? (io ? (const void*)msg_ws_kernel<2, 2, true, kOpen> : (const void*)msg_ws_kernel<2, 2, false, kOpen>)
                  : (io ? (const void*)msg_ws_kernel<1, 2, true, kOpen> : (const void*)msg_ws_kernel<1, 2, false, kOpen>));
-  const int lds = li ? (io ? Ws<2, 2, true>::total : Ws<2, 2, false>::total) : (io ? Ws<1, 2, true>::total : Ws<1, 2, false>::total);
+  const int lds = tab ? (io ? Ws<2, 2, true, true>::total : Ws<2, 2, false, true>::total)
+                  : li ? (io ? Ws<2, 2, true>::total : Ws<2, 2, false>::total) : (io ? Ws<1, 2, true>::total : Ws<1, 2, false>::total);
   const int ud = li ? MsgGeom<2, 2>::UD : MsgGeom<1, 2>::UD;
 #else
   const void* kern =
-      pb == kCell ? (io ? (const void*)msg_ws_kernel<2, 2, true, kCell> : (const void*)msg_ws_kernel<2, 2, false, kCell>)
+      pb == kTab  ? (io ? (const void*)msg_ws_kernel<2, 2, true, kTab> : (const void*)msg_ws_kernel<2, 2, false, kTab>)
+      : pb == kCell ? (io ? (const void*)msg_ws_kernel<2, 2, true, kCell> : (const void*)msg_ws_kernel<2, 2, false, kCell>)
       : pb        ? (io ? (const void*)msg_ws_kernel<2, 2, true, kBox> : (const void*)msg_ws_kernel<2, 2, false, kBox>)
                   : (io ? (const void*)msg_ws_kernel<2, 2, true, kOpen> : (const void*)msg_ws_kernel<2, 2, false, kOpen>);
-  const int lds = io ? Ws<2, 2, true>::total : Ws<2, 2, false>::total;
+  const int lds = tab ? (io ? Ws<2, 2, true, true>::total : Ws<2, 2, false, true>::total)
+                      : (io ? Ws<2, 2, true>::total : Ws<2, 2, false>::total);
   const int ud = MsgGeom<2, 2>::UD;
 #endif
   int dev = 0;
   E3_HIP_CHECK(hipGetDevice(&dev));
   static std::mutex mu;
-  static int cus_of[64][2][2][3];
+  static int cus_of[64][2][2][4];
   int cus = 0;
   {
     std::lock_guard<std::mutex> lock(mu);
@@ -1000,7 +1039,7 @@
     void* args[] = {&a};
     return hipLaunchKernel(kern, dim3(nwg), dim3(512), args, lds, stream) == hipSuccess ? E3_OK : E3_ERR_HIP;
   };
-  return cell ? launch(*cell) : launch(make_box(box));
+  return tab ? launch(WsTab{tab}) : cell ? launch(*cell) : launch(make_box(box));
 }
 
 }
diff --git a/scalable-e3-gnn_amd/message.py b/scalable-e3-gnn_amd/message.py
--- a/scalable-e3-gnn_amd/message.py
+++ b/scalable-e3-gnn_amd/message.py
@@ -17,6 +17,7 @@
         self._plans = _lib.DevicePlans("e3_msg_plan_create", "e3_msg_plan_destroy", self.lmax, self.hidden)
         self._packed = {}
         self.tiles_per_block = 0
+        self.last_used_table = False
 
     def __deepcopy__(self, memo):
         return FusedMessage(self.lmax, self.hidden)
@@ -120,8 +121,12 @@
                             fl += 2 * H * M * groups
         return fl
 
+    def takes_edge_table(self, dtype) -> bool:
+        return (self.lmax == 2 and self.hidden == 32 and int(self.tiles_per_block) >= 0 and
+                dtype in (torch.float32, torch.bfloat16))
+
     def forward(self, h: torch.Tensor, g: RadiusGraph, msg1, msg2, in_scale: torch.Tensor | None = None, edges=None,
-                cont=None, return_state: bool = False):
+                cont=None, return_state: bool = False, edge_table: torch.Tensor | None = None):
         if not h.is_cuda or not self.supports(h.dtype):
             raise RuntimeError(f"fused message: ROCm tensor in float32 (or bfloat16 for hidden >= 32) required, got "
                                f"{h.dtype} on {h.device} (no CPU path)")
@@ -135,6 +140,12 @@
         lib = _lib.load()
         src, dst = (g.src, g.dst) if edges is None else edges
         E = int(src.numel())
+        if edge_table is not None:
+            if edges is not None:
+                raise ValueError("fused message: edge_table= is indexed by the edges of g; it excludes edges=")
+            if (tuple(edge_table.shape) != (E, 12) or edge_table.dtype != torch.float32 or edge_table.device != h.device or
+                    not edge_table.is_contiguous()):
+                raise RuntimeError(f"fused message: edge_table must be contiguous float32 [{E}, 12] on {h.device}")
         assert src.dtype == torch.int32 and dst.dtype == torch.int32 and dst.numel() == E
         if cont is None:
             out = torch.empty((N, W), dtype=torch.float32, device=dev)
@@ -166,7 +177,15 @@
             args = (hd, h.data_ptr(), h.stride(0), N, g.pos4.data_ptr(), src.data_ptr(), dst.data_ptr(), E,
                     packed.data_ptr(), sc, premix.data_ptr(), out.data_ptr(), out.stride(0), code,
                     0 if cont is None else 1, int(self.tiles_per_block))
-            if g.cell is not None:
+            st = _lib.E3_ERR_UNSUPPORTED
+            self.last_used_table = False
+            if edge_table is not None:
+                st = lib.e3_msg_forward_tab(*args[:4], edge_table.data_ptr(), *args[5:], stream)
+                if st != _lib.E3_ERR_UNSUPPORTED:
+                    _lib.check(st, "e3_msg_forward_tab")
+            if st != _lib.E3_ERR_UNSUPPORTED:
+                self.last_used_table = True
+            elif g.cell is not None:
                 _lib.check(lib.e3_msg_forward_cell(*args, g.cell_arg, stream), "e3_msg_forward_cell")
             elif g.box is not None:
                 _lib.check(lib.e3_msg_forward_pbc(*args, g.box_arg, stream), "e3_msg_forward_pbc")
diff --git a/scalable-e3-gnn_amd/ops.py b/scalable-e3-gnn_amd/ops.py
--- a/scalable-e3-gnn_amd/ops.py
+++ b/scalable-e3-gnn_amd/ops.py
@@ -21,36 +21,42 @@
     return torch.is_grad_enabled() and any(t is not None and t.requires_grad for t in ts)
 
 
-def _edge_geometry_raw(pos4, g, want_dist, want_node_attr, lmax, want_edge=True, strain=None, structure=None):
+def _edge_geometry_raw(pos4, g, want_dist, want_node_attr, lmax, want_edge=True, strain=None, structure=None,
+                       want_table=False):
     N, E, dev = g.rowptr.numel() - 1, g.num_edges, pos4.device
+    if want_table:
+        if lmax != 2 or strain is not None:
+            raise ValueError("the edge table is the l_max = 2 row of the unstrained geometry")
+        tab = torch.empty((E, 12), dtype=torch.float32, device=dev)
     ny = (lmax + 1) ** 2
     Y = torch.empty((E, ny), dtype=torch.float32, device=dev) if want_edge else None
     d = torch.empty(E, dtype=torch.float32, device=dev) if (want_dist and want_edge) else None
     A = torch.empty((N, ny), dtype=torch.float32, device=dev) if want_node_attr else None
-    fn = {1: "e3_edge_geometry", 2: "e3_edge_geometry_l2"}[lmax]
+    fn = {1: "e3_edge_geometry", 2: "e3_edge_geometry_l2"}[lmax] + ("_tab" if want_table else "")
     outs = (Y.data_ptr() if Y is not None else None, d.data_ptr() if d is not None else None,
-            A.data_ptr() if A is not None else None, _stream(pos4))
+            A.data_ptr() if A is not None else None) + ((tab.data_ptr(),) if want_table else ()) + (_stream(pos4),)
+    src_ptr = g.src.data_ptr() if E > 0 else g.rowptr.data_ptr()
     with torch.cuda.device(dev):
         if strain is not None and g.cell is not None:
             _lib.check(_lib.load().e3_edge_geometry_strained_cell(
-                pos4.data_ptr(), g.rowptr.data_ptr(), g.src.data_ptr(), N, lmax, g.cell_arg, strain.data_ptr(),
+                pos4.data_ptr(), g.rowptr.data_ptr(), src_ptr, N, lmax, g.cell_arg, strain.data_ptr(),
                 structure.data_ptr() if structure is not None else None, strain.shape[0], *outs),
                 "e3_edge_geometry_strained_cell")
         elif strain is not None:
             _lib.check(_lib.load().e3_edge_geometry_strained(
-                pos4.data_ptr(), g.rowptr.data_ptr(), g.src.data_ptr(), N, lmax, g.box_arg, strain.data_ptr(),
+                pos4.data_ptr(), g.rowptr.data_ptr(), src_ptr, N, lmax, g.box_arg, strain.data_ptr(),
                 structure.data_ptr() if structure is not None else None, strain.shape[0], *outs),
                 "e3_edge_geometry_strained")
         elif g.cell is not None:
-            _lib.check(getattr(_lib.load(), fn + "_cell")(pos4.data_ptr(), g.rowptr.data_ptr(), g.src.data_ptr(), N,
+            _lib.check(getattr(_lib.load(), fn + "_cell")(pos4.data_ptr(), g.rowptr.data_ptr(), src_ptr, N,
                                                           g.cell_arg, *outs), fn + "_cell")
         elif g.box is not None:
-            _lib.check(getattr(_lib.load(), fn + "_pbc")(pos4.data_ptr(), g.rowptr.data_ptr(), g.src.data_ptr(), N,
+            _lib.check(getattr(_lib.load(), fn + "_pbc")(pos4.data_ptr(), g.rowptr.data_ptr(), src_ptr, N,
                                                          g.box_arg, *outs), fn + "_pbc")
         else:
-            _lib.check(getattr(_lib.load(), fn)(pos4.data_ptr(), g.rowptr.data_ptr(), g.src.data_ptr(), N, *outs),
+            _lib.check(getattr(_lib.load(), fn)(pos4.data_ptr(), g.rowptr.data_ptr(), src_ptr, N, *outs),
                        "e3_edge_geometry")
-    return Y, d, A
+    return (Y, d, A, tab) if want_table else (Y, d, A)
 
 
 def _strain_args(strain, structure, g):
@@ -121,8 +127,11 @@
 
 
 def edge_geometry(g: RadiusGraph, want_dist=True, want_node_attr=True, lmax: int = 1, pos: torch.Tensor | None = None,
-                  want_edge=True, strain: torch.Tensor | None = None, structure: torch.Tensor | None = None):
+                  want_edge=True, strain: torch.Tensor | None = None, structure: torch.Tensor | None = None,
+                  want_table=False):
     _check(g.pos4, "pos4")
+    if want_table and (strain is not None or lmax != 2 or (pos is not None and _wants_grad(pos))):
+        raise ValueError("want_table: the edge table is the l_max = 2 row of the unstrained, non-differentiable geometry")
     if strain is None:
         if structure is not None:
             raise ValueError("structure= is the structure of each row for a strain=; it needs strain=")
@@ -133,7 +142,7 @@
         if pos is not None:
             pos4 = torch.zeros_like(g.pos4)
             pos4[:, :3] = pos
-        return _edge_geometry_raw(pos4, g, want_dist, want_node_attr, lmax, want_edge)
+        return _edge_geometry_raw(pos4, g, want_dist, want_node_attr, lmax, want_edge, want_table=want_table)
     eps, sid = _strain_args(strain, structure, g)
     if pos is not None:
         _check(pos, "pos")
diff --git a/scalable-e3-gnn_amd/segnn.py b/scalable-e3-gnn_amd/segnn.py
--- a/scalable-e3-gnn_amd/segnn.py
+++ b/scalable-e3-gnn_amd/segnn.py
@@ -57,7 +57,7 @@
             f = self._fused_upd_ok = bool(self.upd1.fused_supported(True))
         return f
 
-    def forward(self, h, g: RadiusGraph, Y, d, A, h_scale=None, halo=None, split=None):
+    def forward(self, h, g: RadiusGraph, Y, d, A, h_scale=None, halo=None, split=None, edge_table=None):
         if (halo is not None or split is not None) and (g.box is not None or g.cell is not None):
             raise NotImplementedError("a periodic graph cannot be sharded (halo / split): build the local graph OPEN over the "
                                       "ghost images of GridHalo(..., periodic=...)")
@@ -94,7 +94,7 @@
         elif one_launch:
             if h_scale is None and f32:
                 h_scale = ops.pow2_scale([h])
-            a = self._msg.forward(h, g, self.msg1, self.msg2, h_scale).to(h.dtype)
+            a = self._msg.forward(h, g, self.msg1, self.msg2, h_scale, edge_table=edge_table).to(h.dtype)
         elif r16:
             if d.dtype != h.dtype:
                 d = d.to(h.dtype)
@@ -157,13 +157,18 @@
                                       "ghost images of GridHalo(..., periodic=...)")
         if split is not None:
             g = split.graph
+        tab = None
         if geometry is not None:
             Y, d, A = geometry
         else:
             one_launch = (not (torch.is_grad_enabled() and _needs_grad(self, x)) and
                           all(l.fused and l.fuse_message and l.fuse_scatter and l._msg is not None and
                               l._msg.supports(x.dtype) for l in self.layers))
-            Y, d, A = ops.edge_geometry(g, lmax=self.lmax, want_edge=not one_launch)
+            if (one_launch and split is None and g.num_edges > 0 and
+                    all(l._msg.takes_edge_table(x.dtype) for l in self.layers)):
+                Y, d, A, tab = ops.edge_geometry(g, lmax=self.lmax, want_edge=False, want_table=True)
+            else:
+                Y, d, A = ops.edge_geometry(g, lmax=self.lmax, want_edge=not one_launch)
         if x.dtype == torch.bfloat16 and self.lmax != 2:
             raise RuntimeError("bf16 storage is implemented for l_max = 2 (BASELINE config 3)")
         h = self.embed(x, A)
@@ -173,7 +178,8 @@
         for layer in self.layers:
             if halo is not None:
                 sc = None
-            h, sc = layer(h, g, Y, d, A, sc, halo=halo, split=split)
+            h, sc = layer(h, g, Y, d, A, sc, halo=halo, split=split, edge_table=tab)
+        del tab
         out = self.readout(h, A)
         if halo is not None and getattr(halo, "overflow", None) is not None and bool(halo.overflow):
             raise RuntimeError("sharded forward: a refreshed ghost row is more than 512 x larger than every row this rank held "
```

New measurement: 11.45 million particles/s, median of 6. No clear change (+0.8%).
